# hagabbar/GenNet

Hardware: AMD Instinct MI355X
Metric: waveforms/sec (CNN+GAN step, 2048-sample BBH) (higher is better)
Workload: dtype f32

## Files before the change

### gennet_amd/csrc/bn.hip

```cpp
#include "common.h"

namespace gn {


__device__ __forceinline__ float bn_bwd_g(float dy, float y, uint8_t keep, int act, float p, float keep_scale) {
  if (!keep) return 0.f;
  const float yact = y / keep_scale;
  return dy * keep_scale * act_grad_from_y(yact, act, p);
}

__device__ __forceinline__ float bn_bwd_g_act(float dy, float yact, uint8_t keep, int act, float p, float keep_scale) {
  if (!keep) return 0.f;
  return dy * keep_scale * act_grad_from_y(yact, act, p);
}

__device__ __forceinline__ void lazy_dy_taps(const LazyDy& z, int C, int q, float wq[5][4]) {
#pragma unroll
  for (int j = 0; j < 5; ++j) {
    float4 w4 = make_float4(0.f, 0.f, 0.f, 0.f);
    if (j < z.k) w4 = *reinterpret_cast<const float4*>(z.w + (size_t)j * C + 4 * q);
    wq[j][0] = w4.x; wq[j][1] = w4.y; wq[j][2] = w4.z; wq[j][3] = w4.w;
  }
}
struct LazyWin {
  float win;
  int base;
  unsigned b;
};
template <bool UNI>
__device__ __forceinline__ void lazy_dy4(const LazyDy& z, unsigned b, int t, const float wq[5][4], float v[4], LazyWin& w) {
  float gv[5];
  if (UNI) {
    b = __builtin_amdgcn_readfirstlane(b);
    t = __builtin_amdgcn_readfirstlane(t);
    const int uhi = t + z.pad_left, ulo = uhi - (z.k - 1);
    if (b != w.b || ulo < w.base || uhi >= w.base + 64) {
      w.b = b;
      w.base = ulo;
      const int idx = ulo + (int)(threadIdx.x & 63);
      w.win = (idx >= 0 && idx < z.Lout) ? z.g[(size_t)b * z.Lout + idx] : 0.f;
    }
#pragma unroll
    for (int j = 0; j < 5; ++j)
      gv[j] = __int_as_float(__builtin_amdgcn_readlane(__float_as_int(w.win), max(uhi - j - w.base, 0)));
  } else {
    const float* gb = z.g + (size_t)b * z.Lout;
#pragma unroll
    for (int j = 0; j < 5; ++j) {
      const int u = t - j + z.pad_left;
      const int uc = min(max(u, 0), z.Lout - 1);
      const float g = gb[uc];
      gv[j] = (u == uc) ? g : 0.f;
    }
  }
  v[0] = v[1] = v[2] = v[3] = 0.f;
#pragma unroll
  for (int j = 0; j < 5; ++j)
#pragma unroll
    for (int e = 0; e < 4; ++e) v[e] = fmaf(gv[j], wq[j][e], v[e]);
}
__device__ __forceinline__ void lazy_dy_pos(const LazyDy& z, size_t r, unsigned* b, int* t) {
  *b = (unsigned)(r / (unsigned)z.L);
  *t = (int)(r - (size_t)*b * z.L);
}
__device__ __forceinline__ void lazy_dy_step(const LazyDy& z, int step, unsigned* b, int* t) {
  *t += step;
  while (*t >= z.L) { *t -= z.L; ++*b; }
}

template <int MODE>
__global__ __launch_bounds__(256) void colred_kernel(ColRedArgs a) {
  constexpr int NV = MODE == 0 ? 1 : 2;
  const int NQ = a.C >> 2;
  const int NQc = NQ < 256 ? NQ : 256;
  const int RL = 256 / NQc;
  const int tid = threadIdx.x, ql = tid % NQc, rl = tid / NQc;
  const int q = blockIdx.x * NQc + ql;
  double s[NV][4];
#pragma unroll
  for (int v = 0; v < NV; ++v)
#pragma unroll
    for (int e = 0; e < 4; ++e) s[v][e] = 0.0;
// ... 172 lines not shown
  else hipLaunchKernelGGL((colred_final_kernel<OUT, 32>), dim3(cdiv(n, 32)), dim3(256), 0, s, part, out, n, chunks);
}

static int colred_chunks(size_t rows, int C) {
  if (C % 4) {
    const int NCc = C < 256 ? C : 256, RL = 256 / NCc;
    const int gx = (C + NCc - 1) / NCc;
    int chunks = (1024 + gx - 1) / gx;
    const size_t max_chunks = (rows + (size_t)RL * 4 - 1) / ((size_t)RL * 4);
    if ((size_t)chunks > max_chunks) chunks = (int)max_chunks;
    return chunks < 1 ? 1 : chunks;
  }
  const int NQ = C / 4, NQc = NQ < 256 ? NQ : 256, RL = 256 / NQc;
  const int gx = (NQ + NQc - 1) / NQc;
  int chunks = (1024 + gx - 1) / gx;
  const size_t max_chunks = (rows + (size_t)RL * 4 - 1) / ((size_t)RL * 4);
  if ((size_t)chunks > max_chunks) chunks = (int)max_chunks;
  if (chunks < 1) chunks = 1;
  return chunks;
}
size_t colred_workspace_bytes(size_t rows, int C) { return (size_t)colred_chunks(rows, C) * 2 * C * sizeof(double); }

int colred_run(int mode, ColRedArgs a, void* ws, size_t ws_bytes, double* out_f64, float* out_f32, hipStream_t s) {
  if (a.C < 1) { set_error("column reduction: C %d", a.C); return GN_EINVAL; }
  if (a.C % 4 && a.lz.g) { set_error("column reduction: the on-the-fly conv gradient needs C %% 4 == 0"); return GN_EINVAL; }
  if (a.rows == 0) { set_error("column reduction: no rows"); return GN_EINVAL; }
  const int chunks = colred_chunks(a.rows, a.C);
  const int NV = mode == 0 ? 1 : 2;
  if (ws_bytes < (size_t)chunks * NV * a.C * sizeof(double)) { set_error("column reduction: workspace too small"); return GN_EWORKSPACE; }
  a.part = (double*)ws;
  a.rows_per_chunk = (int)((a.rows + chunks - 1) / chunks);
  if (a.C % 4) {
    const int NCc = a.C < 256 ? a.C : 256;
    dim3 grid((a.C + NCc - 1) / NCc, chunks);
    if (mode == 0) hipLaunchKernelGGL(colred_anyc_kernel<0>, grid, dim3(256), 0, s, a);
    else if (mode == 1) hipLaunchKernelGGL(colred_anyc_kernel<1>, grid, dim3(256), 0, s, a);
    else hipLaunchKernelGGL(colred_anyc_kernel<2>, grid, dim3(256), 0, s, a);
  } else {
    const int NQ = a.C / 4, NQc = NQ < 256 ? NQ : 256;
    dim3 grid((NQ + NQc - 1) / NQc, chunks);
    if (mode == 0) hipLaunchKernelGGL(colred_kernel<0>, grid, dim3(256), 0, s, a);
    else if (mode == 1) hipLaunchKernelGGL(colred_kernel<1>, grid, dim3(256), 0, s, a);
    else hipLaunchKernelGGL(colred_kernel<2>, grid, dim3(256), 0, s, a);
  }
  int rc = check_launch("colred");
  if (rc) return rc;
  const size_t n = (size_t)NV * a.C;
  if (out_f32) colred_final_launch((const double*)ws, out_f32, n, chunks, s);
  else colred_final_launch((const double*)ws, out_f64, n, chunks, s);
  return check_launch("colred_final");
}

int colred_finalize(const double* part, double* out_f64, size_t n, int chunks, hipStream_t s) {
  colred_final_launch(part, out_f64, n, chunks, s);
  return check_launch("colred_final");
}
int colred_finalize_f32(const double* part, float* out_f32, size_t n, int chunks, hipStream_t s) {
  colred_final_launch(part, out_f32, n, chunks, s);
  return check_launch("colred_final");
}

__global__ void colsum_anyc_kernel(const float* __restrict__ x, double* __restrict__ acc, size_t n, int C) {
  double s[4] = {0, 0, 0, 0};
  const size_t stride = (size_t)gridDim.x * blockDim.x;
  for (size_t i = (size_t)blockIdx.x * blockDim.x + threadIdx.x; i < n; i += stride) {
    const int c = (int)(i % C);
    const double v = (double)x[i];
    s[0] += c == 0 ? v : 0.0; s[1] += c == 1 ? v : 0.0; s[2] += c == 2 ? v : 0.0; s[3] += c == 3 ? v : 0.0;
  }
  __shared__ double red[4][256];
  for (int c = 0; c < 4; ++c) red[c][threadIdx.x] = s[c];
  __syncthreads();
  for (int sft = 128; sft >= 1; sft >>= 1) {
    if (threadIdx.x < sft)
      for (int c = 0; c < 4; ++c) red[c][threadIdx.x] += red[c][threadIdx.x + sft];
    __syncthreads();
  }
  if (threadIdx.x < C) atomicAdd(&acc[threadIdx.x], red[threadIdx.x][0]);
}
__global__ void f64_to_f32_small_kernel(const double* __restrict__ a, float* __restrict__ o, int n) {
  if ((int)threadIdx.x < n) o[threadIdx.x] = (float)a[threadIdx.x];
}

int bias_grad(const float* dy, float* db, size_t rows, int C, void* ws, size_t ws_bytes, hipStream_t s) {
  if (C % 4 == 0 || C > 4) {
    ColRedArgs r = {};
    r.a = dy; r.rows = rows; r.C = C;
    return colred_run(0, r, ws, ws_bytes, nullptr, db, s);
  }
  if (ws_bytes < 32) { set_error("bias_grad: workspace too small"); return GN_EWORKSPACE; }
  (void)hipMemsetAsync(ws, 0, 32, s);
  size_t g = (rows * C + 255) / 256;
  if (g > 1024) g = 1024;
  hipLaunchKernelGGL(colsum_anyc_kernel, dim3((unsigned)g), dim3(256), 0, s, dy, (double*)ws, rows * C, C);
  hipLaunchKernelGGL(f64_to_f32_small_kernel, dim3(1), dim3(64), 0, s, (const double*)ws, db, C);
  return check_launch("bias_grad");
}

size_t bias_grad_ws(size_t rows, int C) { return C % 4 == 0 || C > 4 ? colred_workspace_bytes(rows, C) : 32; }

__global__ void bn_finalize_kernel(const double* __restrict__ sums, double count, const float* __restrict__ gamma, const float* __restrict__ beta,
                                   float eps, float momentum, float* __restrict__ mm, float* __restrict__ mv, float* __restrict__ bm,
                                   float* __restrict__ bv, float zd_step, float* __restrict__ scale,
                                   float* __restrict__ shift, float* __restrict__ smean, float* __restrict__ sinv, int C, const int32_t* __restrict__ zd_step_dev) {
  const int c = blockIdx.x * blockDim.x + threadIdx.x;
  if (c >= C) return;
  if (zd_step_dev) zd_step = (float)*zd_step_dev;
  const double mean = sums[c] / count;
  double var = sums[C + c] / count - mean * mean;
  if (var < 0) var = 0;
  const float meanf = (float)mean, varf = (float)var;
  const float inv = 1.0f / sqrtf(varf + eps);
  const float sc = gamma[c] * inv;
  scale[c] = sc;
  shift[c] = beta[c] - meanf * sc;
  smean[c] = meanf;
  sinv[c] = inv;
  if (mm) {
    const float corr = (float)(count / (count - (1.0 + (double)eps)));
    const float decay = (float)(1.0 - (double)momentum);
    const float varc = varf * corr;
    if (bm) {
      const float nbm = bm[c] - (bm[c] - meanf) * decay;
      const float nbv = bv[c] - (bv[c] - varc) * decay;
      bm[c] = nbm;
      bv[c] = nbv;
      const float unb = 1.0f - powf(1.0f - decay, zd_step);
      mm[c] = mm[c] - (mm[c] - nbm / unb);
      mv[c] = mv[c] - (mv[c] - nbv / unb);
    } else {
      mm[c] = mm[c] - (mm[c] - meanf) * decay;
      mv[c] = mv[c] - (mv[c] - varc) * decay;
    }
  }
}
static int bn_finalize(const double* sums, double count, const float* gamma, const float* beta, float eps, float momentum, float* mm, float* mv,
                float* bm, float* bv, float zd_step, float* scale, float* shift, float* smean, float* sinv, int C, hipStream_t s, const int32_t* zd_step_dev = nullptr) {
  hipLaunchKernelGGL(bn_finalize_kernel, dim3(cdiv(C, 256)), dim3(256), 0, s, sums, count, gamma, beta, eps, momentum, mm, mv, bm, bv, zd_step, scale, shift,
                     smean, sinv, C, zd_step_dev);
  return check_launch("bn_finalize");
}

__global__ void bn_infer_coeffs_kernel(const float* __restrict__ gamma, const float* __restrict__ beta, const float* __restrict__ mm,
                                       const float* __restrict__ mv, float eps, float* __restrict__ scale, float* __restrict__ shift, int C) {
  const int c = blockIdx.x * blockDim.x + threadIdx.x;
  if (c >= C) return;
  const float sc = gamma[c] / sqrtf(mv[c] + eps);
  scale[c] = sc;
  shift[c] = beta[c] - mm[c] * sc;
}

__global__ void bn_apply_kernel(const float4* __restrict__ x, const float4* __restrict__ scale, const float4* __restrict__ shift,
                                const uchar4* __restrict__ mask, float4* __restrict__ y, size_t n4, int C4, int act, float p, float keep_scale) {
  const size_t stride = (size_t)gridDim.x * blockDim.x;
  for (size_t i = (size_t)blockIdx.x * blockDim.x + threadIdx.x; i < n4; i += stride) {
    const int c = (int)(i % C4);
    const float4 v = x[i], sc = scale[c], sh = shift[c];
    float4 o;
    o.x = act_apply(fmaf(v.x, sc.x, sh.x), act, p); o.y = act_apply(fmaf(v.y, sc.y, sh.y), act, p);
    o.z = act_apply(fmaf(v.z, sc.z, sh.z), act, p); o.w = act_apply(fmaf(v.w, sc.w, sh.w), act, p);
    if (mask) {
      const uchar4 m = mask[i];
      o.x = m.x ? o.x * keep_scale : 0.f; o.y = m.y ? o.y * keep_scale : 0.f;
      o.z = m.z ? o.z * keep_scale : 0.f; o.w = m.w ? o.w * keep_scale : 0.f;
    }
    y[i] = o;
  }
}
__global__ void bn_apply_anyc_kernel(const float* __restrict__ x, const float* __restrict__ scale, const float* __restrict__ shift,
                                     const uint8_t* __restrict__ mask, float* __restrict__ y, size_t n, int C, int act, float p, float keep_scale) {
  const size_t stride = (size_t)gridDim.x * blockDim.x;
  for (size_t i = (size_t)blockIdx.x * blockDim.x + threadIdx.x; i < n; i += stride) {
    const int c = (int)(i % C);
    float o = act_apply(fmaf(x[i], scale[c], shift[c]), act, p);
    if (mask) o = mask[i] ? o * keep_scale : 0.f;
    y[i] = o;
  }
}

__global__ void bn_bwd_apply_kernel(const float* __restrict__ dy, const float* __restrict__ y, const float* __restrict__ x, const uint8_t* __restrict__ mask,
                                    const float* __restrict__ gamma, const float* __restrict__ mean, const float* __restrict__ invstd,
                                    const double* __restrict__ dsums, double count, float* __restrict__ dx, size_t n, int C, int act, float p, float keep_scale,
                                    const float* __restrict__ scale, const float* __restrict__ shift) {
  const size_t stride = (size_t)gridDim.x * blockDim.x;
  for (size_t i = (size_t)blockIdx.x * blockDim.x + threadIdx.x; i < n; i += stride) {
    const int c = (int)(i % C);
    const uint8_t keep = mask ? mask[i] : (uint8_t)1;
    const float g = scale ? bn_bwd_g_act(dy[i], act_apply(fmaf(x[i], scale[c], shift[c]), act, p), keep, act, p, keep_scale)
                          : bn_bwd_g(dy[i], y[i], keep, act, p, keep_scale);
    const float inv = invstd[c];
    const float xh = (x[i] - mean[c]) * inv;
    const float mg = (float)(dsums[c] / count), mgx = (float)(dsums[C + c] / count);
    dx[i] = gamma[c] * inv * (g - mg - xh * mgx);
  }
}
__global__ __launch_bounds__(256) void bn_bwd_apply_v4_kernel(const float* __restrict__ dy, const float* __restrict__ y, const float* __restrict__ x,
                                                              const uint8_t* __restrict__ mask, const float* __restrict__ gamma, const float* __restrict__ mean,
                                                              const float* __restrict__ invstd, const double* __restrict__ dsums, double count,
                                                              const float* __restrict__ scale, const float* __restrict__ shift, float* __restrict__ dx,
                                                              size_t rows, int C, int rows_per_chunk, int act, float p, float keep_scale, LazyDy lz) {
  const int NQ = C >> 2;
  const int NQc = NQ < 256 ? NQ : 256;
  const int RL = 256 / NQc;
  const int tid = threadIdx.x, ql = tid % NQc, rl = tid / NQc;
  const int qblocks = (NQ + NQc - 1) / NQc;
  const int q = (blockIdx.x % qblocks) * NQc + ql;
  const size_t r_lo = (size_t)(blockIdx.x / qblocks) * rows_per_chunk;
  const size_t r_hi = r_lo + rows_per_chunk < rows ? r_lo + rows_per_chunk : rows;
  if (rl >= RL || q >= NQ) return;
  float gi[4], mu[4], is[4], mg[4], mgx[4], sc[4] = {0, 0, 0, 0}, sh[4] = {0, 0, 0, 0};
#pragma unroll
  for (int e = 0; e < 4; ++e) {
    const int c = 4 * q + e;
    is[e] = invstd[c]; mu[e] = mean[c]; gi[e] = gamma[c] * is[e];
    mg[e] = (float)(dsums[c] / count); mgx[e] = (float)(dsums[C + c] / count);
    if (scale) { sc[e] = scale[c]; sh[e] = shift[c]; }
  }
  float wq[5][4];
  LazyWin lw = {0.f, 0, 0xffffffffu};
  unsigned lb = 0;
  int lt = 0;
  if (lz.g) {
    lazy_dy_taps(lz, C, q, wq);
    lazy_dy_pos(lz, r_lo + rl, &lb, &lt);
  }
  constexpr int U = 2;
  const bool uni = ((NQc | NQ) & 63) == 0;
  for (size_t r = r_lo + rl; r < r_hi; r += (size_t)RL * U) {
    float4 d4[U], x4[U], y4[U];
    uchar4 m4[U];
    bool ok[U];
#pragma unroll
    for (int u = 0; u < U; ++u) {
      const size_t ru = r + (size_t)u * RL;
      ok[u] = ru < r_hi;
      const size_t o = (ok[u] ? ru : r) * C + 4 * q;
      x4[u] = *reinterpret_cast<const float4*>(x + o);
      if (!lz.g) d4[u] = *reinterpret_cast<const float4*>(dy + o);
      if (!scale) y4[u] = *reinterpret_cast<const float4*>(y + o);
      m4[u] = mask ? *reinterpret_cast<const uchar4*>(mask + o) : make_uchar4(1, 1, 1, 1);
    }
#pragma unroll
    for (int u = 0; u < U; ++u) {
      if (!ok[u]) break;
      const size_t o = (r + (size_t)u * RL) * C + 4 * q;
      const float xv[4] = {x4[u].x, x4[u].y, x4[u].z, x4[u].w};
      float dv[4];
      if (lz.g) {
        if (uni) lazy_dy4<true>(lz, lb, lt, wq, dv, lw);
        else lazy_dy4<false>(lz, lb, lt, wq, dv, lw);
        lazy_dy_step(lz, RL, &lb, &lt);
      } else {
        dv[0] = d4[u].x; dv[1] = d4[u].y; dv[2] = d4[u].z; dv[3] = d4[u].w;
      }
      float yv[4] = {0, 0, 0, 0};
      if (!scale) { yv[0] = y4[u].x; yv[1] = y4[u].y; yv[2] = y4[u].z; yv[3] = y4[u].w; }
      const uint8_t k[4] = {m4[u].x, m4[u].y, m4[u].z, m4[u].w};
      float ov[4];
#pragma unroll
      for (int e = 0; e < 4; ++e) {
        const float g = scale ? bn_bwd_g_act(dv[e], act_apply(fmaf(xv[e], sc[e], sh[e]), act, p), k[e], act, p, keep_scale)
                              : bn_bwd_g(dv[e], yv[e], k[e], act, p, keep_scale);
        const float xh = (xv[e] - mu[e]) * is[e];
        ov[e] = gi[e] * (g - mg[e] - xh * mgx[e]);
      }
      *reinterpret_cast<float4*>(dx + o) = make_float4(ov[0], ov[1], ov[2], ov[3]);
    }
  }
}
__global__ void bn_param_grads_kernel(const double* __restrict__ dsums_local, float* __restrict__ dgamma, float* __restrict__ dbeta, int C) {
  const int c = blockIdx.x * blockDim.x + threadIdx.x;
  if (c >= C) return;
  dbeta[c] = (float)dsums_local[c];
  dgamma[c] = (float)dsums_local[C + c];
}
static int bn_bwd_apply(const float* dy, const float* y, const float* x, const uint8_t* mask, const float* gamma, const float* mean, const float* invstd,
                 const double* dsums_global, double count, const double* dsums_local, float* dx, float* dgamma, float* dbeta, size_t rows, int C,
                 int act, float p, float rate, const float* scale, const float* shift, hipStream_t s, const LazyDy* lz = nullptr) {
  const size_t n = rows * C;
  if (!n) return GN_OK;
  LazyDy z = {};
  if (lz) z = *lz;
  if (z.g && (C % 4 || !scale)) { set_error("bn_bwd_apply: the on-the-fly conv gradient needs C %% 4 == 0 and scale / shift"); return GN_EINVAL; }
  if (C % 4 == 0) {
    const int NQ = C / 4, NQc = NQ < 256 ? NQ : 256, RL = 256 / NQc, qblocks = cdiv(NQ, NQc);
    size_t chunks = 8192 / qblocks;
    if (chunks < 1) chunks = 1;
    size_t rpc = (rows + chunks - 1) / chunks;
    rpc = ((rpc + RL - 1) / RL) * RL;
    if (rpc < (size_t)RL) rpc = RL;
    chunks = (rows + rpc - 1) / rpc;
    hipLaunchKernelGGL(bn_bwd_apply_v4_kernel, dim3((unsigned)(chunks * qblocks)), dim3(256), 0, s, dy, y, x, mask, gamma, mean, invstd, dsums_global, count, scale,
                       shift, dx, rows, C, (int)rpc, act, p, 1.0f / (1.0f - rate), z);
  } else {
    if (!y && !scale) { set_error("bn_bwd_apply: C %d %% 4 != 0 needs the stored layer output y or scale / shift", C); return GN_EINVAL; }
    hipLaunchKernelGGL(bn_bwd_apply_kernel, dim3(stream_grid(n)), dim3(256), 0, s, dy, y, x, mask, gamma, mean, invstd, dsums_global, count, dx, n, C, act, p,
                       1.0f / (1.0f - rate), y ? nullptr : scale, y ? nullptr : shift);
  }
  int rc = check_launch("bn_bwd_apply");
  if (rc) return rc;
  hipLaunchKernelGGL(bn_param_grads_kernel, dim3(cdiv(C, 256)), dim3(256), 0, s, dsums_local, dgamma, dbeta, C);
  return check_launch("bn_param_grads");
}

static int lazy_dy_check(const char* who, const float* g, const float* w, int L, int Lout, int k, int pad_left, size_t rows, int C, const float* scale,
                         const float* shift, LazyDy* z) {
  GN_REQUIRE(g && w && L > 0 && Lout > 0 && k >= 1 && k <= 5 && pad_left >= 0, "%s: bad conv description (1 filter, 1..5 taps, stride 1)", who);
  GN_REQUIRE(C % 4 == 0 && scale && shift, "%s: needs C %% 4 == 0 and the forward pass' scale / shift", who);
  GN_REQUIRE(rows % (size_t)L == 0 && rows / (size_t)L < 0x7fffffffull, "%s: rows %zu is not a whole number of length-%d segments", who, rows, L);
  z->g = g; z->w = w; z->L = L; z->Lout = Lout; z->k = k; z->pad_left = pad_left;
  return GN_OK;
}

}

using namespace gn;

extern "C" {

size_t gn_bn_stats_workspace(size_t rows, int C) { return colred_workspace_bytes(rows, C) + 256; }

int gn_bn_stats(const float* x, size_t rows, int C, double* sums, void* ws, size_t ws_bytes, void* stream) {
  GN_REQUIRE(x && sums && ws && rows > 0 && C > 0, "bn_stats: bad arguments");
  ColRedArgs r = {};
  r.a = x; r.rows = rows; r.C = C;
  return colred_run(1, r, ws, ws_bytes, sums, nullptr, (hipStream_t)stream);
}

int gn_bn_finalize(const double* sums, double count, const float* gamma, const float* beta, float eps, float momentum, float* moving_mean, float* moving_var,
                   float* scale, float* shift, float* save_mean, float* save_invstd, int C, void* stream) {
  GN_REQUIRE(sums && gamma && beta && scale && shift && save_mean && save_invstd && C > 0 && count > 1.0, "bn_finalize: bad arguments");
  GN_REQUIRE((moving_mean == nullptr) == (moving_var == nullptr), "bn_finalize: moving_mean/moving_var must both be given or both be NULL");
  return bn_finalize(sums, count, gamma, beta, eps, momentum, moving_mean, moving_var, nullptr, nullptr, 0.f, scale, shift, save_mean, save_invstd, C,
                     (hipStream_t)stream);
}
int gn_bn_finalize_zero_debias(const double* sums, double count, const float* gamma, const float* beta, float eps, float momentum, float* moving_mean,
                               float* moving_var, float* biased_mean, float* biased_var, int local_step, float* scale, float* shift, float* save_mean,
                               float* save_invstd, int C, void* stream) {
  GN_REQUIRE(sums && gamma && beta && scale && shift && save_mean && save_invstd && C > 0 && count > 1.0, "bn_finalize_zero_debias: bad arguments");
  GN_REQUIRE(moving_mean && moving_var && biased_mean && biased_var && local_step >= 1,
             "bn_finalize_zero_debias: needs moving_mean/var, the biased accumulators and the incremented local_step (>= 1, got %d)", local_step);
  return bn_finalize(sums, count, gamma, beta, eps, momentum, moving_mean, moving_var, biased_mean, biased_var, (float)local_step, scale, shift, save_mean,
                     save_invstd, C, (hipStream_t)stream);
}
int gn_bn_finalize_zero_debias_dyn(const double* sums, double count, const float* gamma, const float* beta, float eps, float momentum, float* moving_mean,
                                   float* moving_var, float* biased_mean, float* biased_var, const int32_t* local_step_dev, float* scale, float* shift,
                                   float* save_mean, float* save_invstd, int C, void* stream) {
  GN_REQUIRE(sums && gamma && beta && scale && shift && save_mean && save_invstd && C > 0 && count > 1.0, "bn_finalize_zero_debias_dyn: bad arguments");
  GN_REQUIRE(moving_mean && moving_var && biased_mean && biased_var && local_step_dev, "bn_finalize_zero_debias_dyn: needs moving statistics, accumulators, step");
  return bn_finalize(sums, count, gamma, beta, eps, momentum, moving_mean, moving_var, biased_mean, biased_var, 1.f, scale, shift, save_mean, save_invstd, C,
                     (hipStream_t)stream, local_step_dev);
}

int gn_bn_infer_coeffs(const float* gamma, const float* beta, const float* moving_mean, const float* moving_var, float eps, float* scale, float* shift, int C,
                       void* stream) {
  GN_REQUIRE(gamma && beta && moving_mean && moving_var && scale && shift && C > 0, "bn_infer_coeffs: bad arguments");
  hipLaunchKernelGGL(bn_infer_coeffs_kernel, dim3(cdiv(C, 256)), dim3(256), 0, (hipStream_t)stream, gamma, beta, moving_mean, moving_var, eps, scale, shift, C);
  return check_launch("bn_infer_coeffs");
}

int gn_bn_apply(const float* x, const float* scale, const float* shift, const uint8_t* mask, float* y, size_t rows, int C, int act, float p, float rate,
                void* stream) {
  GN_REQUIRE(x && scale && shift && y && C > 0, "bn_apply: bad arguments");
  GN_REQUIRE(rate >= 0.f && rate < 1.f && (mask || rate == 0.f), "bn_apply: dropout rate %f without mask", rate);
  hipStream_t s = (hipStream_t)stream;
  const float keep_scale = 1.0f / (1.0f - (mask ? rate : 0.f));
  if (C % 4) {
    const size_t n = rows * C;
    if (!n) return GN_OK;
    hipLaunchKernelGGL(bn_apply_anyc_kernel, dim3(stream_grid(n)), dim3(256), 0, s, x, scale, shift, mask, y, n, C, act, p, keep_scale);
    return check_launch("bn_apply");
  }
  const size_t n4 = rows * (C / 4);
  if (!n4) return GN_OK;
  hipLaunchKernelGGL(bn_apply_kernel, dim3(stream_grid(n4)), dim3(256), 0, s, (const float4*)x, (const float4*)scale, (const float4*)shift, (const uchar4*)mask,
                     (float4*)y, n4, C / 4, act, p, keep_scale);
  return check_launch("bn_apply");
}

int gn_bn_bwd_stats(const float* dy, const float* y, const float* x, const uint8_t* mask, const float* save_mean, const float* save_invstd, double* dsums, void* ws,
                    size_t ws_bytes, size_t rows, int C, int act, float p, float rate, const float* scale, const float* shift, void* stream) {
  GN_REQUIRE(dy && x && save_mean && save_invstd && dsums && ws && rows > 0 && C > 0, "bn_bwd_stats: bad arguments");
  GN_REQUIRE((scale == nullptr) == (shift == nullptr) && (y || scale), "bn_bwd_stats: needs the layer output y, or scale AND shift to recompute it");
  ColRedArgs r = {};
  r.a = dy; r.y = y; r.xpre = x; r.mask = mask; r.mean = save_mean; r.invstd = save_invstd; r.scale = scale; r.shift = shift;
  r.rows = rows; r.C = C; r.act = act; r.act_param = p; r.keep_scale = 1.0f / (1.0f - (mask ? rate : 0.f));
  return colred_run(2, r, ws, ws_bytes, dsums, nullptr, (hipStream_t)stream);
}
int gn_bn_bwd_apply(const float* dy, const float* y, const float* x, const uint8_t* mask, const float* gamma, const float* save_mean, const float* save_invstd,
                    const double* dsums_global, double count, const double* dsums_local, float* dx, float* dgamma, float* dbeta, size_t rows, int C, int act,
                    float p, float rate, const float* scale, const float* shift, void* stream) {
  GN_REQUIRE(dy && x && gamma && save_mean && save_invstd && dsums_global && dsums_local && dx && dgamma && dbeta && C > 0, "bn_bwd_apply: bad arguments");
  GN_REQUIRE((scale == nullptr) == (shift == nullptr) && (y || scale), "bn_bwd_apply: needs the layer output y, or scale AND shift to recompute it");
  return bn_bwd_apply(dy, y, x, mask, gamma, save_mean, save_invstd, dsums_global, count, dsums_local, dx, dgamma, dbeta, rows, C, act, p, mask ? rate : 0.f, scale,
                      shift, (hipStream_t)stream);
}

int gn_bn_bwd_stats_conv1(const float* g, const float* w, int L, int Lout, int k, int pad_left, const float* x, const uint8_t* mask, const float* save_mean,
                          const float* save_invstd, double* dsums, void* ws, size_t ws_bytes, size_t rows, int C, int act, float p, float rate,
                          const float* scale, const float* shift, void* stream) {
  GN_REQUIRE(x && save_mean && save_invstd && dsums && ws && rows > 0 && C > 0, "bn_bwd_stats_conv1: bad arguments");
  ColRedArgs r = {};
  int rc = lazy_dy_check("bn_bwd_stats_conv1", g, w, L, Lout, k, pad_left, rows, C, scale, shift, &r.lz);
  if (rc) return rc;
  r.a = nullptr; r.y = nullptr; r.xpre = x; r.mask = mask; r.mean = save_mean; r.invstd = save_invstd; r.scale = scale; r.shift = shift;
  r.rows = rows; r.C = C; r.act = act; r.act_param = p; r.keep_scale = 1.0f / (1.0f - (mask ? rate : 0.f));
  return colred_run(2, r, ws, ws_bytes, dsums, nullptr, (hipStream_t)stream);
}
int gn_bn_bwd_apply_conv1(const float* g, const float* w, int L, int Lout, int k, int pad_left, const float* x, const uint8_t* mask, const float* gamma,
                          const float* save_mean, const float* save_invstd, const double* dsums_global, double count, const double* dsums_local, float* dx,
                          float* dgamma, float* dbeta, size_t rows, int C, int act, float p, float rate, const float* scale, const float* shift, void* stream) {
  GN_REQUIRE(x && gamma && save_mean && save_invstd && dsums_global && dsums_local && dx && dgamma && dbeta && C > 0, "bn_bwd_apply_conv1: bad arguments");
  LazyDy z = {};
  int rc = lazy_dy_check("bn_bwd_apply_conv1", g, w, L, Lout, k, pad_left, rows, C, scale, shift, &z);
  if (rc) return rc;
  return bn_bwd_apply(nullptr, nullptr, x, mask, gamma, save_mean, save_invstd, dsums_global, count, dsums_local, dx, dgamma, dbeta, rows, C, act, p,
                      mask ? rate : 0.f, scale, shift, (hipStream_t)stream, &z);
}

size_t gn_bias_grad_workspace(size_t rows, int C) { return bias_grad_ws(rows, C) + 256; }

int gn_bias_grad(const float* dy, float* db, void* ws, size_t ws_bytes, size_t rows, int C, void* stream) {
  GN_REQUIRE(dy && db && ws && rows > 0 && C > 0, "bias_grad: bad arguments");
  return bias_grad(dy, db, rows, C, ws, ws_bytes, (hipStream_t)stream);
}

}
```

### gennet_amd/csrc/capi.hip

```cpp
#include <stdarg.h>
#include <algorithm>
#include <mutex>
#include <vector>
#include <stdlib.h>
#include "common.h"

namespace gn {

static thread_local char g_err[512] = "";

void set_error(const char* fmt, ...) {
  va_list ap;
  va_start(ap, fmt);
  vsnprintf(g_err, sizeof(g_err), fmt, ap);
  va_end(ap);
}

int check_launch(const char* what) {
  hipError_t e = hipGetLastError();
  if (e != hipSuccess) {
    set_error("%s: %s", what, hipGetErrorString(e));
    return GN_ELAUNCH;
  }
  return GN_OK;
// ... 393 lines not shown
  return dgrad_impl(dy, wt, dx, B, L, Cin, Cout, k, stride, pad_left, Lout, y_prev, mask_prev, act_prev, act_param_prev, mask_prev ? rate_prev : 0.f, stream);
}

static WgradArgs wgrad_args(const float* x, const float* dy, void* ws, int B, int L, int Cin, int Cout, int k, int stride, int pad_left, int Lout) {
  WgradArgs a = {};
  a.x = x; a.dy = dy; a.part = (float*)ws;
  a.B = B; a.Lin = L; a.Cin = Cin; a.Cout = Cout; a.M = Lout; a.ntaps = k; a.in_stride = stride;
  for (int j = 0; j < k && j < 8; ++j) a.off[j] = j - pad_left;
  return a;
}

size_t gn_conv1d_wgrad_workspace(int B, int L, int Cin, int Cout, int k, int stride, int Lout) {
  WgradArgs a = wgrad_args(nullptr, nullptr, nullptr, B, L, Cin, Cout, k, stride, 0, Lout);
  a.any_channels = 1;
  return std::max(wgrad_ws_need(select_wgrad(a), a), bias_grad_ws((size_t)B * Lout, Cout)) + 256;
}

static int wgrad_impl(const float* x, const float* dy, float* dw, float* db, void* ws, size_t ws_bytes, int B, int L, int Cin, int Cout, int k, int stride,
                      int pad_left, int Lout, bool any_channels, void* stream) {
  GN_REQUIRE(x && dy && dw && ws, "conv1d_wgrad: null pointer");
  GN_REQUIRE(B > 0 && L > 0 && Cin > 0 && Cout > 0 && k >= 1 && k <= 5 && stride >= 1 && Lout > 0 && pad_left >= 0, "conv1d_wgrad: bad shape");
  hipStream_t s = (hipStream_t)stream;
  WgradArgs a = wgrad_args(x, dy, ws, B, L, Cin, Cout, k, stride, pad_left, Lout);
  a.db = db;
  a.any_channels = any_channels;
  const WgradFamily f = select_wgrad(a);
  int rc = ws_check("conv1d_wgrad", std::max(wgrad_ws_need(f, a), bias_grad_ws((size_t)B * Lout, Cout)) + 256, ws_bytes);
  if (rc) return rc;
  switch (f) {
    case WGRAD_SMALL: {
      WgradSmallArgs sa = {x, dy, (float*)ws, B, L, Cin, Cout, Lout, k, stride};
      std::copy(a.off, a.off + k, sa.off);
      rc = wgrad_small_dispatch(sa, dw, ws_bytes, s);
      break;
    }
    case WGRAD_WINO: rc = wgrad_wino_run(a, dw, s); break;
    case WGRAD_WINO_S2: rc = wgrad_wino_s2_run(a, dw, s); break;
    case WGRAD_ANYC: rc = wgrad_anyc_dispatch(a, dw, ws_bytes, s); break;
    case WGRAD_BF16X3:
      rc = ws_check("conv-math", wgrad_bf16x3_workspace_bytes(B, Lout, Cin, Cout, stride), g_conv_ws_bytes);
      if (!rc) rc = wgrad_bf16x3_dispatch(a, dw, g_conv_ws, g_conv_ws_bytes, s);
      break;
    default:
      rc = wgrad_mfma_dispatch(a, dw, ws_bytes, s);
      if (!rc && a.db_done) return GN_OK;
  }
  if (rc) return rc;
  return db ? bias_grad(dy, db, (size_t)B * Lout, Cout, ws, ws_bytes, s) : GN_OK;
}

int gn_conv1d_wgrad(const float* x, const float* dy, float* dw, float* db, void* ws, size_t ws_bytes, int B, int L, int Cin, int Cout, int k, int stride,
                    int pad_left, int Lout, void* stream) {
  return wgrad_impl(x, dy, dw, db, ws, ws_bytes, B, L, Cin, Cout, k, stride, pad_left, Lout, false, stream);
}
int gn_conv1d_wgrad_any(const float* x, const float* dy, float* dw, float* db, void* ws, size_t ws_bytes, int B, int L, int Cin, int Cout, int k, int stride,
                        int pad_left, int Lout, void* stream) {
  return wgrad_impl(x, dy, dw, db, ws, ws_bytes, B, L, Cin, Cout, k, stride, pad_left, Lout, true, stream);
}

int gn_dense_fwd(const float* x, const float* w, const float* bias, float* y, int B, int in, int out, int act, float act_param, void* stream) {
  GN_REQUIRE(x && w && y && B >= 0 && in > 0 && out > 0, "dense_fwd: bad arguments");
  if (B == 0) return GN_OK;
  if (dense_any_shape(in, out))
    return dense_any_gemm(x, w, bias, y, B, out, in, (size_t)in, 1, (size_t)out, 1, act, act_param, (hipStream_t)stream);
  if (out <= 4) return dense_small_fwd(x, w, bias, y, B, in, out, act, act_param, (hipStream_t)stream);
  return conv_mfma_dispatch(fwd_args(x, w, bias, y, 1, B, in, out, 1, 1, 0, B, act, act_param), (hipStream_t)stream);
}

size_t gn_dense_bwd_workspace(int B, int in, int out) {
  if (out <= 4) return 256;
  if (dense_any_shape(in, out)) return bias_grad_ws((size_t)B, out) + 256;
  size_t w = wgrad_workspace_bytes(1, B, in, out, 1);
  size_t b = bias_grad_ws((size_t)B, out);
  return (w > b ? w : b) + (size_t)in * out * sizeof(float) + 256;
}

int gn_dense_bwd_fused(const float* x, const float* w, const float* dy, float* dx, float* dw, float* db, int B, int in, int out, const uint8_t* mask_prev,
                       int act_prev, float act_param_prev, float rate_prev, void* stream) {
  GN_REQUIRE(x && w && dy && dx && dw && B > 0 && in > 0 && out >= 1 && out <= 4, "dense_bwd_fused: bad arguments (small-output heads only)");
  GN_REQUIRE(rate_prev >= 0.f && rate_prev < 1.f, "dense_bwd_fused: bad rate");
  return dense_small_bwd(x, w, dy, dx, dw, db, B, in, out, (hipStream_t)stream, act_prev, act_param_prev, mask_prev, 1.0f / (1.0f - (mask_prev ? rate_prev : 0.f)));
}

int gn_dense_bwd(const float* x, const float* w, const float* dy, float* dx, float* dw, float* db, void* ws, size_t ws_bytes, int B, int in, int out, void* stream) {
  GN_REQUIRE(x && w && dy && dw && B > 0 && in > 0 && out > 0, "dense_bwd: bad arguments");
  hipStream_t s = (hipStream_t)stream;
  if (dense_any_shape(in, out)) {
    GN_REQUIRE(ws, "dense_bwd: null workspace");
    if (int rc = ws_check("dense_bwd", gn_dense_bwd_workspace(B, in, out), ws_bytes)) return rc;
    int rc = dx ? dense_any_gemm(dy, w, nullptr, dx, B, in, out, (size_t)out, 1, 1, (size_t)out, GN_ACT_LINEAR, 0.f, s) : GN_OK;
    if (!rc) rc = dense_any_gemm(x, dy, nullptr, dw, in, out, B, 1, (size_t)in, (size_t)out, 1, GN_ACT_LINEAR, 0.f, s);
    if (!rc && db) rc = bias_grad(dy, db, (size_t)B, out, ws, ws_bytes, s);
    return rc;
  }
  if (out <= 4) return dense_small_bwd(x, w, dy, dx, dw, db, B, in, out, s);
  GN_REQUIRE(ws, "dense_bwd: null workspace");
  if (int rc = ws_check("dense_bwd", gn_dense_bwd_workspace(B, in, out), ws_bytes)) return rc;
  const size_t wt_bytes = (size_t)in * out * sizeof(float);
  float* wt = (float*)ws;
  void* ws2 = (char*)ws + wt_bytes;
  const size_t ws2_bytes = ws_bytes - wt_bytes;
  int rc;
  if (dx) {
    rc = transpose_w(w, wt, 1, in, out, s);
    if (rc) return rc;
    rc = conv_run(fwd_args(dy, wt, nullptr, dx, 1, B, out, in, 1, 1, 0, B, GN_ACT_LINEAR, 0.f), s);
    if (rc) return rc;
  }
  WgradArgs g = wgrad_args(x, dy, ws2, 1, B, in, out, 1, 1, 0, B);
  rc = wgrad_mfma_dispatch(g, dw, ws2_bytes, s);
  if (rc) return rc;
  if (db) rc = bias_grad(dy, db, (size_t)B, out, ws2, ws2_bytes, s);
  return rc;
}

}
```

### gennet_amd/csrc/common.h

```cpp
#pragma once
#include <hip/hip_runtime.h>
#include <stdint.h>
#include <stdio.h>
#include "../../include/gennet_hip.h"

#define GN_LDS_DMA_CLOBBER() asm volatile("" ::: "v0", "v1", "v2", "v3")
#define gn_buffer_load_lds(...) do { __builtin_amdgcn_raw_ptr_buffer_load_lds(__VA_ARGS__); GN_LDS_DMA_CLOBBER(); } while (0)
#define gn_global_load_lds(...) do { __builtin_amdgcn_global_load_lds(__VA_ARGS__); GN_LDS_DMA_CLOBBER(); } while (0)

namespace gn {

void set_error(const char* fmt, ...);
int check_launch(const char* what);

struct Switches {
  bool conv_nopipe, conv_nodma, conv_nomerge, conv_nonarrow, conv_nopatch;
  bool wgrad_nopipe, bf16x3_no_merge;
  double bf16x3_min_gflop;
};
const Switches& switches();

const uint64_t* rng_base();
void prof_begin(hipStream_t s);
void prof_end(hipStream_t s, double flop, int kind, double bytes = 0.0);
// ... 39 lines not shown
  int ntaps, in_stride;
  int off[8];
  int chunks_per_split;
  double* db_part;
  float* db;
  int db_done;
  int any_channels;
};

struct WgradSmallArgs {
  const float* x;
  const float* dy;
  float* part;
  int B, Lin, Cin, Cout, M;
  int ntaps, in_stride;
  int off[8];
  int rows_per_chunk;
};

struct LazyDy {
  const float* g;
  const float* w;
  int L, Lout, k, pad_left;
};

struct ColRedArgs {
  const float* a;
  const float* y;
  const float* xpre;
  const uint8_t* mask;
  const float* mean;
  const float* invstd;
  const float* scale;
  const float* shift;
  double* part;
  size_t rows;
  int C;
  int rows_per_chunk;
  int act;
  float act_param;
  float keep_scale;
  LazyDy lz;
};

int conv_mfma_dispatch(const ConvArgs& a, hipStream_t s);
size_t wgrad_workspace_bytes(int B, int M, int Cin, int Cout, int ntaps);
int wgrad_mfma_dispatch(WgradArgs& a, float* dw, size_t ws_bytes, hipStream_t s);
int wgrad_bf16x3_dispatch(WgradArgs& a, float* dw, void* split_ws, size_t split_ws_bytes, hipStream_t s);
int conv_pipe_try(const ConvArgs& a, bool tall, hipStream_t s, bool* launched);
bool conv_pipe_merged_supported(const ConvArgs& a);
int conv_pipe_run_merged(const ConvArgs& a, hipStream_t s);
void wgrad_pipe_launch(const WgradArgs& a, dim3 grid, bool narrow, hipStream_t s);
size_t conv_bf16x3_workspace_bytes(int B, int Lin, int Cin, int Cout, int w_taps);
bool conv_bf16x3_supported(const ConvArgs& a);
int conv_bf16x3_split(const ConvArgs& a, int w_taps, void* ws, size_t ws_bytes, bool split_x, bool split_w, hipStream_t s);
int conv_bf16x3_run(const ConvArgs& a, int w_taps, void* ws, hipStream_t s);
int conv_bf16x3_merged_kind(const ConvArgs& a);
int conv_bf16x3_run_merged(const ConvArgs& a, void* ws, hipStream_t s);
size_t conv_wino_workspace_bytes(int Cin, int Cout);
bool conv_wino_supported(const ConvArgs& a);
int conv_wino_run(const ConvArgs& a, void* ws, size_t ws_bytes, hipStream_t s);
size_t conv_wino_s2_workspace_bytes(int Cin, int Cout);
int conv_wino_s2_kind(const ConvArgs& a);
int conv_wino_s2_run(const ConvArgs& a, void* ws, size_t ws_bytes, hipStream_t s);
void wgrad_split_plan(int B, int M, int Cin, int Cout, int TC, int TN, int* splits, int* chunks_per_split);
bool wgrad_wino_supported(const WgradArgs& a);
size_t wgrad_wino_workspace_bytes(int B, int M, int Cin, int Cout);
int wgrad_wino_run(WgradArgs& a, float* dw, hipStream_t s);
bool wgrad_wino_s2_supported(const WgradArgs& a);
size_t wgrad_wino_s2_workspace_bytes(int B, int M, int Cin, int Cout);
int wgrad_wino_s2_run(WgradArgs& a, float* dw, hipStream_t s);
size_t wgrad_bf16x3_workspace_bytes(int B, int M, int Cin, int Cout, int in_stride);
bool wgrad_bf16x3_supported(const WgradArgs& a);
int wgrad_bf16x3_run(const WgradArgs& a, int splits, void* ws, size_t ws_bytes, hipStream_t s);
int conv_anyc_dispatch(const ConvArgs& a, hipStream_t s);
size_t wgrad_anyc_workspace_bytes(int B, int M, int Cin, int Cout, int ntaps);
int wgrad_anyc_dispatch(WgradArgs& a, float* dw, size_t ws_bytes, hipStream_t s);
int conv_smallcin_dispatch(const ConvArgs& a, hipStream_t s);
int conv_smallcout_dispatch(const ConvArgs& a, hipStream_t s);
size_t wgrad_small_workspace_bytes(int B, int M, int Cin, int Cout, int ntaps);
int wgrad_small_dispatch(WgradSmallArgs a, float* dw, size_t ws_bytes, hipStream_t s);
int dense_small_fwd(const float* x, const float* w, const float* bias, float* y, int B, int in, int out, int act, float p, hipStream_t s);
int dense_small_bwd(const float* x, const float* w, const float* dy, float* dx, float* dw, float* db, int B, int in, int out, hipStream_t s,
                    int gact = 0, float gparam = 0.f, const uint8_t* gmask = nullptr, float gscale = 1.f);
size_t colred_workspace_bytes(size_t rows, int C);
int colred_run(int mode, ColRedArgs a, void* ws, size_t ws_bytes, double* out_f64, float* out_f32, hipStream_t s);
int colred_finalize(const double* part, double* out_f64, size_t n, int chunks, hipStream_t s);
int colred_finalize_f32(const double* part, float* out_f32, size_t n, int chunks, hipStream_t s);
size_t bias_grad_ws(size_t rows, int C);
int bias_grad(const float* dy, float* db, size_t rows, int C, void* ws, size_t ws_bytes, hipStream_t s);
int transpose_w(const float* w, float* wt, int k, int Cin, int Cout, hipStream_t s);

static inline unsigned cdiv(size_t a, size_t b) { return (unsigned)((a + b - 1) / b); }
static inline unsigned stream_grid(size_t n_items, int block = 256) {
  size_t g = (n_items + block - 1) / block;
  if (g > 256 * 8) g = 256 * 8;
  if (g < 1) g = 1;
  return (unsigned)g;
}

static inline void allow_big_lds(const void* kernel, unsigned long long* done) {
  int dev = 0;
  (void)hipGetDevice(&dev);
  const unsigned long long bit = 1ull << (dev & 63);
  if (!(*done & bit)) {
    (void)hipFuncSetAttribute(kernel, hipFuncAttributeMaxDynamicSharedMemorySize, 160 * 1024);
    *done |= bit;
  }
}

#define GN_REQUIRE(cond, ...)            \
  do {                                   \
    if (!(cond)) {                       \
      gn::set_error(__VA_ARGS__);        \
      return GN_EINVAL;                  \
    }                                    \
  } while (0)

__device__ __forceinline__ float gn_tanhf(float x) {
  const float ax = fabsf(x);
  const float e = __builtin_amdgcn_exp2f(ax * 2.8853900817779268f);
  const float big = 1.f - 2.f * __builtin_amdgcn_rcpf(e + 1.f);
  const float x2 = ax * ax;
  float q = fmaf(x2, -1382.f / 155925.f, 62.f / 2835.f);
  q = fmaf(x2, q, -17.f / 315.f);
  q = fmaf(x2, q, 2.f / 15.f);
  q = fmaf(x2, q, -1.f / 3.f);
  const float small = fmaf(ax * x2, q, ax);
  return copysignf(ax < 0.35f ? small : big, x);
}

__device__ __forceinline__ float act_apply(float x, int act, float p) {
  switch (act) {
    case GN_ACT_RELU: return fmaxf(x, 0.f);
    case GN_ACT_RELU_MAX: return fminf(fmaxf(x, 0.f), p);
    case GN_ACT_LEAKY: return x > 0.f ? x : p * x;
    case GN_ACT_TANH: return gn_tanhf(x);
    case GN_ACT_SIGMOID: return 1.f / (1.f + expf(-x));
    default: return x;
  }
}

__device__ __forceinline__ float act_grad_from_y(float y, int act, float p) {
  switch (act) {
    case GN_ACT_RELU: return y > 0.f ? 1.f : 0.f;
    case GN_ACT_RELU_MAX: return (y > 0.f && y < p) ? 1.f : 0.f;
    case GN_ACT_LEAKY: return y > 0.f ? 1.f : p;
    case GN_ACT_TANH: return 1.f - y * y;
    case GN_ACT_SIGMOID: return y * (1.f - y);
    default: return 1.f;
  }
}

struct Philox4 {
  uint32_t v[4];
};

__host__ __device__ __forceinline__ uint32_t mulhi32(uint32_t a, uint32_t b) { return (uint32_t)(((uint64_t)a * b) >> 32); }

__host__ __device__ __forceinline__ Philox4 philox4x32_10(uint64_t counter, uint64_t seed) {
  uint32_t c0 = (uint32_t)counter, c1 = (uint32_t)(counter >> 32), c2 = 0, c3 = 0;
  uint32_t k0 = (uint32_t)seed, k1 = (uint32_t)(seed >> 32);
#pragma unroll
  for (int r = 0; r < 10; ++r) {
    const uint32_t M0 = 0xD2511F53u, M1 = 0xCD9E8D57u;
    uint32_t h0 = mulhi32(M0, c0), l0 = M0 * c0;
    uint32_t h1 = mulhi32(M1, c2), l1 = M1 * c2;
// ... 17 lines not shown
```

### gennet_amd/csrc/small_conv.hip

```cpp
#include "common.h"

namespace gn {

static double small_conv_flop(int B, int M, int ntaps, int Cin, int Cout) { return 2.0 * B * (double)M * ntaps * Cin * Cout; }


constexpr int SMALLCIN_WIN = (2 * 255 + 5) * 4 + 4;

template <int CIN>
__global__ __launch_bounds__(256) void conv_smallcin_kernel(ConvArgs a, int m_tiles, int MT) {
  constexpr int MAXT = 5;
  const int NQ = a.Cout >> 2;
  const int NQc = NQ < 256 ? NQ : 256;
  const int RL = 256 / NQc;
  const int tid = threadIdx.x;
  const int q0 = tid % NQc, rl = tid / NQc;
  const int m_tile = blockIdx.x % m_tiles, b = blockIdx.x / m_tiles;
  const int m_lo = m_tile * MT, m_hi = min(a.M, m_lo + MT);
  const float* xb = a.x + (size_t)b * a.Lin * CIN;
  float* yb = a.y + (size_t)b * a.Ly * a.Cout;
  __shared__ float xw[SMALLCIN_WIN];
  int minoff = a.t.off[0], maxoff = a.t.off[0];
  for (int j = 1; j < a.t.ntaps; ++j) {
    minoff = min(minoff, a.t.off[j]);
// ... 510 lines not shown
    switch (CS) {
      case 1: hipLaunchKernelGGL(wgrad_smallcout_s1_kernel<1>, grid, dim3(256), 0, s, a); break;
      case 2: hipLaunchKernelGGL(wgrad_smallcout_s1_kernel<2>, grid, dim3(256), 0, s, a); break;
      case 3: hipLaunchKernelGGL(wgrad_smallcout_s1_kernel<3>, grid, dim3(256), 0, s, a); break;
      default: hipLaunchKernelGGL(wgrad_smallcout_s1_kernel<4>, grid, dim3(256), 0, s, a); break;
    }
    prof_end(s, small_conv_flop(a.B, a.M, a.ntaps, a.Cin, a.Cout), 16);
    int rc1 = check_launch("wgrad_smallcout_s1");
    if (rc1) return rc1;
    const size_t n1 = (size_t)a.ntaps * a.Cin * a.Cout;
    return sum_partials(a.part, dw, n1, chunks, s);
  }
#define GN_WS(CSV)                                                                                            \
  if (small_in) hipLaunchKernelGGL((wgrad_smallcin_tab_kernel<CSV>), grid, dim3(256), 0, s, a);               \
  else hipLaunchKernelGGL((wgrad_small_kernel<CSV, false>), grid, dim3(256), 0, s, a);
  prof_begin(s);
  switch (CS) {
    case 1: GN_WS(1); break;
    case 2: GN_WS(2); break;
    case 3: GN_WS(3); break;
    default: GN_WS(4); break;
  }
#undef GN_WS
  prof_end(s, small_conv_flop(a.B, a.M, a.ntaps, a.Cin, a.Cout), small_in ? 14 : 15);
  int rc = check_launch("wgrad_small");
  if (rc) return rc;
  const size_t n = (size_t)a.ntaps * a.Cin * a.Cout;
  return sum_partials(a.part, dw, n, chunks, s);
}

template <int OUT>
__global__ __launch_bounds__(1024) void dense_small_fwd_kernel(const float* __restrict__ x, const float* __restrict__ w, const float* __restrict__ bias,
                                                               float* __restrict__ y, int in, int act, float act_param) {
  const int b = blockIdx.x, tid = threadIdx.x;
  const float* xb = x + (size_t)b * in;
  float acc[OUT];
#pragma unroll
  for (int o = 0; o < OUT; ++o) acc[o] = 0.f;
  for (int i = 4 * tid; i < in; i += 4096) {
    const float4 xv = *reinterpret_cast<const float4*>(xb + i);
    if (OUT == 1) {
      const float4 wv = *reinterpret_cast<const float4*>(w + i);
      acc[0] = fmaf(xv.x, wv.x, acc[0]); acc[0] = fmaf(xv.y, wv.y, acc[0]);
      acc[0] = fmaf(xv.z, wv.z, acc[0]); acc[0] = fmaf(xv.w, wv.w, acc[0]);
    } else {
      const float xs[4] = {xv.x, xv.y, xv.z, xv.w};
#pragma unroll
      for (int e = 0; e < 4; ++e)
#pragma unroll
        for (int o = 0; o < OUT; ++o) acc[o] = fmaf(xs[e], w[(size_t)(i + e) * OUT + o], acc[o]);
    }
  }
  __shared__ float red[16][OUT];
#pragma unroll
  for (int o = 0; o < OUT; ++o) {
    float v = acc[o];
#pragma unroll
    for (int sft = 32; sft >= 1; sft >>= 1) v += __shfl_xor(v, sft, 64);
    if ((tid & 63) == 0) red[tid >> 6][o] = v;
  }
  __syncthreads();
  if (tid < OUT) {
    float v = 0.f;
    for (int k = 0; k < 16; ++k) v += red[k][tid];
    y[(size_t)b * OUT + tid] = act_apply(v + (bias ? bias[tid] : 0.f), act, act_param);
  }
}

int dense_small_fwd(const float* x, const float* w, const float* bias, float* y, int B, int in, int out, int act, float p, hipStream_t s) {
  if (out < 1 || out > 4 || in % 4) {
    set_error("dense_small_fwd: out %d (1..4) / in %d (%%4) unsupported", out, in);
    return GN_EINVAL;
  }
  if (B == 0) return GN_OK;
  switch (out) {
    case 1: hipLaunchKernelGGL(dense_small_fwd_kernel<1>, dim3(B), dim3(1024), 0, s, x, w, bias, y, in, act, p); break;
    case 2: hipLaunchKernelGGL(dense_small_fwd_kernel<2>, dim3(B), dim3(1024), 0, s, x, w, bias, y, in, act, p); break;
    case 3: hipLaunchKernelGGL(dense_small_fwd_kernel<3>, dim3(B), dim3(1024), 0, s, x, w, bias, y, in, act, p); break;
    default: hipLaunchKernelGGL(dense_small_fwd_kernel<4>, dim3(B), dim3(1024), 0, s, x, w, bias, y, in, act, p); break;
  }
  return check_launch("dense_small_fwd");
}

template <int OUT>
__global__ __launch_bounds__(256) void dense_small_bwd_kernel(const float* __restrict__ x, const float* __restrict__ w, const float* __restrict__ dy,
                                                              float* __restrict__ dx, float* __restrict__ dw, int B, int in, int gact, float gparam,
                                                              const uint8_t* __restrict__ gmask, float gscale) {
  const size_t i = ((size_t)blockIdx.x * 256 + threadIdx.x) * 4;
  if (i >= (size_t)in) return;
  float wv[4][OUT], acc[4][OUT];
#pragma unroll
  for (int e = 0; e < 4; ++e)
#pragma unroll
    for (int o = 0; o < OUT; ++o) {
      wv[e][o] = w[(i + e) * OUT + o];
      acc[e][o] = 0.f;
    }
  constexpr int U = 8;
  for (int b0 = 0; b0 < B; b0 += U) {
    float4 xq[U];
    uchar4 mq[U];
#pragma unroll
    for (int u = 0; u < U; ++u) {
      const int bb = min(b0 + u, B - 1);
      xq[u] = *reinterpret_cast<const float4*>(x + (size_t)bb * in + i);
      mq[u] = (dx && gmask) ? *reinterpret_cast<const uchar4*>(gmask + (size_t)bb * in + i) : make_uchar4(1, 1, 1, 1);
    }
#pragma unroll
    for (int u = 0; u < U; ++u) {
    const int b = b0 + u;
    if (b >= B) break;
    const float4 xv = xq[u];
    const float xs[4] = {xv.x, xv.y, xv.z, xv.w};
    float g[OUT];
#pragma unroll
    for (int o = 0; o < OUT; ++o) g[o] = dy[(size_t)b * OUT + o];
    float d[4] = {0.f, 0.f, 0.f, 0.f};
#pragma unroll
    for (int e = 0; e < 4; ++e)
#pragma unroll
      for (int o = 0; o < OUT; ++o) {
        acc[e][o] = fmaf(xs[e], g[o], acc[e][o]);
        d[e] = fmaf(g[o], wv[e][o], d[e]);
      }
    if (dx) {
      if (gact != GN_ACT_LINEAR || gmask) {
        const uint8_t k[4] = {mq[u].x, mq[u].y, mq[u].z, mq[u].w};
#pragma unroll
        for (int e = 0; e < 4; ++e) d[e] = k[e] ? d[e] * gscale * act_grad_from_y(xs[e] / gscale, gact, gparam) : 0.f;
      }
      *reinterpret_cast<float4*>(dx + (size_t)b * in + i) = make_float4(d[0], d[1], d[2], d[3]);
    }
    }
  }
#pragma unroll
  for (int e = 0; e < 4; ++e)
#pragma unroll
    for (int o = 0; o < OUT; ++o) dw[(i + e) * OUT + o] = acc[e][o];
}

__global__ void colsum_small_kernel(const float* __restrict__ dy, float* __restrict__ db, int B, int out) {
  const int o = threadIdx.x;
  if (o >= out) return;
  float s = 0.f;
  for (int b = 0; b < B; ++b) s += dy[(size_t)b * out + o];
  db[o] = s;
}

int dense_small_bwd(const float* x, const float* w, const float* dy, float* dx, float* dw, float* db, int B, int in, int out, hipStream_t s, int gact,
                    float gparam, const uint8_t* gmask, float gscale) {
  if (out < 1 || out > 4 || in % 4) {
    set_error("dense_small_bwd: out %d (1..4) / in %d (%%4) unsupported", out, in);
    return GN_EINVAL;
  }
  const unsigned grid = cdiv((size_t)in / 4, 256);
  switch (out) {
    case 1: hipLaunchKernelGGL(dense_small_bwd_kernel<1>, dim3(grid), dim3(256), 0, s, x, w, dy, dx, dw, B, in, gact, gparam, gmask, gscale); break;
    case 2: hipLaunchKernelGGL(dense_small_bwd_kernel<2>, dim3(grid), dim3(256), 0, s, x, w, dy, dx, dw, B, in, gact, gparam, gmask, gscale); break;
    case 3: hipLaunchKernelGGL(dense_small_bwd_kernel<3>, dim3(grid), dim3(256), 0, s, x, w, dy, dx, dw, B, in, gact, gparam, gmask, gscale); break;
    default: hipLaunchKernelGGL(dense_small_bwd_kernel<4>, dim3(grid), dim3(256), 0, s, x, w, dy, dx, dw, B, in, gact, gparam, gmask, gscale); break;
  }
  int rc = check_launch("dense_small_bwd");
  if (rc) return rc;
  if (db) {
    hipLaunchKernelGGL(colsum_small_kernel, dim3(1), dim3(64), 0, s, dy, db, B, out);
    rc = check_launch("colsum_small");
  }
  return rc;
}

}
```

### gennet_amd/engine.py

```python
import re

import numpy as np
import torch

from . import ops

_DEVICE = None


def device():
    global _DEVICE
    if _DEVICE is None:
        import os
        if not torch.cuda.is_available():
            from ._lib import GennetHipError
            raise GennetHipError('gennet_amd needs an AMD GPU (torch.cuda.is_available() is False); there is no CPU execution path')
        idx = int(os.environ.get('LOCAL_RANK', '0')) % max(torch.cuda.device_count(), 1)
        torch.cuda.set_device(idx)
        _DEVICE = torch.device('cuda', idx)
        ops.set_conv_math(device=_DEVICE)
    return _DEVICE


def to_device(a, dtype=torch.float32):
# ... 156 lines not shown
        i = len(self.providers)
        if i >= self.SLOTS:
            raise RuntimeError('StepGraph: more than %d step-varying scalars' % self.SLOTS)
        self.providers.append((i, fmt, provider))
        return ops.DevScalar(self.dev.data_ptr() + 8 * i)

    def capture(self, fn):
        global _CAPTURE
        if _CAPTURE is not None:
            raise RuntimeError('StepGraph.capture: already capturing')
        rng = device_rng()
        self.rng_start = rng.offset

        def keep(buf):
            if not any(b is buf for b in self.scratch):
                self.scratch.append(buf)

        def rng_base():
            base = device_rng().offset - self.rng_start
            device_rng().offset += self.rng_taken
            return base
        base = self.slot('Q', rng_base)
        if ops.conv_math_workspace() is not None:
            keep(ops.conv_math_workspace())
        self.graph = torch.cuda.CUDAGraph()
        _CAPTURE = self
        ops.set_rng_base(base.ptr)
        ops._ws_on_use = keep
        prof = ops.prof_enabled()
        if prof:
            ops.prof_enable(False)
        try:
            with torch.cuda.graph(self.graph):
                self.outputs = fn()
        finally:
            ops.set_rng_base(None)
            ops._ws_on_use = None
            _CAPTURE = None
            if prof:
                ops.prof_enable(True)
            self.rng_taken = rng.offset - self.rng_start
            rng.offset = self.rng_start
        return self.outputs

    def wait_inputs_consumed(self):
        if self._copied_once:
            self.copied.synchronize()

    def replay(self):
        for i, fmt, provider in self.providers:
            self._struct.pack_into('<' + fmt, self.hostbuf, 8 * i, provider())
        self.dev.copy_(self.host, non_blocking=True)
        self.copied.record()
        self._copied_once = True
        self.graph.replay()
        return self.outputs


def set_device_seed(seed):
    global _RNG
    _RNG = PhiloxStream(seed)


def device_rng():
    return _RNG


class RunContext(object):
    def __init__(self, training, dp=None, dropout_masks=None, train_params=None, site=None, row_map=None):
        self.training = training
        self.row_map = row_map
        self.site = site
        self.capture = None
        self.dp = dp
        self.dropout_masks = dropout_masks or {}
        self.train_ids = None if train_params is None else set(id(p) for p in train_params)
        self.tape = {}
        self.epi = {}
        self.pre_applied = set()
        self.skip = set()
        self.bn_sums = {}
        self.reg = None
        self.reg_y = {}

    def wants_grad(self, layer):
        if self.train_ids is None:
            return False
        return any(id(p) in self.train_ids for p in layer.trainable_params())


class SymTensor(object):
    def __init__(self, shape, layer=None, inbound=(), name=None):
        self.shape = tuple(shape)
        self.layer = layer
        self.inbound = tuple(inbound)
        self.name = name


_NAME_COUNTS = {}


def to_snake_case(name):
    intermediate = re.sub('(.)([A-Z][a-z0-9]+)', r'\1_\2', name)
    insecure = re.sub('([a-z])([A-Z])', r'\1_\2', intermediate).lower()
    return 'private' + insecure if insecure[0] == '_' else insecure


def _unique_name(base):
    _NAME_COUNTS[base] = _NAME_COUNTS.get(base, 0) + 1
    return '%s_%d' % (base, _NAME_COUNTS[base])


def Input(shape=None, name=None, batch_shape=None, dtype=None):
    if shape is None and batch_shape is not None:
        shape = tuple(batch_shape[1:])
    return SymTensor(shape, name=name or _unique_name('input'))


class Layer(object):

    def __init__(self, input_shape=None, name=None, trainable=True, **kwargs):
        if name is None:
            name = _unique_name(to_snake_case(self.__class__.__name__))
        self.name = name
        self.trainable = trainable
        self.built = False
        self.input_shape_arg = tuple(input_shape) if input_shape is not None else None
        self.params = []
        self.buffers = []

    def add_weight(self, name, value, trainable=True, regularizer=None):
        p = Param('%s/%s' % (self.name, name), value, trainable, regularizer)
        (self.params if trainable else self.buffers).append(p)
        return p

    def trainable_params(self):
        return self.params

    @property
    def trainable_weights(self):
        return list(self.params) if self.trainable else []

    @property
    def non_trainable_weights(self):
        return list(self.buffers) + ([] if self.trainable else list(self.params))

    @property
    def weights(self):
        return list(self.params) + list(self.buffers)

    def get_weights(self):
        return [p.numpy() for p in self.weights]

    def set_weights(self, ws):
        assert len(ws) == len(self.weights), '%s expects %d arrays' % (self.name, len(self.weights))
        for p, w in zip(self.weights, ws):
            p.assign(w)

    def count_params(self):
        return sum(p.size for p in self.weights)

    def build(self, input_shape):
        self.built = True

    def compute_output_shape(self, input_shape):
        return input_shape

    def get_config(self):
        from . import keras_io
        return keras_io.layer_config(self)

    def _is_user_layer(self):
        return callable(getattr(type(self), 'call', None)) and type(self).forward is Layer.forward

    def _ensure_built(self, input_shape):
        if not self.built:
            self.build((None,) + tuple(input_shape) if self._is_user_layer() else tuple(input_shape))
            self.built = True

    def _shape_after(self, input_shape):
        if self._is_user_layer():
            out = tuple(self.compute_output_shape((None,) + tuple(input_shape)))[1:]
            self._lower(tuple(input_shape), out)
            return out
        return tuple(self.compute_output_shape(tuple(input_shape)))

    def _lower(self, input_shape, out_shape):
        if getattr(self, '_lowered', None) is None or self._lowered_for != input_shape:
            from .keras import backend as K
            self._lowered = K.lower_layer_call(self, input_shape)
            self._lowered_for = input_shape
            if tuple(out_shape) != (input_shape[0], 2, 1):
                raise ValueError('%s.compute_output_shape gives %r; its call produces %r' % (type(self).__name__, (None,) + tuple(out_shape), (None, input_shape[0], 2, 1)))
        return self._lowered

    def __call__(self, x):
        if isinstance(x, (list, tuple)):
            if not self.is_merge:
                raise ValueError('%s (%s) takes a single tensor, not a list of %d: only the merge layers (Add, Subtract, Multiply, Average, Maximum, '
                                 'Minimum, Concatenate) join tensors' % (self.name, type(self).__name__, len(x)))
            if len(x) < 2:
                raise ValueError('A merge layer should be called on a list of at least 2 inputs (%s got %d)' % (self.name, len(x)))
            shapes = [tuple(t.shape) for t in x]
            if not self.built:
                self.build(shapes)
                self.built = True
            return SymTensor(tuple(self.compute_output_shape(shapes)), self, tuple(x))
        if self.is_merge:
            raise ValueError('A merge layer should be called on a list of at least 2 inputs (%s got a single tensor)' % self.name)
        self._ensure_built(x.shape)
        return SymTensor(self._shape_after(x.shape), self, (x,))

    is_merge = False
    fusable_act = False
    fusable_drop = False
    act_spec = None
    activity_regularizer = None
    drop_rate = None

    def writes_dy(self, node):
        return False

    def forward(self, ctx, node, x):
        if not self._is_user_layer():
            raise NotImplementedError
        low = self._lower(tuple(x.shape[1:]), tuple(node.out_shape))
        b0, b1 = low.betas()
        return ops.affine_stack_fwd(x.contiguous(), low.a0, b0, low.a1, b1)

    def backward(self, ctx, node, dy, need_dx, need_dw):
        if not self._is_user_layer():
            raise NotImplementedError
        return ops.affine_stack_bwd(dy.contiguous(), self._lowered.a0, self._lowered.a1)


class Node(object):
    __slots__ = ('layer', 'inbound', 'fused_act', 'fused_drop', 'absorbed', 'index', 'out_shape', 'owners', 'fuse_prev', 'infer_bn', 'fold_up', 'lazy_bn')

    def __init__(self, layer, inbound, out_shape, owners=()):
        self.layer = layer
        self.owners = tuple(owners)
        self.inbound = list(inbound)
        self.fused_act = None
        self.fused_drop = None
        self.absorbed = False
        self.index = -1
        self.out_shape = out_shape
        self.fuse_prev = -1
        self.fold_up = None
        self.infer_bn = None
        self.lazy_bn = -1


def _f32(x):
    return float(np.float32(x))


class Optimizer(object):
    RULE = None
    SLOTS = ()
    SAVES_ITERATIONS = True
    CONFIG = ()

    def __init__(self, lr, decay=0.0, clipnorm=None, clipvalue=None, **kwargs):
        if kwargs:
            raise TypeError('Unexpected keyword argument passed to optimizer: %s' % sorted(kwargs)[0])
        self.lr, self.decay = _f32(lr), _f32(decay)
        self.clipnorm, self.clipvalue = clipnorm, clipvalue
        self.iterations = 0
        self.state = None

    def _n_slots(self):
        return len(self.SLOTS)

    def _hyper(self):
        return 0.0, 0.0, 0.0, False

    def _lr_eff(self, it):
        return self.lr / (1.0 + self.decay * it) if self.decay > 0 else self.lr

    def _scalar(self, it):
        return self._lr_eff(it)

    def _layout(self):
        return list(range(self._n_slots()))

    def get_config(self):
        cfg = {'lr': self.lr}
        cfg.update((k, getattr(self, k)) for k in self.CONFIG)
        if self.clipnorm is not None:
            cfg['clipnorm'] = self.clipnorm
        if self.clipvalue is not None:
            cfg['clipvalue'] = self.clipvalue
        return cfg

    def bind(self, params):
        self.state = []
        for grp, a, b in segments(params):
            self.state.append((grp, a, b, [torch.zeros(b - a, dtype=torch.float32, device=device()) for _ in range(self._n_slots())]))
        self._partials = self._factor = None
        if self.clipnorm is not None and self.clipnorm > 0:
            self._part_slices, off = [], 0
            for _, a, b, _ in self.state:
                k = ops.optim_sumsq_slots(b - a)
                self._part_slices.append((off, k)); off += k
            self._partials = torch.zeros(off, dtype=torch.float64, device=device())
            self._factor = torch.ones(1, dtype=torch.float32, device=device())

    def _next_scalar(self):
        it = self.iterations
        self.iterations = it + 1
        return self._scalar(it)

    def _clip_scale(self):
        if self._partials is None:
            return None
        for (grp, a, b, _), (o, k) in zip(self.state, self._part_slices):
            ops.optim_sumsq(grp.grad[a:b], self._partials[o:o + k])
        ops.optim_clip_factor(self._partials, self.clipnorm, self._factor)
        return self._factor

    def _update(self, p, g, st, lr, clip):
        h0, h1, eps, nesterov = self._hyper()
        ops.optim_step(self.RULE, p, g, st, lr, h0, h1, eps, nesterov, clip, self.clipvalue if self.clipvalue and self.clipvalue > 0 else 0.0)

    def step(self):
        cap = capturing()
        lr = self._next_scalar() if cap is None else cap.slot('f', self._next_scalar)
        clip = self._clip_scale()
        for grp, a, b, st in self.state:
            self._update(grp.data[a:b], grp.grad[a:b], st, lr, clip)

    def _views(self, p):
        for grp, a, b, st in self.state:
# ... 225 lines not shown
                raise ValueError('graph reaches an Input that is not listed in inputs=')
            inb = [visit(s) for s in t.inbound]
            idx = self._append(t.layer, inb, t.shape)
            index[id(t)] = idx
            return idx

        self.output_ids = [visit(t) for t in outs]
        self.built = True

    def _append(self, layer, inbound, out_shape, owners=()):
        if isinstance(layer, Model):
            assert len(layer.input_shapes) == 1 and len(layer.output_ids) == 1 and len(inbound) == 1, 'nested models must be 1-in / 1-out'
            remap = {}
            for n in layer.nodes:
                inb = [inbound[0] if i < 0 else remap[i] for i in n.inbound]
                remap[n.index] = self._append(n.layer, inb, n.out_shape, tuple(owners) + (layer,) + n.owners)
            return remap[layer.output_ids[0]]
        node = Node(layer, inbound, out_shape, owners)
        node.index = len(self.nodes)
        self.nodes.append(node)
        self._planned = False
        return node.index

    @property
    def layers(self):
        seen, out = set(), []
        for n in self.nodes:
            if id(n.layer) not in seen:
                seen.add(id(n.layer))
                out.append(n.layer)
        return out

    @property
    def output_shape(self):
        shapes = [(None,) + tuple(self.nodes[i].out_shape) for i in self.output_ids]
        return shapes[0] if len(shapes) == 1 else shapes

    def compute_output_shape(self, input_shape):
        return self.nodes[self.output_ids[0]].out_shape

    def trainable_params(self):
        out = []
        for l in self.layers:
            out.extend(l.trainable_params())
        return out

    @property
    def trainable_weights(self):
        if not self.trainable:
            return []
        out = []
        for l in self.layers:
            out.extend(l.trainable_weights)
        return out

    @property
    def non_trainable_weights(self):
        out = []
        for l in self.layers:
            out.extend(l.non_trainable_weights if self.trainable else l.weights)
        return out

    @property
    def weights(self):
        out = []
        for l in self.layers:
            out.extend(l.weights)
        return out

    def get_weights(self):
        return [w for l in self.layers for w in l.get_weights()]

    def set_weights(self, ws):
        ws = list(ws)
        for l in self.layers:
            n = len(l.weights)
            l.set_weights(ws[:n])
            ws = ws[n:]
        assert not ws, 'too many weight arrays'

    def _plan(self):
        for n in self.nodes:
            n.fused_act, n.fused_drop, n.absorbed, n.fuse_prev, n.fold_up, n.infer_bn, n.lazy_bn = None, None, False, -1, None, None, -1
        consumers = {n.index: [] for n in self.nodes}
        for n in self.nodes:
            for i in n.inbound:
                if i >= 0:
                    consumers[i].append(n.index)
        outs = set(self.output_ids)

        def sole_consumer(i):
            if i in outs or len(consumers[i]) != 1:
                return None
            return self.nodes[consumers[i][0]]

        def areg(node):
            return node.layer.activity_regularizer is not None

        for n in self.nodes:
            if n.absorbed or areg(n):
                continue
            tail = n
            own_act = getattr(n.layer, 'activation', None)
            if n.layer.fusable_act and (own_act is None or own_act[0] == 'linear'):
                c = sole_consumer(tail.index)
                if c is not None and c.layer.act_spec is not None:
                    n.fused_act = c.layer.act_spec
                    c.absorbed = True
                    tail = c
            if n.layer.fusable_drop:
                c = sole_consumer(tail.index)
                if c is not None and c.layer.drop_rate is not None:
                    n.fused_drop = (c.layer.drop_rate, c.layer)
                    c.absorbed = True
        for n in self.nodes:
            if n.absorbed or not getattr(n.layer, 'is_upsample2', False) or len(n.inbound) != 1 or n.inbound[0] < 0:
                continue
            c = sole_consumer(n.index)
            if c is not None and not c.absorbed and not areg(c) and hasattr(c.layer, 'can_fold_upsample') and c.layer.can_fold_upsample():
                c.fold_up = n
                n.absorbed = True
        for n in self.nodes:
            if n.absorbed or areg(n) or not getattr(n.layer, 'can_fold_bn', False) or n.fused_act is not None or n.fused_drop is not None:
                continue
            c = sole_consumer(n.index)
            if c is not None and getattr(c.layer, 'is_batchnorm', False):
                n.infer_bn = c
        for n in self.nodes:
            if n.absorbed or len(n.inbound) != 1 or not getattr(n.layer, 'can_absorb_prev_act_bwd', False):
                continue
            cur, ok = n.inbound[0], True
            while cur >= 0 and (self.nodes[cur].absorbed or getattr(self.nodes[cur].layer, 'shape_only', False)):
                if len(consumers[cur]) != 1 or cur in outs:
                    ok = False
                    break
                cur = self.nodes[cur].inbound[0]
            if (ok and cur >= 0 and len(consumers[cur]) == 1 and cur not in outs and getattr(self.nodes[cur].layer, 'offers_act_bwd', False)
                    and not areg(self.nodes[cur])):
                n.fuse_prev = cur
        for n in self.nodes:
            if n.absorbed or len(n.inbound) != 1 or n.fold_up is not None or not hasattr(n.layer, 'can_defer_dgrad'):
                continue
            cur = n.inbound[0]
            while cur >= 0 and self.nodes[cur].absorbed and len(consumers[cur]) == 1 and cur not in outs:
                cur = self.nodes[cur].inbound[0]
            if cur < 0 or len(consumers[cur]) != 1 or cur in outs or not getattr(self.nodes[cur].layer, 'is_batchnorm', False) or self.nodes[cur].absorbed:
                continue
            shp = self.nodes[cur].out_shape
            if len(shp) == 2 and n.layer.can_defer_dgrad(shp[1]):
                n.lazy_bn = cur
        self._planned = True

    def _forward(self, inputs, ctx):
        if not self._planned:
            self._plan()
        vals = {}
        for k, x in enumerate(inputs):
            vals[-1 - k] = x
        for n in self.nodes:
            xs = [vals[i] for i in n.inbound]
            if n.absorbed:
                vals[n.index] = xs[0]
                continue
            vals[n.index] = n.layer.forward(ctx, n, xs[0] if len(xs) == 1 else xs)
            if ctx.reg is not None and n.layer.activity_regularizer is not None:
                y, r = vals[n.index].contiguous(), n.layer.activity_regularizer
                ops.reg_pass(y, None, r.l1, r.l2, ctx.reg[n.index])
                if ctx.training:
                    ctx.reg_y[n.index] = y
            if ctx.capture is not None:
                ctx.capture[n.layer.name] = vals[n.index]
        return [vals[i] for i in self.output_ids]

    def _backward(self, out_grads, ctx):
        grads, held = {}, {}

        def key(t):
            return t.untyped_storage().data_ptr() if isinstance(t, torch.Tensor) else id(t)

        def put(i, t):
            g = grads.get(i)
            if g is None:
                grads[i] = t
                held[key(t)] = held.get(key(t), 0) + 1
            elif held[key(g)] > 1:
                held[key(g)] -= 1
                grads[i] = g = ops.merge_fwd('add', [g.contiguous(), t.contiguous().view(g.shape)])
                held[key(g)] = held.get(key(g), 0) + 1
            else:
                ops.axpy(g, t, 1.0)

        def take(i):
            g = grads.pop(i, None)
            if g is not None:
                held[key(g)] -= 1
                if not held[key(g)]:
                    del held[key(g)]
            return g

        for i, g in zip(self.output_ids, out_grads):
            put(i, g)
        for n in reversed(self.nodes):
            dy = take(n.index)
            if dy is None:
                continue
            if n.index in ctx.reg_y:
                y, r = ctx.reg_y.pop(n.index), n.layer.activity_regularizer
                dy = ops.reg_grad(y, dy.contiguous().view(y.shape), r.l1, r.l2, inplace=key(dy) not in held)
            if n.absorbed:
                dxs = [dy]
            else:
                wanted = [i >= 0 for i in n.inbound]
                need_dx = any(wanted)
                need_dw = ctx.wants_grad(n.layer)
                if not need_dx and not need_dw:
                    continue
                if key(dy) in held and n.layer.writes_dy(n):
                    dy = ops.scale(dy.contiguous(), 1.0)
                if n.layer.is_merge:
                    dxs = n.layer.backward(ctx, n, dy, wanted, need_dw)
                else:
                    prev = ctx.epi.get(n.fuse_prev) if (n.fuse_prev >= 0 and need_dx) else None
                    dxs = [n.layer.backward(ctx, n, dy, need_dx, need_dw, prev) if prev is not None else n.layer.backward(ctx, n, dy, need_dx, need_dw)]
            for i, dx in zip(n.inbound, dxs):
                if i >= 0 and dx is not None:
                    put(i, dx)


    def compile(self, loss=None, optimizer=None, metrics=None, loss_weights=None, data_parallel=None, weighted_metrics=None, sample_weight_mode=None,
                **kwargs):
        if sample_weight_mode is not None:
            raise NotImplementedError('sample_weight_mode=%r: only per-sample weights (None), one weight per row' % (sample_weight_mode,))
        self.loss = loss
# ... 462 lines not shown
```

### gennet_amd/layers.py

```python
import collections

import numpy as np
import torch

from . import ops, regularizers
from .engine import Layer, Model, capturing, device, device_rng, glorot_uniform

import os as _os
_NO_DROPGEN = bool(_os.environ.get('GN_NO_DROPGEN'))
_NO_LAZYGRAD = bool(_os.environ.get('GN_NO_LAZYGRAD'))
_NO_UPFOLD = bool(_os.environ.get('GN_NO_UPFOLD'))
_NO_CONVSTATS = bool(_os.environ.get('GN_NO_CONVSTATS'))

_ACT_NAMES = {'relu': ('relu', 0.0), 'tanh': ('tanh', 0.0), 'sigmoid': ('sigmoid', 0.0), 'linear': ('linear', 0.0), None: ('linear', 0.0)}
_SOFTMAX = ('softmax', 0.0)
_LINEAR = ('linear', 0.0)


def _act_spec(activation, what):
    name = getattr(activation, '__name__', activation) if callable(activation) else activation
    if name == 'softmax':
        return _SOFTMAX
    if name not in _ACT_NAMES:
        raise NotImplementedError('%s(activation=%r): one of relu, tanh, sigmoid, linear, softmax' % (what, activation))
    return _ACT_NAMES[name]


def _activation_name(name):
    def fn(x, *a, **k):
        raise NotImplementedError('gennet_amd.keras.activations.%s is a name for activation=%r; applied to a tensor it has no HIP lowering: use the '
                                  'layer (Activation(%r)%s)' % (name, name, name, ', Softmax(axis)' if name == 'softmax' else ''))
    fn.__name__ = fn.__qualname__ = name
    return fn


ACTIVATIONS = dict((n, _activation_name(n)) for n in ('softmax', 'relu', 'tanh', 'sigmoid', 'linear'))


def _kernel_act(a):
    return _LINEAR if a is _SOFTMAX else a


def _is_softmax(layer):
    return getattr(layer, 'activation', None) is _SOFTMAX


def _channel_softmax(layer, y):
    P = layer.units if hasattr(layer, 'units') else layer.filters
    return ops.softmax_fwd(y, (y.numel() // P, P, 1), inplace=True)


def _check_init(kernel_initializer):
    if kernel_initializer not in (None, 'glorot_uniform'):
        raise NotImplementedError('kernel_initializer %r (only glorot_uniform is used on the hot path)' % (kernel_initializer,))


def _take_regularizers(layer, kernel, bias, activity):
    layer.kernel_regularizer, layer.bias_regularizer = regularizers.get(kernel), regularizers.get(bias)
    layer.activity_regularizer = regularizers.get(activity)


def _conv_fwd(node, ctx, x, w, b, stride, pl, Lout, act, out_shape_for_mask, any_channels=False, drop_ok=True):
    if node.fused_drop is not None:
        assert act is not _SOFTMAX, 'a fused Dropout on a softmax layer'
        assert not any_channels, 'a fused Dropout on a channel pair of the any-channel kernels (plan the model after building it)'
        if not drop_ok:
            raise NotImplementedError('Dropout directly after a Conv1D with <= 4 filters')
        if ctx.training and node.fused_drop[0] > 0.0:
            rate, drop_layer = node.fused_drop
            mask = drop_layer.make_mask(ctx, out_shape_for_mask)
            return ops.conv1d_fwd_dropout(x, w, b, mask, stride, pl, Lout, act[0], act[1], rate), mask, rate
    act = _kernel_act(act)
    return ops.conv1d_fwd(x, w, b, stride, pl, Lout, act[0], act[1], any_channels=any_channels), None, 0.0


def _conv_bwd_epilogue(dy, y, act, mask, rate, ctx=None, node=None):
    if act is _SOFTMAX:
        assert mask is None and node.index not in ctx.pre_applied
        P = node.layer.units if hasattr(node.layer, 'units') else node.layer.filters
        return ops.softmax_bwd(dy, y, (dy.numel() // P, P, 1), inplace=True)
    if ctx is not None and node.index in ctx.pre_applied:
        return dy
    if mask is not None:
        return ops.act_dropout_bwd(dy, y, mask, act[0], act[1], rate, inplace=True)
    if act[0] != 'linear':
        return ops.act_bwd(dy, y, act[0], act[1], inplace=True)
    return dy


def _epilogue_writes_dy(layer, node):
    a = node.fused_act or layer.activation
    return a[0] != 'linear' or node.fused_drop is not None


def _kconv_fwd(x, w, b, stride, pl, Lout, launch=ops.conv1d_fwd):
    if w.shape[0] > 5:
        x, w, pl = ops.conv1d_tapfold_x(x, w.shape[0], pl), ops.conv1d_tapfold_w(w), 0
    return launch(x, w, b, stride, pl, Lout), x, w


def _kconv_dgrad(dy, w, k, L, stride, pl, prev=None, any_channels=False, folded=False):
    if k <= 5:
        return ops.conv1d_dgrad(dy, ops.conv1d_transpose_w(w), L, stride, pl, prev, any_channels=any_channels)
    assert prev is None
    w2 = w if folded else ops.conv1d_tapfold_w(w)
    return ops.conv1d_tapunfold_dx(ops.conv1d_dgrad(dy, ops.conv1d_transpose_w(w2), L + pl, stride, 0, None, any_channels=any_channels), L, k, pl)


def _kconv_wgrad(x, dy, k, stride, pl, dw=None, db=None, want_db=True, any_channels=False, folded=False):
    if k <= 5:
        return ops.conv1d_wgrad(x, dy, k, stride, pl, dw, db, want_db, any_channels)
    x2 = x if folded else ops.conv1d_tapfold_x(x, k, pl)
    dw2, db = ops.conv1d_wgrad(x2, dy, ops.tap_groups(k)[1], stride, 0, None, db, want_db, any_channels)
    return ops.conv1d_tapunfold_dw(dw2, k, dw), db


def _launched_pair(k, Cin, Cout, up_folded=False, stride=1):
    return Cin * ops.tap_groups(k)[0] if k > 5 else Cin, 2 * Cout if up_folded and stride == 1 else Cout


class _ConvRun(object):
    __slots__ = ('L', 'Cin', 'k', 'stride', 'pl', 'Lout', 'tap_folded', 'up_folded', 'Cin_run', 'Cout_run', 'fwd_any', 'any_channels', 'phase')

    def __init__(self, layer, Cin, up_folded, L=None):
        self.L, self.Cin, self.up_folded, self.tap_folded, self.phase = L, Cin, up_folded, layer.k > 5, None
        self.k, self.stride = (3, 1) if up_folded else (layer.k, layer.stride)
        self.Cin_run, self.Cout_run = _launched_pair(layer.k, Cin, layer.filters, up_folded, layer.stride)
        self.fwd_any = ops.conv_needs_any(self.Cin_run, self.Cout_run)
        self.any_channels = self.fwd_any or ops.conv_needs_any(self.Cout_run, self.Cin_run)
        if L is not None and layer.phased:
            assert not up_folded
            d = layer.dilation
            Lout, pl = ops.conv_geometry(L, layer.k, layer.stride, layer.padding, d)
            pr = (layer.k - 1) * d - pl if layer.padding == 'same' else 0
            M = max(-(-(L + pl + pr) // d), layer.k)
            self.phase, self.L, self.pl, self.Lout = (d, pl, L, Lout), M, 0, (M - layer.k) // layer.stride + 1
            return
        self.Lout, self.pl = (None, None) if L is None else (L, 1) if up_folded else ops.conv_geometry(L, layer.k, layer.stride, layer.padding)


def _transpose_pair_ok(k, filters, Cin):
    a, b = _launched_pair(k, filters, Cin)
    return (a % 4 == 0 and b % 4 == 0) or (a <= 4 and b % 4 == 0) or (b <= 4 and a % 4 == 0)


_ConvTape = collections.namedtuple('_ConvTape', 'x y act mask rate w run pl in_shape', defaults=(None, None, None, None))


class Dense(Layer):
    fusable_act = True

    @property
    def offers_act_bwd(self):
        return not _is_softmax(self)

    @property
    def can_absorb_prev_act_bwd(self):
        k = getattr(self, 'kernel', None)
        return self.units <= 4 and (k is None or k.shape[0] % 4 == 0)

    def __init__(self, units, activation=None, kernel_initializer='glorot_uniform', use_bias=True, kernel_regularizer=None, bias_regularizer=None,
                 activity_regularizer=None, **kw):
        Layer.__init__(self, **kw)
        _check_init(kernel_initializer)
        _take_regularizers(self, kernel_regularizer, bias_regularizer, activity_regularizer)
        if not use_bias:
            raise NotImplementedError('Dense(use_bias=False)')
        self.units = int(units)
        self.activation = _act_spec(activation, 'Dense')

    def build(self, input_shape):
        assert len(input_shape) == 1, 'Dense expects (batch, features); Flatten first'
        self.kernel = self.add_weight('kernel', glorot_uniform((input_shape[0], self.units)), regularizer=self.kernel_regularizer)
        self.bias = self.add_weight('bias', np.zeros(self.units, np.float32), regularizer=self.bias_regularizer)

    def compute_output_shape(self, input_shape):
        return (self.units,)

    def forward(self, ctx, node, x):
        a = node.fused_act or self.activation
        ka = _kernel_act(a)
        y = ops.dense_fwd(x, self.kernel.data, self.bias.data, ka[0], ka[1])
        if a is _SOFTMAX:
            y = _channel_softmax(self, y)
        ctx.tape[node.index] = (x, y, a)
        if ctx.training and ka[0] != 'linear':
            ctx.epi[node.index] = (y, a[0], a[1], None, 0.0)
        return y

    def writes_dy(self, node):
        return _epilogue_writes_dy(self, node)

    def backward(self, ctx, node, dy, need_dx, need_dw, prev=None):
        x, y, a = ctx.tape.pop(node.index)
        dy = _conv_bwd_epilogue(dy.contiguous(), y, a, None, 0.0, ctx, node)
        if prev is not None:
            ctx.pre_applied.add(node.fuse_prev)
        if need_dw:
            dx, _, _ = ops.dense_bwd(x, self.kernel.data, dy, need_dx, self.kernel.grad, self.bias.grad, prev=prev)
            return dx
        dx, _, _ = ops.dense_bwd(x, self.kernel.data, dy, True, prev=prev)
        return dx


class Conv1D(Layer):
    fusable_act = True

    @property
    def phased(self):
        return self.dilation > 1 or self.padding == 'causal'

    @property
    def offers_act_bwd(self):
        return not self.phased and not _is_softmax(self)

    @property
    def can_absorb_prev_act_bwd(self):
        return not self.phased

    @property
    def fusable_drop(self):
        if self.phased:
            return False
        if _is_softmax(self):
            return False
        k = getattr(self, 'kernel', None)
        if k is None:
            return True
        if self.filters <= 4:
            return False
        return not any(_ConvRun(self, k.shape[1], up).any_channels for up in ((False, True) if self.can_fold_upsample() else (False,)))

    def __init__(self, filters, kernel_size, strides=1, padding='valid', activation=None, kernel_initializer='glorot_uniform', use_bias=True,
                 dilation_rate=1, kernel_regularizer=None, bias_regularizer=None, activity_regularizer=None, **kw):
        Layer.__init__(self, **kw)
        _check_init(kernel_initializer)
        _take_regularizers(self, kernel_regularizer, bias_regularizer, activity_regularizer)
        if not use_bias:
            raise NotImplementedError('Conv1D(use_bias=False)')
        self.filters = int(filters)
        self.k = int(kernel_size[0] if isinstance(kernel_size, (tuple, list)) else kernel_size)
        self.stride = int(strides[0] if isinstance(strides, (tuple, list)) else strides)
        if isinstance(dilation_rate, (tuple, list)):
            if len(dilation_rate) != 1:
                raise ValueError('Conv1D(dilation_rate=%r): an integer or a tuple / list of 1 integer' % (dilation_rate,))
            dilation_rate = dilation_rate[0]
        self.dilation = int(dilation_rate)
        if self.dilation < 1:
            raise ValueError('Conv1D(dilation_rate=%r): must be >= 1' % (dilation_rate,))
        if self.dilation > 1 and self.stride > 1:
            raise ValueError('Conv1D(strides=%d, dilation_rate=%d): strides > 1 and dilation_rate > 1 exclude each other (as in Keras)'
                             % (self.stride, self.dilation))
        if padding not in ('same', 'valid', 'causal'):
            raise NotImplementedError('padding %r' % (padding,))
        self.padding = padding
        self.activation = _act_spec(activation, 'Conv1D')

    def build(self, input_shape):
        L, Cin = input_shape
        if self.stride < 1 or (Cin > 4 and self.stride > 2):
            raise NotImplementedError('Conv1D(strides=%d) on %d input channels: the matrix-core kernels implement strides 1 and 2 '
                                      '(any stride >= 1 runs for <= 4 input channels)' % (self.stride, Cin))
        if not 1 <= self.k <= 40:
            raise NotImplementedError('Conv1D(kernel_size=%d): 1..40 taps (bbhMahoGANy.py:228 names 5 and 10)' % self.k)
        if self.phased:
            Lout = ops.conv_geometry(L, self.k, self.stride, self.padding, self.dilation)[0]
            if Lout < 1:
                raise ValueError('Conv1D(kernel_size=%d, dilation_rate=%d, padding=%r) on an input of shape %r: the output would have %d rows'
                                 % (self.k, self.dilation, self.padding, tuple(input_shape), Lout))
        if self.stride > 2 and _ConvRun(self, Cin, False).fwd_any:
            raise NotImplementedError('Conv1D(%d filters, strides=%d) on %d input channels: strides above 2 run on the small-Cin kernels only, which '
                                      'need a multiple of 4 filters; the any-channel kernels implement strides 1 and 2'
                                      % (self.filters, self.stride, Cin))
        self.kernel = self.add_weight('kernel', glorot_uniform((self.k, Cin, self.filters)), regularizer=self.kernel_regularizer)
        self.bias = self.add_weight('bias', np.zeros(self.filters, np.float32), regularizer=self.bias_regularizer)

    def compute_output_shape(self, input_shape):
        return (ops.conv_geometry(input_shape[0], self.k, self.stride, self.padding, self.dilation)[0], self.filters)

    @property
    def can_fold_bn(self):
        return self.activation[0] == 'linear' and self.filters % 4 == 0 and self.filters > 4 and not self.phased

    def can_defer_dgrad(self, Cin):
        return (self.filters == 1 and self.stride == 1 and self.k <= 5 and Cin % 4 == 0 and not self.phased and not _is_softmax(self)
                and not _NO_LAZYGRAD)

    def can_fold_upsample(self):
        return self.k == 5 and self.padding == 'same' and self.stride in (1, 2) and not self.phased and not _NO_UPFOLD

    def _launch(self, run, x, w, b, launch):
        if run.up_folded:
            w, b = ops.conv1d_up2_fold(w, b, self.stride)
        return _kconv_fwd(x, w, b, run.stride, run.pl, run.Lout, launch)

    def forward(self, ctx, node, x):
        a = node.fused_act or self.activation
        B = x.shape[0]
        run = _ConvRun(self, x.shape[2], node.fold_up is not None, x.shape[1])
        if run.phase is not None:
            assert node.fused_drop is None and node.infer_bn is None and node.fold_up is None, 'a planner fusion on a dilated or causal Conv1D'
            d, pl, _, Lout = run.phase
            xs = ops.dilate_split(x, d, pl, run.L)
            (ys, _, _), xs, w = self._launch(run, xs, self.kernel.data, self.bias.data, lambda *conv: _conv_fwd(
                node, ctx, *conv, a, None, run.any_channels))
            y = ops.dilate_merge(ys, B, d, 0, Lout) if d > 1 else ys
            if a is _SOFTMAX:
                y = _channel_softmax(self, y)
            ctx.tape[node.index] = _ConvTape(xs, y, a, None, 0.0, w, run)
            return y
        bn_node = None if run.any_channels else node.infer_bn
        if not ctx.training and bn_node is not None and run.Cin > 4:
            bn = bn_node.layer
            scale, shift = ops.bn_infer_coeffs(bn.gamma.data, bn.beta.data, bn.moving_mean.data, bn.moving_variance.data, bn.epsilon)
            w, b = ops.conv_fold_bn(self.kernel.data, self.bias.data, scale, shift)
            act = bn_node.fused_act or ('linear', 0.0)
            ctx.skip.add(bn_node.index)
            return self._launch(run, x, w, b, lambda *conv: ops.conv1d_fwd(*conv, act[0], act[1]))[0].view(B, -1, self.filters)
        if ctx.training and bn_node is not None and run.Cin_run > 4 and run.Cout_run == self.filters and not _NO_CONVSTATS:
            (y, sums), x, w = self._launch(run, x, self.kernel.data, self.bias.data, ops.conv1d_fwd_stats)
            ctx.bn_sums[bn_node.index] = sums
            ctx.tape[node.index] = _ConvTape(x, y, a, None, 0.0, w, run)
            return y
        (y, mask, rate), x, w = self._launch(run, x, self.kernel.data, self.bias.data, lambda *conv: _conv_fwd(
            node, ctx, *conv, a, (B, run.Lout, run.Cout_run), run.any_channels, self.filters > 4))
        if a is _SOFTMAX:
            y = _channel_softmax(self, y)
        ctx.tape[node.index] = _ConvTape(x, y, a, mask, rate, w, run)
        y = y.view(B, -1, self.filters)
        if ctx.training and (_kernel_act(a)[0] != 'linear' or mask is not None):
            ctx.epi[node.index] = (y, a[0], a[1], None if mask is None else mask.view(y.shape), rate)
        return y

    def writes_dy(self, node):
        return _epilogue_writes_dy(self, node)

    def backward(self, ctx, node, dy, need_dx, need_dw, prev=None):
        t = ctx.tape.pop(node.index)
        run = t.run
        dy = _conv_bwd_epilogue(dy.contiguous().view(t.y.shape), t.y, t.act, t.mask, t.rate, ctx, node)
        if run.phase is not None:
            d, pl, L, _ = run.phase
            dys = ops.dilate_split(dy, d, 0, run.Lout) if d > 1 else dy
            if need_dw:
                _kconv_wgrad(t.x, dys, run.k, run.stride, 0, self.kernel.grad, self.bias.grad, any_channels=run.any_channels, folded=True)
            if not need_dx:
                return None
            dxs = _kconv_dgrad(dys, t.w, run.k, run.L, run.stride, 0, None, run.any_channels, folded=True)
            return ops.dilate_merge(dxs, dy.shape[0], d, pl, L)
        if need_dw:
            if run.up_folded:
                dwf, dbf = _kconv_wgrad(t.x, dy, run.k, run.stride, run.pl, any_channels=run.any_channels)
                ops.conv1d_up2_unfold_grad(dwf, dbf, self.filters, self.stride, self.kernel.grad, self.bias.grad)
            else:
                _kconv_wgrad(t.x, dy, run.k, run.stride, run.pl, self.kernel.grad, self.bias.grad, any_channels=run.any_channels, folded=True)
        if not need_dx:
            return None
        if prev is not None and not run.tap_folded and ops.can_fuse_dgrad(run.Cin_run, run.Cout_run):
            ctx.pre_applied.add(node.fuse_prev)
        else:
            prev = None
        if node.lazy_bn >= 0:
            return ops.ConvGrad1(dy, self.kernel.data, run.L, run.pl)
        return _kconv_dgrad(dy, t.w, run.k, run.L, run.stride, run.pl, prev, run.any_channels, folded=True)


class Conv2D(Layer):
    fusable_act = True
    can_absorb_prev_act_bwd = True

    @property
    def fusable_drop(self):
        return not _is_softmax(self) and self.filters > 2

    @property
    def offers_act_bwd(self):
        return not _is_softmax(self)

    def __init__(self, filters, kernel_size, strides=(1, 1), padding='valid', activation=None, kernel_initializer='glorot_uniform', use_bias=True,
                 kernel_regularizer=None, bias_regularizer=None, activity_regularizer=None, **kw):
        Layer.__init__(self, **kw)
        _check_init(kernel_initializer)
        _take_regularizers(self, kernel_regularizer, bias_regularizer, activity_regularizer)
        self.filters = int(filters)
        self.kh, self.kw = (kernel_size, kernel_size) if isinstance(kernel_size, int) else tuple(kernel_size)
        self.sh, self.sw = (strides, strides) if isinstance(strides, int) else tuple(strides)
        self.padding = padding
        self.activation = _act_spec(activation, 'Conv2D')
        if self.kw != 5 or self.sw != 1 or padding != 'same' or not use_bias:
            raise NotImplementedError('Conv2D is implemented for the hot-path case only: kernel (kh,5), strides (sh,1), padding "same", width-2 input')

    def build(self, input_shape):
        H, W, Cin = input_shape
        if W != 2:
            raise NotImplementedError('Conv2D is implemented for width-2 images (got width %d)' % W)
        if ops.conv_layer_needs_any(2 * Cin, 2 * self.filters):
            raise NotImplementedError('Conv2D(%d filters) on %d input channels: the width-2 layer runs as a %d -> %d channel Conv1D, and the conv '
                                      'kernels it uses need both counts multiples of 4, or one of them <= 4 and the other a multiple of 4'
                                      % (self.filters, Cin, 2 * Cin, 2 * self.filters))
        self.kernel = self.add_weight('kernel', glorot_uniform((self.kh, self.kw, Cin, self.filters)), regularizer=self.kernel_regularizer)
        self.bias = self.add_weight('bias', np.zeros(self.filters, np.float32), regularizer=self.bias_regularizer)

    def compute_output_shape(self, input_shape):
        return (ops.conv_geometry(input_shape[0], self.kh, self.sh, 'same')[0], 2, self.filters)

    def forward(self, ctx, node, x):
        a = node.fused_act or self.activation
        B, H, W, Cin = x.shape
        Lout, pl = ops.conv_geometry(H, self.kh, self.sh, 'same')
        wf, bf = ops.conv2d_w2_fold(self.kernel.data, self.bias.data)
        xf = x.reshape(B, H, 2 * Cin)
        y, mask, rate = _conv_fwd(node, ctx, xf, wf, bf, self.sh, pl, Lout, a, (B, Lout, 2, self.filters))
        if a is _SOFTMAX:
            y = _channel_softmax(self, y)
        ctx.tape[node.index] = _ConvTape(xf, y, a, mask, rate, wf, pl=pl, in_shape=x.shape)
        if ctx.training and (_kernel_act(a)[0] != 'linear' or mask is not None):
            ctx.epi[node.index] = (y, a[0], a[1], mask, rate)
        return y.reshape(B, Lout, 2, self.filters)

    def writes_dy(self, node):
        return _epilogue_writes_dy(self, node)

    def backward(self, ctx, node, dy, need_dx, need_dw, prev=None):
        t = ctx.tape.pop(node.index)
        Cin = t.in_shape[3]
        dy = _conv_bwd_epilogue(dy.contiguous().reshape(t.y.shape), t.y, t.act, t.mask, t.rate, ctx, node)
        if need_dw:
            dwf, dbf = ops.conv1d_wgrad(t.x, dy, self.kh, self.sh, t.pl)
            ops.conv2d_w2_unfold_grad(dwf, dbf, Cin, self.filters, self.kernel.grad, self.bias.grad)
        if need_dx:
            if prev is not None and ops.can_fuse_dgrad(2 * Cin, 2 * self.filters):
                ctx.pre_applied.add(node.fuse_prev)
            else:
                prev = None
            return ops.conv1d_dgrad(dy, ops.conv1d_transpose_w(t.w), t.x.shape[1], self.sh, t.pl, prev).reshape(t.in_shape)
        return None


def _pair(v, what):
    t = (v, v) if isinstance(v, int) else tuple(int(u) for u in v)
    if len(t) != 2:
        raise ValueError('Conv2DTranspose: %s %r is not a pair' % (what, v))
    return t


class Conv2DTranspose(Layer):
    fusable_act = True

    @property
    def fusable_drop(self):
        return not _is_softmax(self)

    def __init__(self, filters, kernel_size, strides=(1, 1), padding='valid', output_padding=None, data_format=None, dilation_rate=(1, 1),
                 activation=None, use_bias=True, kernel_initializer='glorot_uniform', kernel_regularizer=None, bias_regularizer=None,
                 activity_regularizer=None, **kw):
        Layer.__init__(self, **kw)
        _check_init(kernel_initializer)
        _take_regularizers(self, kernel_regularizer, bias_regularizer, activity_regularizer)
        self.filters = int(filters)
        kh, self.k = _pair(kernel_size, 'kernel_size')
        sh, self.stride = _pair(strides, 'strides')
        supported = ('Conv2DTranspose is implemented for kernel (1, kw) with 1 <= kw <= 40, strides (1, 1) or (1, 2), padding "valid" or "same", '
                     'dilation (1, 1), no output_padding, use_bias=True, channels_last')
        if kh != 1 or sh != 1 or self.stride not in (1, 2) or not 1 <= self.k <= 40:
            raise NotImplementedError('%s (got kernel_size %r, strides %r)' % (supported, kernel_size, strides))
        if _pair(dilation_rate, 'dilation_rate') != (1, 1) or output_padding is not None or not use_bias:
            raise NotImplementedError('%s (got dilation_rate %r, output_padding %r, use_bias %r)' % (supported, dilation_rate, output_padding, use_bias))
        if data_format not in (None, 'channels_last'):
            raise NotImplementedError('%s (got data_format %r)' % (supported, data_format))
        if padding not in ('same', 'valid'):
            raise NotImplementedError('%s (got padding %r)' % (supported, padding))
        if self.k < self.stride:
            raise NotImplementedError('Conv2DTranspose(kernel (1, %d), strides (1, %d)): every stride phase needs a tap (kw >= s)' % (self.k, self.stride))
        self.padding = padding
        self.activation = _act_spec(activation, 'Conv2DTranspose')

    def build(self, input_shape):
        if len(input_shape) != 3:
            raise ValueError('Conv2DTranspose expects (batch, H, W, channels) inputs, got %r' % (tuple(input_shape),))
        if not _transpose_pair_ok(self.k, self.filters, input_shape[2]):
            raise NotImplementedError('Conv2DTranspose(%d filters, kernel (1, %d)) on %d input channels: the conv kernels need both channel counts '
                                      'multiples of 4, or one of them <= 4 and the other a multiple of 4' % (self.filters, self.k, input_shape[2]))
        self.kernel = self.add_weight('kernel', glorot_uniform((1, self.k, self.filters, input_shape[2])), regularizer=self.kernel_regularizer)
        self.bias = self.add_weight('bias', np.zeros(self.filters, np.float32), regularizer=self.bias_regularizer)

    def out_length(self, W):
        return W * self.stride + max(self.k - self.stride, 0) if self.padding == 'valid' else W * self.stride

    def compute_output_shape(self, input_shape):
        return (input_shape[0], self.out_length(input_shape[1]), self.filters)

    def forward(self, ctx, node, x):
        a = node.fused_act or self.activation
        B, H, W, Cin = x.shape
        Wout = self.out_length(W)
        pl = ops.conv_geometry(Wout, self.k, self.stride, self.padding)[1]
        x3 = x.contiguous().view(B * H, W, Cin)
        wadj = self.kernel.data.view(self.k, self.filters, Cin)
        y = _kconv_dgrad(x3, wadj, self.k, Wout, self.stride, pl)
        mask, rate = None, 0.0
        soft, a = a is _SOFTMAX, _kernel_act(a)
        if ctx.training and node.fused_drop is not None and node.fused_drop[0] > 0.0:
            rate, drop_layer = node.fused_drop
            if ctx.dropout_masks.get(drop_layer.name) is None and ctx.row_map is None:
                mask = torch.empty(y.shape, dtype=torch.uint8, device=y.device)
                ops.bias_act_dropout(y, self.bias.data, a[0], a[1], mask, rate, gen=device_rng().take(y.numel()))
            else:
                mask = drop_layer.make_mask(ctx, (B, H, Wout, self.filters)).view(y.shape)
                ops.bias_act_dropout(y, self.bias.data, a[0], a[1], mask, rate)
        else:
            ops.bias_act_dropout(y, self.bias.data, a[0], a[1])
        if soft:
            y, a = _channel_softmax(self, y), _SOFTMAX
        ctx.tape[node.index] = _ConvTape(x3, y, a, mask, rate, wadj, pl=pl, in_shape=x.shape)
        y = y.view(B, H, Wout, self.filters)
        if ctx.training and (_kernel_act(a)[0] != 'linear' or mask is not None):
            ctx.epi[node.index] = (y, a[0], a[1], None if mask is None else mask.view(y.shape), rate)
        return y

    def writes_dy(self, node):
        return _epilogue_writes_dy(self, node)

    def backward(self, ctx, node, dy, need_dx, need_dw, prev=None):
        t = ctx.tape.pop(node.index)
        dy = _conv_bwd_epilogue(dy.contiguous().view(t.y.shape), t.y, t.act, t.mask, t.rate, ctx, node)
        if need_dw:
            ops.bias_grad(dy.view(-1, self.filters), self.bias.grad)
            _kconv_wgrad(dy, t.x, self.k, self.stride, t.pl, self.kernel.grad.view(t.w.shape), want_db=False)
        if not need_dx:
            return None
        return _kconv_fwd(dy, t.w, None, self.stride, t.pl, t.x.shape[1])[0].view(t.in_shape)


BN_MOVING_AVERAGE = 'tf_zero_debias'


class BatchNormalization(Layer):
    def __init__(self, axis=-1, momentum=0.99, epsilon=1e-3, moving_average=None, beta_regularizer=None, gamma_regularizer=None, **kw):
        Layer.__init__(self, **kw)
        self.beta_regularizer, self.gamma_regularizer = regularizers.get(beta_regularizer), regularizers.get(gamma_regularizer)
        if isinstance(axis, bool) or not isinstance(axis, (int, np.integer)):
            raise NotImplementedError('BatchNormalization(axis=%r): one integer axis' % (axis,))
        self.axis = int(axis)
        self.view = None
        self.momentum, self.epsilon = float(momentum), float(epsilon)
        self.moving_average = moving_average or BN_MOVING_AVERAGE
        if self.moving_average not in ('tf_zero_debias', 'ema'):
            raise ValueError("BatchNormalization(moving_average=%r): 'tf_zero_debias' or 'ema'" % (moving_average,))
        self.zero_debias = {}

    def zero_debias_state(self, site):
        st = self.zero_debias.get(site)
        if st is None:
            C = self.gamma.shape[0]
            st = [torch.zeros(C, dtype=torch.float32, device=device()), torch.zeros(C, dtype=torch.float32, device=device()), 0]
            self.zero_debias[site] = st
        return st

    def build(self, input_shape):
        n = len(input_shape) + 1
        if not (1 <= self.axis <= n - 1 or -(n - 1) <= self.axis <= -1):
            raise ValueError('BatchNormalization(axis=%d) on inputs of shape %r: the axis must be one of 1..%d or -1..-%d'
                             % (self.axis, (None,) + tuple(input_shape), n - 1, n - 1))
        k = (self.axis if self.axis > 0 else self.axis + n) - 1
        C = int(input_shape[k])
        self.view = (int(np.prod(input_shape[:k], dtype=np.int64)), C, int(np.prod(input_shape[k + 1:], dtype=np.int64)))
        self._last_axis = k == len(input_shape) - 1
        self.gamma = self.add_weight('gamma', np.ones(C, np.float32), regularizer=self.gamma_regularizer)
        self.beta = self.add_weight('beta', np.zeros(C, np.float32), regularizer=self.beta_regularizer)
        self.moving_mean = self.add_weight('moving_mean', np.zeros(C, np.float32), trainable=False)
        self.moving_variance = self.add_weight('moving_variance', np.ones(C, np.float32), trainable=False)

    @property
    def is_batchnorm(self):
        return self._last_axis if self.view is not None else self.axis == -1

    fusable_act = fusable_drop = is_batchnorm

    def _train_coeffs(self, ctx, sums, count):
        if ctx.dp is not None:
            ctx.dp.all_reduce_sum(sums)
            count *= ctx.dp.world_size
        zd = None
        if self.moving_average == 'tf_zero_debias':
            st = self.zero_debias_state(ctx.site)
            cap = capturing()
            if cap is None:
                st[2] += 1
                zd = (st[0], st[1], st[2])
            else:

                def next_step(st=st):
                    st[2] += 1
                    return st[2]
                zd = (st[0], st[1], cap.slot('i', next_step))
        return ops.bn_finalize(sums, count, self.gamma.data, self.beta.data, self.epsilon, self.momentum,
                               self.moving_mean.data, self.moving_variance.data, zd) + (count,)

    def _param_grads(self, need_dw):
        if need_dw:
            return self.gamma.grad, self.beta.grad
        return torch.empty_like(self.gamma.data), torch.empty_like(self.beta.data)

    def forward(self, ctx, node, x):
        if not self.is_batchnorm:
            return self._forward_axis(ctx, node, x)
        if node.index in ctx.skip:
            return x
        C = x.shape[-1]
        x2 = x.reshape(-1, C)
        act = node.fused_act or ('linear', 0.0)
        if not ctx.training:
            scale, shift = ops.bn_infer_coeffs(self.gamma.data, self.beta.data, self.moving_mean.data, self.moving_variance.data, self.epsilon)
            return ops.bn_apply(x2, scale, shift, None, act[0], act[1]).reshape(x.shape)
        sums = ctx.bn_sums.pop(node.index, None)
        if sums is None:
            sums = ops.bn_stats(x2)
        scale, shift, smean, sinv, count = self._train_coeffs(ctx, sums, x2.shape[0])
        mask, rate = None, 0.0
        if node.fused_drop is not None and node.fused_drop[0] > 0.0:
            rate, drop_layer = node.fused_drop
            if ctx.dropout_masks.get(drop_layer.name) is None and C % 4 == 0 and not _NO_DROPGEN and (ctx.row_map is None or len(ctx.row_map[0]) == 1):
                if ctx.row_map is None:
                    seed, off = device_rng().take(x2.numel())
                else:
                    (g0, nrows), grows = ctx.row_map[0][0], ctx.row_map[1]
                    seed, offs = device_rng().take_rows(x2.numel() // nrows, [(g0, nrows)], grows)
                    off = offs[0]
                y, mask = ops.bn_apply_dropgen(x2, scale, shift, act[0], act[1], rate, seed, off)
                ctx.tape[node.index] = (x2, mask, smean, sinv, count, act, rate, scale, shift)
                return y.reshape(x.shape)
            mask = drop_layer.make_mask(ctx, x2.shape)
        y = ops.bn_apply(x2, scale, shift, mask, act[0], act[1], rate)
        ctx.tape[node.index] = (x2, mask, smean, sinv, count, act, rate, scale, shift)
        return y.reshape(x.shape)

    def backward(self, ctx, node, dy, need_dx, need_dw):
        if not self.is_batchnorm:
            return self._backward_axis(ctx, node, dy, need_dw)
        x2, mask, smean, sinv, count, act, rate, scale, shift = ctx.tape.pop(node.index)
        y = None
        lazy = isinstance(dy, ops.ConvGrad1)
        if lazy:
            local = ops.bn_bwd_stats_conv1(dy, x2, mask, smean, sinv, act[0], act[1], rate, scale, shift)
        else:
            dy2 = dy.contiguous().reshape(x2.shape)
            local = ops.bn_bwd_stats(dy2, y, x2, mask, smean, sinv, act[0], act[1], rate, scale, shift)
        glob = local
        if ctx.dp is not None:
            glob = local.clone()
            ctx.dp.all_reduce_sum(glob)
        dgamma, dbeta = self._param_grads(need_dw)
        if lazy:
            dx = ops.bn_bwd_apply_conv1(dy, x2, mask, self.gamma.data, smean, sinv, glob, count, local, dgamma, dbeta, act[0], act[1], rate, scale, shift)
        else:
            dx = ops.bn_bwd_apply(dy2, y, x2, mask, self.gamma.data, smean, sinv, glob, count, local, dgamma, dbeta, act[0], act[1], rate, scale, shift)
        return dx.reshape(dy.shape)

    def _forward_axis(self, ctx, node, x):
        P, inner = self.view[1], self.view[2]
        xv = x.contiguous().reshape((-1, P) if inner == 1 else (-1, P, inner))
        apply_ = ops.bn_apply if inner == 1 else ops.bn_axis_apply
        if not ctx.training:
            scale, shift = ops.bn_infer_coeffs(self.gamma.data, self.beta.data, self.moving_mean.data, self.moving_variance.data, self.epsilon)
            return apply_(xv, scale, shift).reshape(x.shape)
        sums = ops.bn_stats(xv) if inner == 1 else ops.bn_axis_stats(xv)
        scale, shift, smean, sinv, count = self._train_coeffs(ctx, sums, xv.shape[0] * inner)
        ctx.tape[node.index] = (xv, smean, sinv, count, scale, shift)
        return apply_(xv, scale, shift).reshape(x.shape)

    def _backward_axis(self, ctx, node, dy, need_dw):
        xv, smean, sinv, count, scale, shift = ctx.tape.pop(node.index)
        dyv = dy.contiguous().reshape(xv.shape)
        if xv.dim() == 2:
            local = ops.bn_bwd_stats(dyv, None, xv, None, smean, sinv, scale=scale, shift=shift)
        else:
            local = ops.bn_axis_bwd_stats(dyv, xv, smean, sinv)
        glob = local
        if ctx.dp is not None:
            glob = local.clone()
            ctx.dp.all_reduce_sum(glob)
        dgamma, dbeta = self._param_grads(need_dw)
        if xv.dim() == 2:
            dx = ops.bn_bwd_apply(dyv, None, xv, None, self.gamma.data, smean, sinv, glob, count, local, dgamma, dbeta, scale=scale, shift=shift)
        else:
            dx = ops.bn_axis_bwd_apply(dyv, xv, self.gamma.data, smean, sinv, glob, count, local, dgamma, dbeta)
        return dx.reshape(dy.shape)


def _softmax_view(layer, axis, input_shape):
    n = len(input_shape) + 1
    what = '%s (%s)' % (layer.name, type(layer).__name__)
    if n == 1:
        raise ValueError('%s: Cannot apply softmax to a tensor that is 1D' % what)
    if axis == 0 or axis == -n:
        raise ValueError('%s: softmax over axis %d is the batch axis: it would normalise across the samples of a batch, and under data parallelism '
                         'across ranks; choose one of 1..%d or -1..-%d' % (what, axis, n - 1, n - 1))
    if not (1 <= axis <= n - 1 or -(n - 1) <= axis <= -1):
        raise ValueError('%s: softmax axis %d on inputs of shape %r: the axis must be one of 1..%d or -1..-%d'
                         % (what, axis, (None,) + tuple(input_shape), n - 1, n - 1))
    k = (axis if axis > 0 else axis + n) - 1
    return (int(np.prod(input_shape[:k], dtype=np.int64)), int(input_shape[k]), int(np.prod(input_shape[k + 1:], dtype=np.int64)))


class Softmax(Layer):

    def __init__(self, axis=-1, **kw):
        Layer.__init__(self, **kw)
        if isinstance(axis, bool) or not isinstance(axis, (int, np.integer)):
            raise ValueError('%s (Softmax): axis=%r is not one integer' % (self.name, axis))
        self.axis = int(axis)
        self.view = None

    def build(self, input_shape):
        self.view = _softmax_view(self, self.axis, input_shape)

    def compute_output_shape(self, input_shape):
        _softmax_view(self, self.axis, input_shape)
        return tuple(input_shape)

    def forward(self, ctx, node, x):
        per, P, inner = self.view
        view = (x.shape[0] * per, P, inner)
        y = ops.softmax_fwd(x.contiguous(), view)
        ctx.tape[node.index] = (y, view)
        return y

    def backward(self, ctx, node, dy, need_dx, need_dw):
        y, view = ctx.tape.pop(node.index)
        return ops.softmax_bwd(dy.contiguous(), y, view)


class Activation(Layer):

    def __init__(self, activation, **kw):
        Layer.__init__(self, **kw)
        spec = _act_spec(activation, 'Activation')
        self.softmax = spec is _SOFTMAX
        self.act_spec = None if self.softmax else spec
# ... 593 lines not shown
```

### gennet_amd/ops.py

```python
import ctypes
import functools

import torch

from . import _lib

ACT = _lib.enum_members('GN_ACT_')
ACT[None] = ACT['linear']

_ws = {}


def _stream():
    return torch.cuda.current_stream().cuda_stream


def _p(t):
    return None if t is None else t.data_ptr()


def _chk(*ts):
    for t in ts:
        if t is None:
            continue
# ... 108 lines not shown
def conv1d_fwd_dropout(x, w, b, mask, stride, pad_left, Lout, act, act_param, rate):
    _chk(x, w, b, mask)
    B, L, Cin = x.shape
    k, _, Cout = w.shape
    y = torch.empty((B, Lout, Cout), dtype=torch.float32, device=x.device)
    assert mask.numel() == y.numel()
    _lib.call('gn_conv1d_fwd_dropout', _p(x), _p(w), _p(b), _p(mask), _p(y), B, L, Cin, Cout, k, stride, pad_left, Lout, ACT[act], float(act_param),
              float(rate), _stream())
    return y


def act_dropout_bwd(dy, y, mask, act, act_param, rate, inplace=False):
    _chk(dy, y, mask)
    dx = dy if inplace else torch.empty_like(dy)
    _lib.call('gn_act_dropout_bwd', _p(dy), _p(y), _p(mask), _p(dx), dy.numel(), ACT[act], float(act_param), float(rate), _stream())
    return dx


def conv1d_transpose_w(w):
    _chk(w)
    k, Cin, Cout = w.shape
    wt = torch.empty((k, Cout, Cin), dtype=torch.float32, device=w.device)
    _lib.call('gn_conv1d_transpose_w', _p(w), _p(wt), k, Cin, Cout, _stream())
    return wt


def conv1d_dgrad(dy, wt, L, stride, pad_left, prev=None, any_channels=False):
    _chk(dy, wt)
    B, Lout, Cout = dy.shape
    k, _, Cin = wt.shape
    if any_channels and prev is not None:
        raise ValueError('conv1d_dgrad(any_channels=True) has no fused producer gradient')
    dx = torch.empty((B, L, Cin), dtype=torch.float32, device=dy.device)
    if prev is None:
        _lib.call('gn_conv1d_dgrad_any' if any_channels else 'gn_conv1d_dgrad', _p(dy), _p(wt), _p(dx), B, L, Cin, Cout, k, stride, pad_left, Lout, _stream())
    else:
        y_prev, act, param, mask, rate = prev
        _chk(y_prev, mask)
        assert y_prev.numel() == dx.numel()
        _lib.call('gn_conv1d_dgrad_fused', _p(dy), _p(wt), _p(dx), B, L, Cin, Cout, k, stride, pad_left, Lout, _p(y_prev), _p(mask), ACT[act], float(param),
                  float(rate), _stream())
    return dx


def can_fuse_dgrad(Cin, Cout):
    return Cin > 4 and Cout > 4 and not conv_needs_any(Cin, Cout)


def conv1d_wgrad(x, dy, k, stride, pad_left, dw=None, db=None, want_db=True, any_channels=False):
    _chk(x, dy, dw, db)
    B, L, Cin = x.shape
    _, Lout, Cout = dy.shape
    if dw is None:
        dw = torch.empty((k, Cin, Cout), dtype=torch.float32, device=x.device)
    if db is None and want_db:
        db = torch.empty((Cout,), dtype=torch.float32, device=x.device)
    nb = _lib.size('gn_conv1d_wgrad_workspace', B, L, Cin, Cout, k, stride, Lout)
    ws = workspace(nb, x.device)
    _lib.call('gn_conv1d_wgrad_any' if any_channels else 'gn_conv1d_wgrad', _p(x), _p(dy), _p(dw), _p(db), _p(ws), ws.numel(), B, L, Cin, Cout, k, stride, pad_left, Lout, _stream())
    return dw, db


def bias_act_dropout(y, b, act='linear', act_param=0.0, mask=None, rate=0.0, gen=None):
    _chk(y, b, mask)
    C = y.shape[-1]
    if mask is not None:
        assert mask.numel() == y.numel()
    seed, off = gen if gen is not None else (0, 0)
    _lib.call('gn_bias_act_dropout', _p(y), _p(b), _p(mask), y.numel() // C, C, ACT[act], float(act_param), float(rate), 1 if gen is not None else 0,
              int(seed), int(off), _stream())
    return y


def bias_grad(dy2d, db=None):
    _chk(dy2d, db)
    rows, C = dy2d.shape
    if db is None:
        db = torch.empty((C,), dtype=torch.float32, device=dy2d.device)
    ws = workspace(_lib.size('gn_bias_grad_workspace', rows, C), dy2d.device)
    _lib.call('gn_bias_grad', _p(dy2d), _p(db), _p(ws), ws.numel(), rows, C, _stream())
    return db


def conv2d_w2_fold(w, b):
    _chk(w, b)
    kh, kw, Cin, Cout = w.shape
    assert kw == 5
    wf = torch.empty((kh, 2 * Cin, 2 * Cout), dtype=torch.float32, device=w.device)
    bf = torch.empty((2 * Cout,), dtype=torch.float32, device=w.device)
    _lib.call('gn_conv2d_w2_fold', _p(w), _p(b), _p(wf), _p(bf), kh, Cin, Cout, _stream())
    return wf, bf


def conv2d_w2_unfold_grad(dwf, dbf, Cin, Cout, dw=None, db=None):
    _chk(dwf, dbf, dw, db)
    kh = dwf.shape[0]
    if dw is None:
        dw = torch.empty((kh, 5, Cin, Cout), dtype=torch.float32, device=dwf.device)
    if db is None:
        db = torch.empty((Cout,), dtype=torch.float32, device=dwf.device)
    _lib.call('gn_conv2d_w2_unfold_grad', _p(dwf), _p(dbf), _p(dw), _p(db), kh, Cin, Cout, _stream())
    return dw, db


def maxpool_h2_fwd(x):
    _chk(x)
    B, H = x.shape[0], x.shape[1]
    R = x.numel() // max(B * H, 1)
    y = torch.empty((B, H // 2) + tuple(x.shape[2:]), dtype=torch.float32, device=x.device)
    _lib.call('gn_maxpool_h2_fwd', _p(x), _p(y), B, H, R, _stream())
    return y


def maxpool_h2_bwd(dy, x):
    _chk(dy, x)
    B, H = x.shape[0], x.shape[1]
    R = x.numel() // max(B * H, 1)
    dx = torch.empty_like(x)
    _lib.call('gn_maxpool_h2_bwd', _p(dy), _p(x), _p(dx), B, H, R, _stream())
    return dx


POOL_MODES = _lib.enum_members('GN_POOL_')


def _pool_args(x_shape, pool, strides, padding):
    B, H, W, C = (int(v) for v in x_shape)
    (Ho, pt), (Wo, pl) = pool_geometry(H, pool[0], strides[0], padding), pool_geometry(W, pool[1], strides[1], padding)
    return B, H, W, C, int(pool[0]), int(pool[1]), int(strides[0]), int(strides[1]), pt, pl, Ho, Wo


def pool2d_fwd(mode, x, pool, strides, padding, out=None):
    _chk(x, out)
    B, H, W, C, ph, pw, sh, sw, pt, pl, Ho, Wo = _pool_args(x.shape, pool, strides, padding)
    y = torch.empty((B, Ho, Wo, C), dtype=torch.float32, device=x.device) if out is None else out
    assert tuple(y.shape) == (B, Ho, Wo, C)
    _lib.call('gn_pool2d_fwd', POOL_MODES[mode], _p(x), _p(y), B, H, W, C, ph, pw, sh, sw, pt, pl, Ho, Wo, _stream())
    return y


def pool2d_bwd(mode, dy, x, x_shape, pool, strides, padding, out=None):
    _chk(dy, x, out)
    B, H, W, C, ph, pw, sh, sw, pt, pl, Ho, Wo = _pool_args(x_shape, pool, strides, padding)
    assert tuple(dy.shape) == (B, Ho, Wo, C) and (x is None or tuple(x.shape) == (B, H, W, C))
    dx = torch.empty((B, H, W, C), dtype=torch.float32, device=dy.device) if out is None else out
    _lib.call('gn_pool2d_bwd', POOL_MODES[mode], _p(dy), _p(x), _p(dx), B, H, W, C, ph, pw, sh, sw, pt, pl, Ho, Wo, _stream())
    return dx


def _global_pool_ws(B, P, C, device):
    return workspace(_lib.size('gn_global_pool_workspace', B, P, C), device)


def global_pool_fwd(mode, x, out=None):
    _chk(x, out)
    B, P, C = (int(v) for v in x.shape)
    y = torch.empty((B, C), dtype=torch.float32, device=x.device) if out is None else out
    ws = _global_pool_ws(B, P, C, x.device)
    _lib.call('gn_global_pool_fwd', POOL_MODES[mode], _p(x), _p(y), _p(ws), ws.numel(), B, P, C, _stream())
    return y


def global_pool_bwd(mode, dy, x, y, x_shape, out=None):
    _chk(dy, x, y, out)
    B, P, C = (int(v) for v in x_shape)
    dx = torch.empty((B, P, C), dtype=torch.float32, device=dy.device) if out is None else out
    ws = _global_pool_ws(B, P, C, dy.device)
    _lib.call('gn_global_pool_bwd', POOL_MODES[mode], _p(dy), _p(x), _p(y), _p(dx), _p(ws), ws.numel(), B, P, C, _stream())
    return dx


@functools.lru_cache(maxsize=None)
def tap_groups(k):
    G, h = ctypes.c_int(), ctypes.c_int()
    _lib.call('gn_conv1d_tap_groups', k, ctypes.byref(G), ctypes.byref(h))
    return G.value, h.value


def conv1d_tapfold_x(x, k, pl):
    _chk(x)
    B, L, Cin = x.shape
    x2 = torch.empty((B, L + pl, tap_groups(k)[0] * Cin), dtype=torch.float32, device=x.device)
    _lib.call('gn_conv1d_tapfold_x', _p(x), _p(x2), B, L, Cin, k, pl, _stream())
    return x2


def conv1d_tapunfold_dx(dx2, L, k, pl):
    _chk(dx2)
    B, L2, C2 = dx2.shape
    G = tap_groups(k)[0]
    assert L2 == L + pl and C2 % G == 0
    dx = torch.empty((B, L, C2 // G), dtype=torch.float32, device=dx2.device)
    _lib.call('gn_conv1d_tapunfold_dx', _p(dx2), _p(dx), B, L, C2 // G, k, pl, _stream())
    return dx


def conv1d_tapfold_w(w):
    _chk(w)
    k, Cin, Cout = w.shape
    G, h = tap_groups(k)
    w2 = torch.empty((h, G * Cin, Cout), dtype=torch.float32, device=w.device)
    _lib.call('gn_conv1d_tapfold_w', _p(w), _p(w2), k, Cin, Cout, _stream())
    return w2


def conv1d_tapunfold_dw(dw2, k, dw=None):
    _chk(dw2, dw)
    h, C2, Cout = dw2.shape
    G, hh = tap_groups(k)
    assert h == hh and C2 % G == 0
    if dw is None:
        dw = torch.empty((k, C2 // G, Cout), dtype=torch.float32, device=dw2.device)
    _lib.call('gn_conv1d_tapunfold_dw', _p(dw2), _p(dw), k, C2 // G, Cout, _stream())
    return dw


def conv1d_up2_fold(w, b, stride):
    _chk(w, b)
    k, Cin, Cout = w.shape
    assert k == 5 and stride in (1, 2)
    Cf = Cout * (2 if stride == 1 else 1)
    wf = torch.empty((3, Cin, Cf), dtype=torch.float32, device=w.device)
    bf = torch.empty((Cf,), dtype=torch.float32, device=w.device)
    _lib.call('gn_conv1d_up2_fold', _p(w), _p(b), _p(wf), _p(bf), Cin, Cout, stride, _stream())
    return wf, bf


def conv1d_up2_unfold_grad(dwf, dbf, Cout, stride, dw=None, db=None):
    _chk(dwf, dbf, dw, db)
    Cin = dwf.shape[1]
    assert dwf.shape[0] == 3 and dwf.shape[2] == Cout * (2 if stride == 1 else 1)
    if dw is None:
        dw = torch.empty((5, Cin, Cout), dtype=torch.float32, device=dwf.device)
    if db is None:
        db = torch.empty((Cout,), dtype=torch.float32, device=dwf.device)
    _lib.call('gn_conv1d_up2_unfold_grad', _p(dwf), _p(dbf), _p(dw), _p(db), Cin, Cout, stride, _stream())
    return dw, db


def dense_fwd(x, w, b, act='linear', act_param=0.0):
    _chk(x, w, b)
    B, n_in = x.shape
    n_out = w.shape[1]
    y = torch.empty((B, n_out), dtype=torch.float32, device=x.device)
    _lib.call('gn_dense_fwd', _p(x), _p(w), _p(b), _p(y), B, n_in, n_out, ACT[act], float(act_param), _stream())
    return y


def dense_bwd(x, w, dy, need_dx=True, dw=None, db=None, prev=None):
    _chk(x, w, dy, dw, db)
    B, n_in = x.shape
    n_out = w.shape[1]
    dx = torch.empty_like(x) if need_dx else None
    if prev is not None:
        _, act, param, mask, rate = prev
        assert need_dx and n_out <= 4
        if dw is None:
            dw = torch.empty_like(w)
        if db is None:
            db = torch.empty((n_out,), dtype=torch.float32, device=x.device)
        _lib.call('gn_dense_bwd_fused', _p(x), _p(w), _p(dy), _p(dx), _p(dw), _p(db), B, n_in, n_out, _p(mask), ACT[act], float(param), float(rate), _stream())
        return dx, dw, db
    if dw is None:
        dw = torch.empty_like(w)
    if db is None:
        db = torch.empty((n_out,), dtype=torch.float32, device=x.device)
    nb = _lib.size('gn_dense_bwd_workspace', B, n_in, n_out)
    ws = workspace(nb, x.device)
    _lib.call('gn_dense_bwd', _p(x), _p(w), _p(dy), _p(dx), _p(dw), _p(db), _p(ws), ws.numel(), B, n_in, n_out, _stream())
    return dx, dw, db


def act_fwd(x, act, act_param=0.0):
    _chk(x)
    y = torch.empty_like(x)
    _lib.call('gn_act_fwd', _p(x), _p(y), x.numel(), ACT[act], float(act_param), _stream())
    return y


def act_bwd(dy, y, act, act_param=0.0, inplace=False):
    _chk(dy, y)
    dx = dy if inplace else torch.empty_like(dy)
    _lib.call('gn_act_bwd', _p(dy), _p(y), _p(dx), dy.numel(), ACT[act], float(act_param), _stream())
    return dx


def _softmax_view(t, view):
    outer, P, inner = (int(v) for v in view)
    if outer < 1 or P < 1 or inner < 1 or outer * P * inner != t.numel():
        raise ValueError('softmax: the (outer, P, inner) view %r does not cover a tensor of %d elements' % ((outer, P, inner), t.numel()))
    if P * inner >= 1 << 31:
        raise ValueError('softmax: P * inner = %d * %d does not fit the int parameters of the kernels (< 2^31)' % (P, inner))
    return outer, P, inner


def softmax_fwd(x, view, out=None, inplace=False):
    _chk(x, out)
    outer, P, inner = _softmax_view(x, view)
    y = x if inplace else torch.empty_like(x) if out is None else out
    _lib.call('gn_softmax_fwd', _p(x), _p(y), outer, P, inner, _stream())
    return y


def softmax_bwd(dy, y, view, out=None, inplace=False):
    _chk(dy, y, out)
    outer, P, inner = _softmax_view(dy, view)
    assert y.numel() == dy.numel()
    dx = dy if inplace else torch.empty_like(dy) if out is None else out
    _lib.call('gn_softmax_bwd', _p(dy), _p(y), _p(dx), outer, P, inner, _stream())
    return dx


def bmm(a, b, trans_a=False, trans_b=False, out=None, valu=False):
    _chk(a, b, out)
    if a.dim() != 3 or b.dim() != 3 or a.dtype != torch.float32 or b.dtype != torch.float32 or a.shape[0] != b.shape[0]:
        raise ValueError('bmm: float32 tensors (batch, ., .) of one batch size are expected, got %r and %r' % (tuple(a.shape), tuple(b.shape)))
    batch = a.shape[0]
    K, M = (a.shape[1], a.shape[2]) if trans_a else (a.shape[2], a.shape[1])
    Kb, N = (b.shape[2], b.shape[1]) if trans_b else (b.shape[1], b.shape[2])
    if K != Kb:
        raise ValueError('bmm: the contracted extents differ, %d and %d (a %r%s, b %r%s)'
                         % (K, Kb, tuple(a.shape), '^T' if trans_a else '', tuple(b.shape), '^T' if trans_b else ''))
    c = torch.empty((batch, M, N), dtype=torch.float32, device=a.device) if out is None else out
    assert c.numel() == batch * M * N
    a_m, a_k = (1, M) if trans_a else (K, 1)
    b_k, b_n = (1, K) if trans_b else (N, 1)
    _lib.call('gn_bmm_valu' if valu else 'gn_bmm', _p(a), _p(b), _p(c), batch, M, N, K, M * K, a_m, a_k, K * N, b_k, b_n, _stream())
    return c


def _l2norm_view(t, view):
    outer, P, inner = (int(v) for v in view)
    if outer < 0 or P < 1 or inner < 1 or outer * P * inner != t.numel():
        raise ValueError('l2norm: the (outer, P, inner) view %r does not cover a tensor of %d elements' % ((outer, P, inner), t.numel()))
    return outer, P, inner


def l2norm_fwd(x, view):
    _chk(x)
    outer, P, inner = _l2norm_view(x, view)
    y = torch.empty_like(x)
    inv = torch.empty((outer, inner), dtype=torch.float32, device=x.device)
    _lib.call('gn_l2norm_fwd', _p(x), _p(y), _p(inv), outer, P, inner, _stream())
    return y, inv


def l2norm_bwd(dy, y, inv, view, out=None):
    _chk(dy, y, inv, out)
    outer, P, inner = _l2norm_view(dy, view)
# ... 594 lines not shown
    xs = torch.empty((B * d, M, C), dtype=torch.float32, device=x.device) if out is None else out
    assert tuple(xs.shape) == (B * d, M, C)
    _lib.call('gn_dilate_split', _p(x), _p(xs), B, L, C, d, off, M, _stream())
    return xs


def dilate_merge(xs, B, d, off, L, out=None):
    _chk(xs, out)
    Bd, M, C = (int(v) for v in xs.shape)
    B, d, off, L = int(B), int(d), int(off), int(L)
    if B < 1 or d < 1 or L < 1 or Bd != B * d:
        raise ValueError('dilate_merge: %d phase sequences are not B = %d times d = %d (L = %d)' % (Bd, B, d, L))
    x = torch.empty((B, L, C), dtype=torch.float32, device=xs.device) if out is None else out
    assert tuple(x.shape) == (B, L, C)
    _lib.call('gn_dilate_merge', _p(xs), _p(x), B, L, C, d, off, M, _stream())
    return x


def bn_stats(x2d):
    _chk(x2d)
    rows, Cc = x2d.shape
    sums = torch.empty((2 * Cc,), dtype=torch.float64, device=x2d.device)
    nb = _lib.size('gn_bn_stats_workspace', rows, Cc)
    ws = workspace(nb, x2d.device)
    _lib.call('gn_bn_stats', _p(x2d), rows, Cc, _p(sums), _p(ws), ws.numel(), _stream())
    return sums


def bn_finalize(sums, count, gamma, beta, eps, momentum, moving_mean, moving_var, zero_debias=None):
    Cc = gamma.numel()
    dev = gamma.device
    scale, shift, smean, sinv = (torch.empty((Cc,), dtype=torch.float32, device=dev) for _ in range(4))
    if zero_debias is not None:
        bm, bv, step = zero_debias
        if isinstance(step, DevScalar):
            _lib.call('gn_bn_finalize_zero_debias_dyn', _p(sums), float(count), _p(gamma), _p(beta), float(eps), float(momentum), _p(moving_mean), _p(moving_var),
                      _p(bm), _p(bv), step.ptr, _p(scale), _p(shift), _p(smean), _p(sinv), Cc, _stream())
        else:
            _lib.call('gn_bn_finalize_zero_debias', _p(sums), float(count), _p(gamma), _p(beta), float(eps), float(momentum), _p(moving_mean), _p(moving_var),
                      _p(bm), _p(bv), int(step), _p(scale), _p(shift), _p(smean), _p(sinv), Cc, _stream())
    else:
        _lib.call('gn_bn_finalize', _p(sums), float(count), _p(gamma), _p(beta), float(eps), float(momentum), _p(moving_mean), _p(moving_var),
                  _p(scale), _p(shift), _p(smean), _p(sinv), Cc, _stream())
    return scale, shift, smean, sinv


def bn_infer_coeffs(gamma, beta, moving_mean, moving_var, eps):
    Cc = gamma.numel()
    scale, shift = (torch.empty((Cc,), dtype=torch.float32, device=gamma.device) for _ in range(2))
    _lib.call('gn_bn_infer_coeffs', _p(gamma), _p(beta), _p(moving_mean), _p(moving_var), float(eps), _p(scale), _p(shift), Cc, _stream())
    return scale, shift


def bn_apply(x2d, scale, shift, mask=None, act='linear', act_param=0.0, rate=0.0):
    _chk(x2d, mask)
    rows, Cc = x2d.shape
    y = torch.empty_like(x2d)
    _lib.call('gn_bn_apply', _p(x2d), _p(scale), _p(shift), _p(mask), _p(y), rows, Cc, ACT[act], float(act_param), float(rate), _stream())
    return y


def bn_apply_dropgen(x2d, scale, shift, act, act_param, rate, seed, offset):
    _chk(x2d)
    rows, Cc = x2d.shape
    y = torch.empty_like(x2d)
    mask = torch.empty((rows, Cc), dtype=torch.uint8, device=x2d.device)
    _lib.call('gn_bn_apply_dropgen', _p(x2d), _p(scale), _p(shift), _p(mask), _p(y), rows, Cc, ACT[act], float(act_param), float(rate), int(seed), int(offset),
              _stream())
    return y, mask


def bn_bwd_stats(dy2d, y2d, x2d, mask, smean, sinv, act='linear', act_param=0.0, rate=0.0, scale=None, shift=None):
    _chk(dy2d, y2d, x2d, mask)
    rows, Cc = x2d.shape
    dsums = torch.empty((2 * Cc,), dtype=torch.float64, device=x2d.device)
    nb = _lib.size('gn_bn_stats_workspace', rows, Cc)
    ws = workspace(nb, x2d.device)
    _lib.call('gn_bn_bwd_stats', _p(dy2d), _p(y2d), _p(x2d), _p(mask), _p(smean), _p(sinv), _p(dsums), _p(ws), ws.numel(), rows, Cc,
              ACT[act], float(act_param), float(rate), _p(scale), _p(shift), _stream())
    return dsums


def bn_bwd_apply(dy2d, y2d, x2d, mask, gamma, smean, sinv, dsums_global, count, dsums_local, dgamma, dbeta, act='linear', act_param=0.0, rate=0.0,
                 scale=None, shift=None):
    rows, Cc = x2d.shape
    dx = torch.empty_like(x2d)
    _lib.call('gn_bn_bwd_apply', _p(dy2d), _p(y2d), _p(x2d), _p(mask), _p(gamma), _p(smean), _p(sinv), _p(dsums_global), float(count),
              _p(dsums_local), _p(dx), _p(dgamma), _p(dbeta), rows, Cc, ACT[act], float(act_param), float(rate), _p(scale), _p(shift), _stream())
    return dx


def _axis_ws(x3d):
    outer, P, inner = x3d.shape
    return workspace(_lib.size('gn_bn_axis_stats_workspace', outer, P, inner), x3d.device)


def bn_axis_stats(x3d):
    _chk(x3d)
    outer, P, inner = x3d.shape
    sums = torch.empty((2 * P,), dtype=torch.float64, device=x3d.device)
    ws = _axis_ws(x3d)
    _lib.call('gn_bn_axis_stats', _p(x3d), outer, P, inner, _p(sums), _p(ws), ws.numel(), _stream())
    return sums


def bn_axis_apply(x3d, scale, shift):
    _chk(x3d)
    outer, P, inner = x3d.shape
    y = torch.empty_like(x3d)
    _lib.call('gn_bn_axis_apply', _p(x3d), _p(scale), _p(shift), _p(y), outer, P, inner, _stream())
    return y


def bn_axis_bwd_stats(dy3d, x3d, smean, sinv):
    _chk(dy3d, x3d)
    outer, P, inner = x3d.shape
    dsums = torch.empty((2 * P,), dtype=torch.float64, device=x3d.device)
    ws = _axis_ws(x3d)
    _lib.call('gn_bn_axis_bwd_stats', _p(dy3d), _p(x3d), _p(smean), _p(sinv), _p(dsums), _p(ws), ws.numel(), outer, P, inner, _stream())
    return dsums


def bn_axis_bwd_apply(dy3d, x3d, gamma, smean, sinv, dsums_global, count, dsums_local, dgamma, dbeta):
    _chk(dy3d, x3d)
    outer, P, inner = x3d.shape
    dx = torch.empty_like(x3d)
    ws = _axis_ws(x3d)
    _lib.call('gn_bn_axis_bwd_apply', _p(dy3d), _p(x3d), _p(gamma), _p(smean), _p(sinv), _p(dsums_global), float(count), _p(dsums_local), _p(dx),
              _p(dgamma), _p(dbeta), _p(ws), ws.numel(), outer, P, inner, _stream())
    return dx


class ConvGrad1(object):

    def __init__(self, g, w, L, pad_left):
        _chk(g, w)
        self.g, self.w, self.L, self.pad_left = g, w, int(L), int(pad_left)
        self.B, self.Lout = int(g.shape[0]), int(g.shape[1])
        self.k, self.C = int(w.shape[0]), int(w.shape[1])
        self.shape = (self.B, self.L, self.C)


def bn_bwd_stats_conv1(cg, x2d, mask, smean, sinv, act, act_param, rate, scale, shift):
    _chk(x2d, mask)
    rows, Cc = x2d.shape
    assert rows == cg.B * cg.L and Cc == cg.C
    dsums = torch.empty((2 * Cc,), dtype=torch.float64, device=x2d.device)
    ws = workspace(_lib.size('gn_bn_stats_workspace', rows, Cc), x2d.device)
    _lib.call('gn_bn_bwd_stats_conv1', _p(cg.g), _p(cg.w), cg.L, cg.Lout, cg.k, cg.pad_left, _p(x2d), _p(mask), _p(smean), _p(sinv), _p(dsums), _p(ws),
              ws.numel(), rows, Cc, ACT[act], float(act_param), float(rate), _p(scale), _p(shift), _stream())
    return dsums


def bn_bwd_apply_conv1(cg, x2d, mask, gamma, smean, sinv, dsums_global, count, dsums_local, dgamma, dbeta, act, act_param, rate, scale, shift):
    rows, Cc = x2d.shape
    dx = torch.empty_like(x2d)
    _lib.call('gn_bn_bwd_apply_conv1', _p(cg.g), _p(cg.w), cg.L, cg.Lout, cg.k, cg.pad_left, _p(x2d), _p(mask), _p(gamma), _p(smean), _p(sinv),
              _p(dsums_global), float(count), _p(dsums_local), _p(dx), _p(dgamma), _p(dbeta), rows, Cc, ACT[act], float(act_param), float(rate),
              _p(scale), _p(shift), _stream())
    return dx


def loss(kind, p, y, Bglobal=None):
    _chk(p, y)
    B = p.shape[0]
    dp = torch.empty_like(p)
    out = torch.empty((2,), dtype=torch.float32, device=p.device)
    fn = {'binary_crossentropy': 'gn_bce_loss', 'mean_squared_error': 'gn_mse_loss'}[kind]
    _lib.call(fn, _p(p), _p(y), _p(dp), _p(out), B, int(Bglobal or B), _stream())
    return dp, out


LOSS_KINDS = _lib.enum_members('GN_LOSS_')
del LOSS_KINDS['kinds']
LOSS_ALIASES = {'mse': 'mean_squared_error', 'mae': 'mean_absolute_error', 'mape': 'mean_absolute_percentage_error',
                'msle': 'mean_squared_logarithmic_error', 'kld': 'kullback_leibler_divergence', 'cosine': 'cosine_proximity'}
LOSS_PASS_MIN_ELEMENTS = 131072


def loss_pass(kind, p, y, denom=None, grad=True, dp=None):
    _chk(p, y, dp)
    rows, cols = p.shape
    if grad and dp is None:
        dp = torch.empty_like(p)
    out = torch.empty((2,), dtype=torch.float32, device=p.device)
    ws = workspace(_lib.size('gn_loss_pass_workspace', rows, cols), p.device)
    _lib.call('gn_loss_pass', LOSS_KINDS.get(kind, kind), _p(p), _p(y), _p(dp) if grad else None, _p(out), rows, cols, float(rows if denom is None else denom),
              _p(ws), ws.numel(), _stream())
    return (dp if grad else None), out


def weight_count(w, count=None):
    _chk(w, count)
    if count is None:
        count = torch.empty((1,), dtype=torch.float64, device=w.device)
    ws = workspace(_lib.size('gn_weight_count_workspace', w.numel()), w.device)
    _lib.call('gn_weight_count', _p(w), w.numel(), _p(count), _p(ws), ws.numel(), _stream())
    return count


def loss_pass_weighted(kind, p, y, w, count, grad=True, dp=None):
    _chk(p, y, w, count, dp)
    rows, cols = p.shape
    if w.numel() != rows or w.dtype != torch.float32:
        raise ValueError('loss_pass_weighted: %d float32 weights expected, got %s %s' % (rows, tuple(w.shape), w.dtype))
    if count.numel() != 1 or count.dtype != torch.float64:
        raise ValueError('loss_pass_weighted: count is one float64 value on the device')
    if grad and dp is None:
        dp = torch.empty_like(p)
    out = torch.empty((3,), dtype=torch.float32, device=p.device)
    ws = workspace(_lib.size('gn_loss_pass_weighted_workspace', rows, cols), p.device)
    _lib.call('gn_loss_pass_weighted', LOSS_KINDS.get(kind, kind), _p(p), _p(y), _p(w), _p(count), _p(dp) if grad else None, _p(out), rows, cols,
              _p(ws), ws.numel(), _stream())
    return (dp if grad else None), out


def adam_step(p, g, m, v, lr_t, b1, b2, eps):
    _chk(p, g, m, v)
    if isinstance(lr_t, DevScalar):
        _lib.call('gn_adam_step_dyn', _p(p), _p(g), _p(m), _p(v), p.numel(), lr_t.ptr, float(b1), float(b2), float(eps), _stream())
    else:
        _lib.call('gn_adam_step', _p(p), _p(g), _p(m), _p(v), p.numel(), float(lr_t), float(b1), float(b2), float(eps), _stream())


OPT_RULES = _lib.enum_members('GN_OPT_')


def optim_step(rule, p, g, states, lr, h0=0.0, h1=0.0, eps=0.0, nesterov=False, clip_scale=None, clipvalue=0.0):
    _chk(p, g, *states)
    st = [_p(s) for s in states] + [None] * (3 - len(states))
    dyn = isinstance(lr, DevScalar)
    _lib.call('gn_optim_step', OPT_RULES[rule], _p(p), _p(g), st[0], st[1], st[2], p.numel(), 0.0 if dyn else float(lr), lr.ptr if dyn else None,
              float(h0), float(h1), float(eps), 1 if nesterov else 0, None if clip_scale is None else _p(clip_scale), float(clipvalue), _stream())


def optim_sumsq_slots(n):
    return _lib.size('gn_optim_sumsq_slots', int(n))


# ... 68 lines not shown
```

### include/gennet_hip.h

```cpp
#ifndef GENNET_HIP_H
#define GENNET_HIP_H

#include <stddef.h>
#include <stdint.h>

#ifdef __cplusplus
extern "C" {
#endif

#define GN_OK 0
#define GN_EINVAL (-1)
#define GN_ELAUNCH (-2)
#define GN_EWORKSPACE (-3)

enum gn_act { GN_ACT_LINEAR = 0, GN_ACT_RELU = 1, GN_ACT_RELU_MAX = 2, GN_ACT_LEAKY = 3, GN_ACT_TANH = 4, GN_ACT_SIGMOID = 5 };

const char* gn_last_error(void);
int gn_version(void);

int gn_conv1d_fwd(const float* x, const float* w, const float* bias, float* y,
                  int B, int L, int Cin, int Cout, int k, int stride, int pad_left, int Lout,
                  int act, float act_param, void* stream);

size_t gn_conv1d_bf16x3_workspace(int B, int L, int Cin, int Cout, int k);
int gn_conv1d_fwd_bf16x3(const float* x, const float* w, const float* bias, float* y, void* ws, size_t ws_bytes,
                         int B, int L, int Cin, int Cout, int k, int stride, int pad_left, int Lout,
                         int act, float act_param, int resplit, void* stream);
size_t gn_conv1d_wino_workspace(int Cin, int Cout);
int gn_conv1d_fwd_wino(const float* x, const float* w, const float* bias, float* y, void* ws, size_t ws_bytes,
                       int B, int L, int Cin, int Cout, int k, int stride, int pad_left, int Lout,
                       int act, float act_param, void* stream);
int gn_set_conv_math(int mode, void* workspace, size_t workspace_bytes);

int gn_conv1d_fwd_dropout(const float* x, const float* w, const float* bias, const uint8_t* mask, float* y,
                          int B, int L, int Cin, int Cout, int k, int stride, int pad_left, int Lout,
                          int act, float act_param, float rate, void* stream);
size_t gn_conv1d_fwd_stats_workspace(int B, int Lout, int Cout);
int gn_conv1d_fwd_stats(const float* x, const float* w, const float* bias, float* y, double* sums, void* ws, size_t ws_bytes,
                        int B, int L, int Cin, int Cout, int k, int stride, int pad_left, int Lout, void* stream);

int gn_conv1d_transpose_w(const float* w, float* wt, int k, int Cin, int Cout, void* stream);

int gn_conv1d_dgrad(const float* dy, const float* wt, float* dx,
                    int B, int L, int Cin, int Cout, int k, int stride, int pad_left, int Lout, void* stream);

int gn_conv1d_dgrad_fused(const float* dy, const float* wt, float* dx,
                          int B, int L, int Cin, int Cout, int k, int stride, int pad_left, int Lout,
                          const float* y_prev, const uint8_t* mask_prev, int act_prev, float act_param_prev, float rate_prev, void* stream);

size_t gn_conv1d_wgrad_workspace(int B, int L, int Cin, int Cout, int k, int stride, int Lout);
int gn_conv1d_wgrad(const float* x, const float* dy, float* dw, float* db, void* ws, size_t ws_bytes,
                    int B, int L, int Cin, int Cout, int k, int stride, int pad_left, int Lout, void* stream);

int gn_conv1d_needs_any(int Cin, int Cout);
int gn_conv1d_fwd_any(const float* x, const float* w, const float* bias, float* y,
                      int B, int L, int Cin, int Cout, int k, int stride, int pad_left, int Lout,
                      int act, float act_param, void* stream);
int gn_conv1d_dgrad_any(const float* dy, const float* wt, float* dx,
                        int B, int L, int Cin, int Cout, int k, int stride, int pad_left, int Lout, void* stream);
int gn_conv1d_wgrad_any(const float* x, const float* dy, float* dw, float* db, void* ws, size_t ws_bytes,
                        int B, int L, int Cin, int Cout, int k, int stride, int pad_left, int Lout, void* stream);

int gn_conv2d_w2_fold(const float* w, const float* bias, float* wf, float* biasf, int kh, int Cin, int Cout, void* stream);
int gn_conv2d_w2_unfold_grad(const float* dwf, const float* dbf, float* dw, float* db, int kh, int Cin, int Cout, void* stream);
int gn_conv1d_tap_groups(int k, int* groups, int* taps);
int gn_conv1d_tapfold_x(const float* x, float* x2, int B, int L, int Cin, int k, int pad_left, void* stream);
int gn_conv1d_tapunfold_dx(const float* dx2, float* dx, int B, int L, int Cin, int k, int pad_left, void* stream);
int gn_conv1d_tapfold_w(const float* w, float* w2, int k, int Cin, int Cout, void* stream);
int gn_conv1d_tapunfold_dw(const float* dw2, float* dw, int k, int Cin, int Cout, void* stream);

int gn_conv1d_up2_fold(const float* w, const float* bias, float* wf, float* biasf, int Cin, int Cout, int stride, void* stream);
int gn_conv1d_up2_unfold_grad(const float* dwf, const float* dbf, float* dw, float* db, int Cin, int Cout, int stride, void* stream);

int gn_dense_fwd(const float* x, const float* w, const float* bias, float* y, int B, int in, int out,
                 int act, float act_param, void* stream);
size_t gn_dense_bwd_workspace(int B, int in, int out);
int gn_dense_bwd(const float* x, const float* w, const float* dy, float* dx, float* dw, float* db,
                 void* ws, size_t ws_bytes, int B, int in, int out, void* stream);

int gn_dense_bwd_fused(const float* x, const float* w, const float* dy, float* dx, float* dw, float* db, int B, int in, int out,
                       const uint8_t* mask_prev, int act_prev, float act_param_prev, float rate_prev, void* stream);

int gn_act_fwd(const float* x, float* y, size_t n, int act, float act_param, void* stream);
int gn_act_bwd(const float* dy, const float* y, float* dx, size_t n, int act, float act_param, void* stream);
int gn_act_dropout_bwd(const float* dy, const float* y, const uint8_t* mask, float* dx, size_t n, int act, float act_param, float rate, void* stream);
int gn_bn_apply_dropgen(const float* x, const float* scale, const float* shift, uint8_t* mask_out, float* y, size_t rows, int C,
                        int act, float act_param, float rate, uint64_t seed, uint64_t offset, void* stream);
int gn_bias_act_dropout(float* y, const float* bias, uint8_t* mask, size_t rows, int C, int act, float act_param, float rate, int gen,
                        uint64_t seed, uint64_t offset, void* stream);
size_t gn_bias_grad_workspace(size_t rows, int C);
int gn_bias_grad(const float* dy, float* db, void* ws, size_t ws_bytes, size_t rows, int C, void* stream);
int gn_conv_fold_bn(const float* w, const float* bias, const float* scale, const float* shift, float* w_out, float* bias_out,
                    size_t rows, int Cout, void* stream);
int gn_prelu_fwd(const float* x, const float* alpha, float* y, int B, size_t F, void* stream);
int gn_prelu_bwd(const float* dy, const float* x, const float* alpha, float* dx, float* dalpha, int B, size_t F, void* stream);
int gn_dropout_mask(uint8_t* mask, size_t n, float rate, uint64_t seed, uint64_t offset, void* stream);
int gn_dropout_apply(const float* x, const uint8_t* mask, float* y, size_t n, float rate, void* stream);
int gn_upsample2_fwd(const float* x, float* y, int B, int L, int C, void* stream);
int gn_upsample2_bwd(const float* dy, float* dx, int B, int L, int C, void* stream);
int gn_maxpool_h2_fwd(const float* x, float* y, int B, int H, int R, void* stream);
int gn_maxpool_h2_bwd(const float* dy, const float* x, float* dx, int B, int H, int R, void* stream);
enum gn_pool { GN_POOL_MAX = 0, GN_POOL_AVG = 1 };
int gn_pool2d_fwd(int mode, const float* x, float* y, int B, int H, int W, int C, int ph, int pw, int sh, int sw,
                  int pad_top, int pad_left, int Ho, int Wo, void* stream);
int gn_pool2d_bwd(int mode, const float* dy, const float* x, float* dx, int B, int H, int W, int C, int ph, int pw, int sh, int sw,
                  int pad_top, int pad_left, int Ho, int Wo, void* stream);
size_t gn_global_pool_workspace(int B, int P, int C);
int gn_global_pool_fwd(int mode, const float* x, float* y, void* ws, size_t ws_bytes, int B, int P, int C, void* stream);
int gn_global_pool_bwd(int mode, const float* dy, const float* x, const float* y, float* dx, void* ws, size_t ws_bytes, int B, int P, int C,
                       void* stream);
int gn_subtract_stack_fwd(const float* x, const float* event, float* img, int B, int n, void* stream);
int gn_subtract_stack_bwd(const float* dimg, float* dx, int B, int n, void* stream);
int gn_affine_stack_fwd(const float* x, const float* b0, const float* b1, float a0, float a1, float* img, int B, int n, void* stream);
int gn_affine_stack_bwd(const float* dimg, float a0, float a1, float* dx, int B, int n, void* stream);
int gn_assemble_d_batch(const float* real, const float* noise, const float* fake, const float* event, float* sX, int B, int n, void* stream);
int gn_fill_uniform(float* out, size_t n, float lo, float hi, uint64_t seed, uint64_t offset, void* stream);
int gn_fill_normal(float* out, size_t n, float mean, float std, uint64_t seed, uint64_t offset, void* stream);
int gn_gaussian_noise_fwd(const float* x, float* y, size_t n, float stddev, uint64_t seed, uint64_t offset, void* stream);
int gn_gaussian_dropout_apply(const float* x, float* y, size_t n, float sd, uint64_t seed, uint64_t offset, void* stream);
int gn_alpha_dropout_fwd(const float* x, float* y, size_t n, float rate, float a, float b, float alpha_p, uint64_t seed, uint64_t offset, void* stream);
int gn_alpha_dropout_bwd(const float* dy, float* dx, size_t n, float rate, float a, uint64_t seed, uint64_t offset, void* stream);
int gn_gather_rows(const float* src, const int64_t* idx, float* out, int rows, int width, void* stream);
int gn_axpy(float* y, const float* x, float a, size_t n, void* stream);

#define GN_MERGE_MAX_INPUTS 8
enum gn_merge { GN_MERGE_ADD = 0, GN_MERGE_SUB = 1, GN_MERGE_MUL = 2, GN_MERGE_AVG = 3, GN_MERGE_MAX = 4, GN_MERGE_MIN = 5 };
int gn_merge_fwd(int mode, const float* const* xs_host, int n_inputs, float* y, size_t n, void* stream);
int gn_merge_bwd(int mode, const float* dy, const float* const* xs_host, int n_inputs, int which, float* dx, size_t n, void* stream);
int gn_scale(const float* x, float a, float* y, size_t n, void* stream);
int gn_concat_fwd(const float* const* xs_host, const int* widths_host, int n_inputs, float* y, size_t outer, void* stream);
int gn_concat_bwd(const float* dy, float* const* dxs_host, const int* widths_host, int n_inputs, size_t outer, void* stream);

int gn_dilate_split(const float* x, float* xs, int B, int L, int C, int d, int off, int M, void* stream);
int gn_dilate_merge(const float* xs, float* x, int B, int L, int C, int d, int off, int M, void* stream);

size_t gn_bn_stats_workspace(size_t rows, int C);
int gn_bn_stats(const float* x, size_t rows, int C, double* sums, void* ws, size_t ws_bytes, void* stream);
int gn_bn_finalize(const double* sums, double count, const float* gamma, const float* beta, float eps, float momentum,
                   float* moving_mean, float* moving_var, float* scale, float* shift,
                   float* save_mean, float* save_invstd, int C, void* stream);
int gn_bn_finalize_zero_debias(const double* sums, double count, const float* gamma, const float* beta, float eps, float momentum,
                               float* moving_mean, float* moving_var, float* biased_mean, float* biased_var, int local_step,
                               float* scale, float* shift, float* save_mean, float* save_invstd, int C, void* stream);
int gn_bn_infer_coeffs(const float* gamma, const float* beta, const float* moving_mean, const float* moving_var,
                       float eps, float* scale, float* shift, int C, void* stream);
int gn_bn_apply(const float* x, const float* scale, const float* shift, const uint8_t* mask, float* y,
                size_t rows, int C, int act, float act_param, float rate, void* stream);
int gn_bn_bwd_stats(const float* dy, const float* y, const float* x, const uint8_t* mask,
                    const float* save_mean, const float* save_invstd, double* dsums, void* ws, size_t ws_bytes,
                    size_t rows, int C, int act, float act_param, float rate, const float* scale, const float* shift, void* stream);
int gn_bn_bwd_apply(const float* dy, const float* y, const float* x, const uint8_t* mask,
                    const float* gamma, const float* save_mean, const float* save_invstd,
                    const double* dsums_global, double count, const double* dsums_local, float* dx, float* dgamma, float* dbeta,
                    size_t rows, int C, int act, float act_param, float rate, const float* scale, const float* shift, void* stream);

int gn_bn_bwd_stats_conv1(const float* g, const float* w, int L, int Lout, int k, int pad_left, const float* x, const uint8_t* mask,
                          const float* save_mean, const float* save_invstd, double* dsums, void* ws, size_t ws_bytes, size_t rows, int C,
                          int act, float act_param, float rate, const float* scale, const float* shift, void* stream);
int gn_bn_bwd_apply_conv1(const float* g, const float* w, int L, int Lout, int k, int pad_left, const float* x, const uint8_t* mask,
                          const float* gamma, const float* save_mean, const float* save_invstd, const double* dsums_global, double count,
                          const double* dsums_local, float* dx, float* dgamma, float* dbeta, size_t rows, int C, int act, float act_param,
                          float rate, const float* scale, const float* shift, void* stream);

size_t gn_bn_axis_stats_workspace(size_t outer, int P, int inner);
int gn_bn_axis_stats(const float* x, size_t outer, int P, int inner, double* sums, void* ws, size_t ws_bytes, void* stream);
int gn_bn_axis_apply(const float* x, const float* scale, const float* shift, float* y, size_t outer, int P, int inner, void* stream);
int gn_bn_axis_bwd_stats(const float* dy, const float* x, const float* save_mean, const float* save_invstd, double* dsums, void* ws,
                         size_t ws_bytes, size_t outer, int P, int inner, void* stream);
int gn_bn_axis_bwd_apply(const float* dy, const float* x, const float* gamma, const float* save_mean, const float* save_invstd,
                         const double* dsums_global, double count, const double* dsums_local, float* dx, float* dgamma, float* dbeta,
                         void* ws, size_t ws_bytes, size_t outer, int P, int inner, void* stream);

int gn_softmax_fwd(const float* x, float* y, size_t outer, int P, int inner, void* stream);
int gn_softmax_bwd(const float* dy, const float* y, float* dx, size_t outer, int P, int inner, void* stream);

int gn_bmm(const float* a, const float* b, float* c, int batch, int M, int N, int K, long long a_batch, long long a_m, long long a_k,
           long long b_batch, long long b_k, long long b_n, void* stream);
int gn_bmm_valu(const float* a, const float* b, float* c, int batch, int M, int N, int K, long long a_batch, long long a_m, long long a_k,
                long long b_batch, long long b_k, long long b_n, void* stream);

int gn_l2norm_fwd(const float* x, float* y, float* inv, size_t outer, int P, int inner, void* stream);
int gn_l2norm_bwd(const float* dy, const float* y, const float* inv, float* dx, size_t outer, int P, int inner, void* stream);

enum gn_lstm_act { GN_LSTM_TANH = 0, GN_LSTM_SIGMOID = 1, GN_LSTM_RELU = 2, GN_LSTM_LINEAR = 3, GN_LSTM_HARD_SIGMOID = 4 };
size_t gn_lstm_fwd_workspace(int u);
size_t gn_lstm_bwd_workspace(int u);
int gn_lstm_fwd(const float* zx, const float* U, const float* bias, const float* h0, const float* c0, float* h, float* gates, float* c, float* hprev,
                void* ws, size_t ws_bytes, int B, int T, int u, int act, int ract, int reverse, int training, void* stream);
int gn_lstm_bwd(const float* dy, const float* gates, const float* c, const float* c0, const float* U, float* dz, float* dh0, float* dc0, void* ws,
                size_t ws_bytes, int B, int T, int u, int act, int ract, int reverse, int dy_seq, void* stream);

int gn_lstm_pair_fwd(const float* const* zx, const float* const* U, const float* const* bias, float* const* h, float* const* gates, float* const* c,
                     float* const* hprev, void* ws, size_t ws_bytes, int B, int T, int u, int ld, int act, int ract, int reverse0, int seq, int training,
                     void* stream);
int gn_lstm_pair_bwd(const float* const* dy, const float* const* gates, const float* const* c, const float* const* U, float* const* dz, void* ws,
                     size_t ws_bytes, int B, int T, int u, int ld, int act, int ract, int reverse0, int dy_seq, void* stream);

size_t gn_gru_fwd_workspace(int u);
size_t gn_gru_bwd_workspace(int u);
int gn_gru_fwd(const float* zx, const float* U, const float* bias, const float* rbias, const float* h0, float* h, float* gates, float* hprev, float* aux,
               void* ws, size_t ws_bytes, int B, int T, int u, int act, int ract, int reset_after, int reverse, int training, void* stream);
int gn_gru_bwd(const float* dy, const float* gates, const float* hprev, const float* aux, const float* U, float* dz, float* dzr, float* dh0, void* ws,
               size_t ws_bytes, int B, int T, int u, int act, int ract, int reset_after, int reverse, int dy_seq, void* stream);

int gn_gru_pair_fwd(const float* const* zx, const float* const* U, const float* const* bias, const float* const* rbias, float* const* h, float* const* gates,
                    float* const* hprev, float* const* aux, void* ws, size_t ws_bytes, int B, int T, int u, int ld, int act, int ract, int reset_after,
                    int reverse0, int seq, int training, void* stream);
int gn_gru_pair_bwd(const float* const* dy, const float* const* gates, const float* const* hprev, const float* const* aux, const float* const* U,
                    float* const* dz, float* const* dzr, void* ws, size_t ws_bytes, int B, int T, int u, int ld, int act, int ract, int reset_after,
                    int reverse0, int dy_seq, void* stream);

size_t gn_rnn_fwd_workspace(int u);
size_t gn_rnn_bwd_workspace(int u);
int gn_rnn_fwd(const float* zx, const float* U, const float* bias, const float* h0, float* h, float* hs, float* hprev, void* ws, size_t ws_bytes, int B,
               int T, int u, int act, int reverse, int training, void* stream);
int gn_rnn_bwd(const float* dy, const float* hs, const float* U, float* dz, float* dh0, void* ws, size_t ws_bytes, int B, int T, int u, int act,
               int reverse, int dy_seq, void* stream);

int gn_rnn_pair_fwd(const float* const* zx, const float* const* U, const float* const* bias, float* const* h, float* const* hs, float* const* hprev,
                    void* ws, size_t ws_bytes, int B, int T, int u, int ld, int act, int reverse0, int seq, int training, void* stream);
int gn_rnn_pair_bwd(const float* const* dy, const float* const* hs, const float* const* U, float* const* dz, void* ws, size_t ws_bytes, int B, int T,
                    int u, int ld, int act, int reverse0, int dy_seq, void* stream);

size_t gn_dwconv1d_wgrad_workspace(int B, int Lout, int C, int k, int dm);
int gn_dwconv1d_fwd(const float* x, const float* w, float* y, int B, int L, int C, int k, int dm, int stride, int dilation, int pad_left, int Lout,
                    void* stream);
int gn_dwconv1d_dgrad(const float* dy, const float* w, float* dx, int B, int L, int C, int k, int dm, int stride, int dilation, int pad_left, int Lout,
                      void* stream);
int gn_dwconv1d_wgrad(const float* x, const float* dy, float* dw, void* ws, size_t ws_bytes, int B, int L, int C, int k, int dm, int stride, int dilation,
                      int pad_left, int Lout, void* stream);

int gn_bce_loss(const float* p, const float* y, float* dp, float* out, int B, int Bglobal, void* stream);
int gn_mse_loss(const float* p, const float* y, float* dp, float* out, int B, int Bglobal, void* stream);

enum gn_loss {
  GN_LOSS_BINARY_CROSSENTROPY = 0, GN_LOSS_MEAN_SQUARED_ERROR = 1, GN_LOSS_MEAN_ABSOLUTE_ERROR = 2, GN_LOSS_MEAN_ABSOLUTE_PERCENTAGE_ERROR = 3,
  GN_LOSS_MEAN_SQUARED_LOGARITHMIC_ERROR = 4, GN_LOSS_HINGE = 5, GN_LOSS_SQUARED_HINGE = 6, GN_LOSS_LOGCOSH = 7, GN_LOSS_POISSON = 8,
  GN_LOSS_KULLBACK_LEIBLER_DIVERGENCE = 9, GN_LOSS_CATEGORICAL_CROSSENTROPY = 10, GN_LOSS_COSINE_PROXIMITY = 11,
  GN_LOSS_CATEGORICAL_ACCURACY = 12, GN_LOSS_KINDS = 13
};
size_t gn_loss_pass_workspace(long long rows, int cols);
int gn_loss_pass(int kind, const float* p, const float* y, float* dp, float* out, long long rows, int cols, double denom,
                 void* ws, size_t ws_bytes, void* stream);

size_t gn_weight_count_workspace(long long rows);
int gn_weight_count(const float* w, long long rows, double* count, void* ws, size_t ws_bytes, void* stream);
// ... 65 lines not shown
```

Measured before the change: 1945.

## Fuse downstream bias-gradient column sums into BN backward apply and dense backward

The BN backward apply kernel and the small-output dense backward kernel can now also accumulate per-channel column sums of the dx they produce. Partial sums are written to a workspace and finalized into the previous layer's bias gradient, so the separate bias_grad pass that re-read dx is no longer needed. The Python layers route the previous conv's db through these fused paths. The cost is extra double-precision accumulation, a shared-memory reduction and a finalize launch. When the fused path runs, the chunk geometry switches to colred_chunks, which may change occupancy.

```diff
diff --git a/gennet_amd/csrc/bn.hip b/gennet_amd/csrc/bn.hip
--- a/gennet_amd/csrc/bn.hip
+++ b/gennet_amd/csrc/bn.hip
@@ -1,3 +1,5 @@
+#include <atomic>
+
 #include "common.h"
 
 namespace gn {
@@ -336,7 +338,9 @@
   if ((int)threadIdx.x < n) o[threadIdx.x] = (float)a[threadIdx.x];
 }
 
+static std::atomic<size_t> g_bias_grad_passes{0};
 int bias_grad(const float* dy, float* db, size_t rows, int C, void* ws, size_t ws_bytes, hipStream_t s) {
+  g_bias_grad_passes.fetch_add(1, std::memory_order_relaxed);
   if (C % 4 == 0 || C > 4) {
     ColRedArgs r = {};
     r.a = dy; r.rows = rows; r.C = C;
@@ -448,11 +452,13 @@
     dx[i] = gamma[c] * inv * (g - mg - xh * mgx);
   }
 }
-__global__ __launch_bounds__(256) void bn_bwd_apply_v4_kernel(const float* __restrict__ dy, const float* __restrict__ y, const float* __restrict__ x,
-                                                              const uint8_t* __restrict__ mask, const float* __restrict__ gamma, const float* __restrict__ mean,
-                                                              const float* __restrict__ invstd, const double* __restrict__ dsums, double count,
-                                                              const float* __restrict__ scale, const float* __restrict__ shift, float* __restrict__ dx,
-                                                              size_t rows, int C, int rows_per_chunk, int act, float p, float keep_scale, LazyDy lz) {
+template <bool DB>
+__device__ __forceinline__ void bn_bwd_apply_v4_rows(const float* __restrict__ dy, const float* __restrict__ y, const float* __restrict__ x,
+                                                     const uint8_t* __restrict__ mask, const float* __restrict__ gamma, const float* __restrict__ mean,
+                                                     const float* __restrict__ invstd, const double* __restrict__ dsums, double count,
+                                                     const float* __restrict__ scale, const float* __restrict__ shift, float* __restrict__ dx,
+                                                     size_t rows, int C, int rows_per_chunk, int act, float p, float keep_scale, const LazyDy& lz,
+                                                     double (&ds)[4]) {
   const int NQ = C >> 2;
   const int NQc = NQ < 256 ? NQ : 256;
   const int RL = 256 / NQc;
@@ -519,6 +525,37 @@
         ov[e] = gi[e] * (g - mg[e] - xh * mgx[e]);
       }
       *reinterpret_cast<float4*>(dx + o) = make_float4(ov[0], ov[1], ov[2], ov[3]);
+      if (DB) {
+#pragma unroll
+        for (int e = 0; e < 4; ++e) ds[e] += (double)ov[e];
+      }
+    }
+  }
+}
+template <bool DB>
+__global__ __launch_bounds__(256) void bn_bwd_apply_v4_kernel(const float* __restrict__ dy, const float* __restrict__ y, const float* __restrict__ x,
+                                                              const uint8_t* __restrict__ mask, const float* __restrict__ gamma, const float* __restrict__ mean,
+                                                              const float* __restrict__ invstd, const double* __restrict__ dsums, double count,
+                                                              const float* __restrict__ scale, const float* __restrict__ shift, float* __restrict__ dx,
+                                                              size_t rows, int C, int rows_per_chunk, int act, float p, float keep_scale, LazyDy lz,
+                                                              double* __restrict__ part) {
+  double ds[4] = {0.0, 0.0, 0.0, 0.0};
+  bn_bwd_apply_v4_rows<DB>(dy, y, x, mask, gamma, mean, invstd, dsums, count, scale, shift, dx, rows, C, rows_per_chunk, act, p, keep_scale, lz, ds);
+  if (DB) {
+    const int NQ = C >> 2, NQc = NQ < 256 ? NQ : 256, RL = 256 / NQc, qblocks = (NQ + NQc - 1) / NQc;
+    const int tid = threadIdx.x, ql = tid % NQc, rl = tid / NQc, q = (blockIdx.x % qblocks) * NQc + ql;
+    __shared__ double red[256 * 4];
+#pragma unroll
+    for (int e = 0; e < 4; ++e) red[tid * 4 + e] = ds[e];
+    __syncthreads();
+    if (rl == 0 && q < NQ) {
+      double t[4] = {red[ql * 4], red[ql * 4 + 1], red[ql * 4 + 2], red[ql * 4 + 3]};
+      for (int k = 1; k < RL; ++k)
+#pragma unroll
+        for (int e = 0; e < 4; ++e) t[e] += red[(k * NQc + ql) * 4 + e];
+      double* d = part + (size_t)(blockIdx.x / qblocks) * C + 4 * q;
+#pragma unroll
+      for (int e = 0; e < 4; ++e) d[e] = t[e];
     }
   }
 }
@@ -528,24 +565,42 @@
   dbeta[c] = (float)dsums_local[c];
   dgamma[c] = (float)dsums_local[C + c];
 }
+static void bn_bwd_apply_geom(size_t rows, int C, size_t* chunks, size_t* rpc, int* qblocks) {
+  const int NQ = C / 4, NQc = NQ < 256 ? NQ : 256, RL = 256 / NQc;
+  *qblocks = cdiv(NQ, NQc);
+  size_t ch = 8192 / *qblocks;
+  if (ch < 1) ch = 1;
+  size_t r = (rows + ch - 1) / ch;
+  r = ((r + RL - 1) / RL) * RL;
+  if (r < (size_t)RL) r = RL;
+  *rpc = r;
+  *chunks = (rows + r - 1) / r;
+}
 static int bn_bwd_apply(const float* dy, const float* y, const float* x, const uint8_t* mask, const float* gamma, const float* mean, const float* invstd,
                  const double* dsums_global, double count, const double* dsums_local, float* dx, float* dgamma, float* dbeta, size_t rows, int C,
-                 int act, float p, float rate, const float* scale, const float* shift, hipStream_t s, const LazyDy* lz = nullptr) {
+                 int act, float p, float rate, const float* scale, const float* shift, hipStream_t s, const LazyDy* lz = nullptr, float* db = nullptr,
+                 void* ws = nullptr, size_t ws_bytes = 0) {
   const size_t n = rows * C;
+  if (db && (C % 4 || !n)) { set_error("bn_bwd_apply_db: the column sums of dx need C %% 4 == 0 and rows > 0 (C %d, rows %zu)", C, rows); return GN_EINVAL; }
   if (!n) return GN_OK;
   LazyDy z = {};
   if (lz) z = *lz;
   if (z.g && (C % 4 || !scale)) { set_error("bn_bwd_apply: the on-the-fly conv gradient needs C %% 4 == 0 and scale / shift"); return GN_EINVAL; }
+  size_t chunks = 0;
   if (C % 4 == 0) {
-    const int NQ = C / 4, NQc = NQ < 256 ? NQ : 256, RL = 256 / NQc, qblocks = cdiv(NQ, NQc);
-    size_t chunks = 8192 / qblocks;
-    if (chunks < 1) chunks = 1;
-    size_t rpc = (rows + chunks - 1) / chunks;
-    rpc = ((rpc + RL - 1) / RL) * RL;
-    if (rpc < (size_t)RL) rpc = RL;
-    chunks = (rows + rpc - 1) / rpc;
-    hipLaunchKernelGGL(bn_bwd_apply_v4_kernel, dim3((unsigned)(chunks * qblocks)), dim3(256), 0, s, dy, y, x, mask, gamma, mean, invstd, dsums_global, count, scale,
-                       shift, dx, rows, C, (int)rpc, act, p, 1.0f / (1.0f - rate), z);
+    size_t rpc;
+    int qblocks;
+    bn_bwd_apply_geom(rows, C, &chunks, &rpc, &qblocks);
+    if (db) {
+      chunks = (size_t)colred_chunks(rows, C);
+      rpc = (rows + chunks - 1) / chunks;
+      if (!ws || ((uintptr_t)ws & 7) || ws_bytes < chunks * C * sizeof(double)) { set_error("bn_bwd_apply_db: workspace missing, misaligned or too small"); return GN_EWORKSPACE; }
+      hipLaunchKernelGGL(bn_bwd_apply_v4_kernel<true>, dim3((unsigned)(chunks * qblocks)), dim3(256), 0, s, dy, y, x, mask, gamma, mean, invstd, dsums_global, count,
+                         scale, shift, dx, rows, C, (int)rpc, act, p, 1.0f / (1.0f - rate), z, (double*)ws);
+    } else {
+      hipLaunchKernelGGL(bn_bwd_apply_v4_kernel<false>, dim3((unsigned)(chunks * qblocks)), dim3(256), 0, s, dy, y, x, mask, gamma, mean, invstd, dsums_global, count,
+                         scale, shift, dx, rows, C, (int)rpc, act, p, 1.0f / (1.0f - rate), z, (double*)nullptr);
+    }
   } else {
     if (!y && !scale) { set_error("bn_bwd_apply: C %d %% 4 != 0 needs the stored layer output y or scale / shift", C); return GN_EINVAL; }
     hipLaunchKernelGGL(bn_bwd_apply_kernel, dim3(stream_grid(n)), dim3(256), 0, s, dy, y, x, mask, gamma, mean, invstd, dsums_global, count, dx, n, C, act, p,
@@ -553,6 +608,10 @@
   }
   int rc = check_launch("bn_bwd_apply");
   if (rc) return rc;
+  if (db) {
+    rc = colred_finalize_f32((const double*)ws, db, (size_t)C, (int)chunks, s);
+    if (rc) return rc;
+  }
   hipLaunchKernelGGL(bn_param_grads_kernel, dim3(cdiv(C, 256)), dim3(256), 0, s, dsums_local, dgamma, dbeta, C);
   return check_launch("bn_param_grads");
 }
@@ -672,7 +731,32 @@
                       mask ? rate : 0.f, scale, shift, (hipStream_t)stream, &z);
 }
 
+size_t gn_bn_bwd_apply_db_workspace(size_t rows, int C) {
+  if (C < 4 || C % 4 || !rows) return 0;
+  return (size_t)colred_chunks(rows, C) * C * sizeof(double) + 256;
+}
+int gn_bn_bwd_apply_db(const float* dy, const float* y, const float* x, const uint8_t* mask, const float* gamma, const float* save_mean, const float* save_invstd,
+                       const double* dsums_global, double count, const double* dsums_local, float* dx, float* dgamma, float* dbeta, size_t rows, int C, int act,
+                       float p, float rate, const float* scale, const float* shift, float* db, void* ws, size_t ws_bytes, void* stream) {
+  GN_REQUIRE(dy && x && gamma && save_mean && save_invstd && dsums_global && dsums_local && dx && dgamma && dbeta && db && C > 0, "bn_bwd_apply_db: bad arguments");
+  GN_REQUIRE((scale == nullptr) == (shift == nullptr) && (y || scale), "bn_bwd_apply_db: needs the layer output y, or scale AND shift to recompute it");
+  return bn_bwd_apply(dy, y, x, mask, gamma, save_mean, save_invstd, dsums_global, count, dsums_local, dx, dgamma, dbeta, rows, C, act, p, mask ? rate : 0.f, scale,
+                      shift, (hipStream_t)stream, nullptr, db, ws, ws_bytes);
+}
+int gn_bn_bwd_apply_conv1_db(const float* g, const float* w, int L, int Lout, int k, int pad_left, const float* x, const uint8_t* mask, const float* gamma,
+                             const float* save_mean, const float* save_invstd, const double* dsums_global, double count, const double* dsums_local, float* dx,
+                             float* dgamma, float* dbeta, size_t rows, int C, int act, float p, float rate, const float* scale, const float* shift, float* db,
+                             void* ws, size_t ws_bytes, void* stream) {
+  GN_REQUIRE(x && gamma && save_mean && save_invstd && dsums_global && dsums_local && dx && dgamma && dbeta && db && C > 0, "bn_bwd_apply_conv1_db: bad arguments");
+  LazyDy z = {};
+  int rc = lazy_dy_check("bn_bwd_apply_conv1_db", g, w, L, Lout, k, pad_left, rows, C, scale, shift, &z);
+  if (rc) return rc;
+  return bn_bwd_apply(nullptr, nullptr, x, mask, gamma, save_mean, save_invstd, dsums_global, count, dsums_local, dx, dgamma, dbeta, rows, C, act, p,
+                      mask ? rate : 0.f, scale, shift, (hipStream_t)stream, &z, db, ws, ws_bytes);
+}
+
 size_t gn_bias_grad_workspace(size_t rows, int C) { return bias_grad_ws(rows, C) + 256; }
+size_t gn_bias_grad_passes(void) { return g_bias_grad_passes.load(std::memory_order_relaxed); }
 
 int gn_bias_grad(const float* dy, float* db, void* ws, size_t ws_bytes, size_t rows, int C, void* stream) {
   GN_REQUIRE(dy && db && ws && rows > 0 && C > 0, "bias_grad: bad arguments");
diff --git a/gennet_amd/csrc/capi.hip b/gennet_amd/csrc/capi.hip
--- a/gennet_amd/csrc/capi.hip
+++ b/gennet_amd/csrc/capi.hip
@@ -499,6 +499,21 @@
   return dense_small_bwd(x, w, dy, dx, dw, db, B, in, out, (hipStream_t)stream, act_prev, act_param_prev, mask_prev, 1.0f / (1.0f - (mask_prev ? rate_prev : 0.f)));
 }
 
+size_t gn_dense_bwd_fused_db_workspace(int in) { return in > 0 ? (size_t)in * sizeof(double) + 256 : 0; }
+
+int gn_dense_bwd_fused_db(const float* x, const float* w, const float* dy, float* dx, float* dw, float* db, int B, int in, int out, const uint8_t* mask_prev,
+                          int act_prev, float act_param_prev, float rate_prev, float* db_prev, int C_prev, void* ws, size_t ws_bytes, void* stream) {
+  GN_REQUIRE(x && w && dy && dx && dw && db_prev && B > 0 && in > 0 && out >= 1 && out <= 4, "dense_bwd_fused_db: bad arguments (small-output heads only)");
+  GN_REQUIRE(rate_prev >= 0.f && rate_prev < 1.f, "dense_bwd_fused_db: bad rate");
+  GN_REQUIRE(C_prev > 0 && C_prev % 4 == 0 && in % C_prev == 0, "dense_bwd_fused_db: C_prev %d must be a multiple of 4 that divides in %d", C_prev, in);
+  GN_REQUIRE(ws && ((uintptr_t)ws & 7) == 0, "dense_bwd_fused_db: workspace missing or not 8-byte aligned");
+  if (int rc = ws_check("dense_bwd_fused_db", (size_t)in * sizeof(double), ws_bytes)) return rc;
+  hipStream_t s = (hipStream_t)stream;
+  int rc = dense_small_bwd(x, w, dy, dx, dw, db, B, in, out, s, act_prev, act_param_prev, mask_prev, 1.0f / (1.0f - (mask_prev ? rate_prev : 0.f)), (double*)ws);
+  if (rc) return rc;
+  return colred_finalize_f32((const double*)ws, db_prev, (size_t)C_prev, in / C_prev, s);
+}
+
 int gn_dense_bwd(const float* x, const float* w, const float* dy, float* dx, float* dw, float* db, void* ws, size_t ws_bytes, int B, int in, int out, void* stream) {
   GN_REQUIRE(x && w && dy && dw && B > 0 && in > 0 && out > 0, "dense_bwd: bad arguments");
   hipStream_t s = (hipStream_t)stream;
diff --git a/gennet_amd/csrc/common.h b/gennet_amd/csrc/common.h
--- a/gennet_amd/csrc/common.h
+++ b/gennet_amd/csrc/common.h
@@ -145,7 +145,7 @@
 int wgrad_small_dispatch(WgradSmallArgs a, float* dw, size_t ws_bytes, hipStream_t s);
 int dense_small_fwd(const float* x, const float* w, const float* bias, float* y, int B, int in, int out, int act, float p, hipStream_t s);
 int dense_small_bwd(const float* x, const float* w, const float* dy, float* dx, float* dw, float* db, int B, int in, int out, hipStream_t s,
-                    int gact = 0, float gparam = 0.f, const uint8_t* gmask = nullptr, float gscale = 1.f);
+                    int gact = 0, float gparam = 0.f, const uint8_t* gmask = nullptr, float gscale = 1.f, double* part = nullptr);
 size_t colred_workspace_bytes(size_t rows, int C);
 int colred_run(int mode, ColRedArgs a, void* ws, size_t ws_bytes, double* out_f64, float* out_f32, hipStream_t s);
 int colred_finalize(const double* part, double* out_f64, size_t n, int chunks, hipStream_t s);
diff --git a/gennet_amd/csrc/small_conv.hip b/gennet_amd/csrc/small_conv.hip
--- a/gennet_amd/csrc/small_conv.hip
+++ b/gennet_amd/csrc/small_conv.hip
@@ -616,13 +616,14 @@
   return check_launch("dense_small_fwd");
 }
 
-template <int OUT>
+template <int OUT, bool DB>
 __global__ __launch_bounds__(256) void dense_small_bwd_kernel(const float* __restrict__ x, const float* __restrict__ w, const float* __restrict__ dy,
                                                               float* __restrict__ dx, float* __restrict__ dw, int B, int in, int gact, float gparam,
-                                                              const uint8_t* __restrict__ gmask, float gscale) {
+                                                              const uint8_t* __restrict__ gmask, float gscale, double* __restrict__ part) {
   const size_t i = ((size_t)blockIdx.x * 256 + threadIdx.x) * 4;
   if (i >= (size_t)in) return;
   float wv[4][OUT], acc[4][OUT];
+  double ds[4] = {0.0, 0.0, 0.0, 0.0};
 #pragma unroll
   for (int e = 0; e < 4; ++e)
 #pragma unroll
@@ -664,6 +665,10 @@
         for (int e = 0; e < 4; ++e) d[e] = k[e] ? d[e] * gscale * act_grad_from_y(xs[e] / gscale, gact, gparam) : 0.f;
       }
       *reinterpret_cast<float4*>(dx + (size_t)b * in + i) = make_float4(d[0], d[1], d[2], d[3]);
+      if (DB) {
+#pragma unroll
+        for (int e = 0; e < 4; ++e) ds[e] += (double)d[e];
+      }
     }
     }
   }
@@ -671,6 +676,10 @@
   for (int e = 0; e < 4; ++e)
 #pragma unroll
     for (int o = 0; o < OUT; ++o) dw[(i + e) * OUT + o] = acc[e][o];
+  if (DB) {
+#pragma unroll
+    for (int e = 0; e < 4; ++e) part[i + e] = ds[e];
+  }
 }
 
 __global__ void colsum_small_kernel(const float* __restrict__ dy, float* __restrict__ db, int B, int out) {
@@ -681,19 +690,26 @@
   db[o] = s;
 }
 
+template <bool DB>
+static void dense_small_bwd_launch(const float* x, const float* w, const float* dy, float* dx, float* dw, int B, int in, int out, hipStream_t s, int gact,
+                                   float gparam, const uint8_t* gmask, float gscale, double* part) {
+  const unsigned grid = cdiv((size_t)in / 4, 256);
+  switch (out) {
+    case 1: hipLaunchKernelGGL((dense_small_bwd_kernel<1, DB>), dim3(grid), dim3(256), 0, s, x, w, dy, dx, dw, B, in, gact, gparam, gmask, gscale, part); break;
+    case 2: hipLaunchKernelGGL((dense_small_bwd_kernel<2, DB>), dim3(grid), dim3(256), 0, s, x, w, dy, dx, dw, B, in, gact, gparam, gmask, gscale, part); break;
+    case 3: hipLaunchKernelGGL((dense_small_bwd_kernel<3, DB>), dim3(grid), dim3(256), 0, s, x, w, dy, dx, dw, B, in, gact, gparam, gmask, gscale, part); break;
+    default: hipLaunchKernelGGL((dense_small_bwd_kernel<4, DB>), dim3(grid), dim3(256), 0, s, x, w, dy, dx, dw, B, in, gact, gparam, gmask, gscale, part); break;
+  }
+}
 int dense_small_bwd(const float* x, const float* w, const float* dy, float* dx, float* dw, float* db, int B, int in, int out, hipStream_t s, int gact,
-                    float gparam, const uint8_t* gmask, float gscale) {
+                    float gparam, const uint8_t* gmask, float gscale, double* part) {
   if (out < 1 || out > 4 || in % 4) {
     set_error("dense_small_bwd: out %d (1..4) / in %d (%%4) unsupported", out, in);
     return GN_EINVAL;
   }
-  const unsigned grid = cdiv((size_t)in / 4, 256);
-  switch (out) {
-    case 1: hipLaunchKernelGGL(dense_small_bwd_kernel<1>, dim3(grid), dim3(256), 0, s, x, w, dy, dx, dw, B, in, gact, gparam, gmask, gscale); break;
-    case 2: hipLaunchKernelGGL(dense_small_bwd_kernel<2>, dim3(grid), dim3(256), 0, s, x, w, dy, dx, dw, B, in, gact, gparam, gmask, gscale); break;
-    case 3: hipLaunchKernelGGL(dense_small_bwd_kernel<3>, dim3(grid), dim3(256), 0, s, x, w, dy, dx, dw, B, in, gact, gparam, gmask, gscale); break;
-    default: hipLaunchKernelGGL(dense_small_bwd_kernel<4>, dim3(grid), dim3(256), 0, s, x, w, dy, dx, dw, B, in, gact, gparam, gmask, gscale); break;
-  }
+  if (part && !dx) { set_error("dense_small_bwd: the sums of dx need dx"); return GN_EINVAL; }
+  if (part) dense_small_bwd_launch<true>(x, w, dy, dx, dw, B, in, out, s, gact, gparam, gmask, gscale, part);
+  else dense_small_bwd_launch<false>(x, w, dy, dx, dw, B, in, out, s, gact, gparam, gmask, gscale, nullptr);
   int rc = check_launch("dense_small_bwd");
   if (rc) return rc;
   if (db) {
diff --git a/gennet_amd/engine.py b/gennet_amd/engine.py
--- a/gennet_amd/engine.py
+++ b/gennet_amd/engine.py
@@ -262,6 +262,7 @@
         self.bn_sums = {}
         self.reg = None
         self.reg_y = {}
+        self.bias_sums = {}
 
     def wants_grad(self, layer):
         if self.train_ids is None:
@@ -397,6 +398,13 @@
     act_spec = None
     activity_regularizer = None
     drop_rate = None
+    sums_prev_bias = False
+
+    def takes_bias_sum(self, node, fused):
+        return False
+
+    def bias_sum_slot(self, ctx, node, fused):
+        return None
 
     def writes_dy(self, node):
         return False
@@ -415,7 +423,8 @@
 
 
 class Node(object):
-    __slots__ = ('layer', 'inbound', 'fused_act', 'fused_drop', 'absorbed', 'index', 'out_shape', 'owners', 'fuse_prev', 'infer_bn', 'fold_up', 'lazy_bn')
+    __slots__ = ('layer', 'inbound', 'fused_act', 'fused_drop', 'absorbed', 'index', 'out_shape', 'owners', 'fuse_prev', 'infer_bn', 'fold_up', 'lazy_bn',
+                 'bias_to')
 
     def __init__(self, layer, inbound, out_shape, owners=()):
         self.layer = layer
@@ -430,6 +439,7 @@
         self.fold_up = None
         self.infer_bn = None
         self.lazy_bn = -1
+        self.bias_to = None
 
 
 def _f32(x):
@@ -821,6 +831,7 @@
     def _plan(self):
         for n in self.nodes:
             n.fused_act, n.fused_drop, n.absorbed, n.fuse_prev, n.fold_up, n.infer_bn, n.lazy_bn = None, None, False, -1, None, None, -1
+            n.bias_to = None
         consumers = {n.index: [] for n in self.nodes}
         for n in self.nodes:
             for i in n.inbound:
@@ -888,6 +899,19 @@
             shp = self.nodes[cur].out_shape
             if len(shp) == 2 and n.layer.can_defer_dgrad(shp[1]):
                 n.lazy_bn = cur
+        for n in self.nodes:
+            if n.absorbed or len(n.inbound) != 1 or not n.layer.sums_prev_bias:
+                continue
+            cur = n.inbound[0] if getattr(n.layer, 'is_batchnorm', False) else n.fuse_prev
+            if cur < 0 or len(consumers[cur]) != 1 or cur in outs:
+                continue
+            own_act = getattr(self.nodes[cur].layer, 'activation', None)
+            epilogue = (self.nodes[cur].fused_act is not None and self.nodes[cur].fused_act[0] != 'linear') or self.nodes[cur].fused_drop is not None \
+                or (own_act is not None and own_act[0] != 'linear')
+            if epilogue != (cur == n.fuse_prev):
+                continue
+            if cur >= 0 and not self.nodes[cur].absorbed and not areg(self.nodes[cur]) and self.nodes[cur].layer.takes_bias_sum(self.nodes[cur], cur == n.fuse_prev):
+                n.bias_to = self.nodes[cur]
         self._planned = True
 
     def _forward(self, inputs, ctx):
diff --git a/gennet_amd/layers.py b/gennet_amd/layers.py
--- a/gennet_amd/layers.py
+++ b/gennet_amd/layers.py
@@ -11,6 +11,7 @@
 _NO_LAZYGRAD = bool(_os.environ.get('GN_NO_LAZYGRAD'))
 _NO_UPFOLD = bool(_os.environ.get('GN_NO_UPFOLD'))
 _NO_CONVSTATS = bool(_os.environ.get('GN_NO_CONVSTATS'))
+_BIAS_SUM_PASS = _os.environ.get('GENNET_BIAS_SUM') == 'pass'
 
 _ACT_NAMES = {'relu': ('relu', 0.0), 'tanh': ('tanh', 0.0), 'sigmoid': ('sigmoid', 0.0), 'linear': ('linear', 0.0), None: ('linear', 0.0)}
 _SOFTMAX = ('softmax', 0.0)
@@ -91,6 +92,20 @@
 def _epilogue_writes_dy(layer, node):
     a = node.fused_act or layer.activation
     return a[0] != 'linear' or node.fused_drop is not None
+
+
+def _bias_slot(ctx, node, fused=False):
+    p = node.bias_to
+    if p is None or _BIAS_SUM_PASS or ctx.row_map is not None or not ctx.training or not ctx.wants_grad(p.layer):
+        return None
+    slot = p.layer.bias_sum_slot(ctx, p, fused)
+    if slot is not None:
+        ctx.bias_sums[p.index] = slot
+    return slot
+
+
+def _linear_epilogue(t_act, mask):
+    return mask is None and t_act is not _SOFTMAX and _kernel_act(t_act)[0] == 'linear'
 
 
 def _kconv_fwd(x, w, b, stride, pl, Lout, launch=ops.conv1d_fwd):
@@ -159,6 +174,15 @@
         k = getattr(self, 'kernel', None)
         return self.units <= 4 and (k is None or k.shape[0] % 4 == 0)
 
+    sums_prev_bias = can_absorb_prev_act_bwd
+
+    def takes_bias_sum(self, node, fused):
+        return self.units % 4 == 0
+
+    def bias_sum_slot(self, ctx, node, fused):
+        x, y, a = ctx.tape[node.index]
+        return self.bias.grad if (fused and a is not _SOFTMAX) or _linear_epilogue(a, None) else None
+
     def __init__(self, units, activation=None, kernel_initializer='glorot_uniform', use_bias=True, kernel_regularizer=None, bias_regularizer=None,
                  activity_regularizer=None, **kw):
         Layer.__init__(self, **kw)
@@ -194,12 +218,20 @@
     def backward(self, ctx, node, dy, need_dx, need_dw, prev=None):
         x, y, a = ctx.tape.pop(node.index)
         dy = _conv_bwd_epilogue(dy.contiguous(), y, a, None, 0.0, ctx, node)
+        db_prev = None
         if prev is not None:
             ctx.pre_applied.add(node.fuse_prev)
+            slot = _bias_slot(ctx, node, fused=True)
+            if slot is not None and slot.numel() % 4 == 0 and x.shape[1] % slot.numel() == 0:
+                db_prev = (slot, slot.numel())
+            elif slot is not None:
+                del ctx.bias_sums[node.bias_to.index]
         if need_dw:
-            dx, _, _ = ops.dense_bwd(x, self.kernel.data, dy, need_dx, self.kernel.grad, self.bias.grad, prev=prev)
+            got = ctx.bias_sums.pop(node.index, None) is not None
+            dx, _, _ = ops.dense_bwd(x, self.kernel.data, dy, need_dx, self.kernel.grad, None if got else self.bias.grad, prev=prev, want_db=not got,
+                                     db_prev=db_prev)
             return dx
-        dx, _, _ = ops.dense_bwd(x, self.kernel.data, dy, True, prev=prev)
+        dx, _, _ = ops.dense_bwd(x, self.kernel.data, dy, True, prev=prev, db_prev=db_prev)
         return dx
 
 
@@ -288,6 +320,15 @@
 
     def can_fold_upsample(self):
         return self.k == 5 and self.padding == 'same' and self.stride in (1, 2) and not self.phased and not _NO_UPFOLD
+
+    def takes_bias_sum(self, node, fused):
+        return not self.phased and self.k <= 5 and self.filters % 4 == 0 and not (node.fold_up is not None and self.stride == 1)
+
+    def bias_sum_slot(self, ctx, node, fused):
+        t = ctx.tape[node.index]
+        if t.run.phase is not None or t.run.tap_folded or t.run.Cout_run != self.filters or t.act is _SOFTMAX or not (fused or _linear_epilogue(t.act, t.mask)):
+            return None
+        return self.bias.grad
 
     def _launch(self, run, x, w, b, launch):
         if run.up_folded:
@@ -348,12 +389,14 @@
                 return None
             dxs = _kconv_dgrad(dys, t.w, run.k, run.L, run.stride, 0, None, run.any_channels, folded=True)
             return ops.dilate_merge(dxs, dy.shape[0], d, pl, L)
+        got = ctx.bias_sums.pop(node.index, None) is not None
         if need_dw:
             if run.up_folded:
-                dwf, dbf = _kconv_wgrad(t.x, dy, run.k, run.stride, run.pl, any_channels=run.any_channels)
-                ops.conv1d_up2_unfold_grad(dwf, dbf, self.filters, self.stride, self.kernel.grad, self.bias.grad)
+                dwf, dbf = _kconv_wgrad(t.x, dy, run.k, run.stride, run.pl, want_db=not got, any_channels=run.any_channels)
+                ops.conv1d_up2_unfold_grad(dwf, dbf, self.filters, self.stride, self.kernel.grad, None if got else self.bias.grad, want_db=not got)
             else:
-                _kconv_wgrad(t.x, dy, run.k, run.stride, run.pl, self.kernel.grad, self.bias.grad, any_channels=run.any_channels, folded=True)
+                _kconv_wgrad(t.x, dy, run.k, run.stride, run.pl, self.kernel.grad, None if got else self.bias.grad, want_db=not got,
+                             any_channels=run.any_channels, folded=True)
         if not need_dx:
             return None
         if prev is not None and not run.tap_folded and ops.can_fuse_dgrad(run.Cin_run, run.Cout_run):
@@ -421,12 +464,25 @@
     def writes_dy(self, node):
         return _epilogue_writes_dy(self, node)
 
+    def takes_bias_sum(self, node, fused):
+        return fused and self.filters % 2 == 0
+
+    def bias_sum_slot(self, ctx, node, fused):
+        t = ctx.tape[node.index]
+        if t.act is _SOFTMAX or not (fused or _linear_epilogue(t.act, t.mask)):
+            return None
+        return torch.empty((2 * self.filters,), dtype=torch.float32, device=t.x.device)
+
     def backward(self, ctx, node, dy, need_dx, need_dw, prev=None):
         t = ctx.tape.pop(node.index)
         Cin = t.in_shape[3]
         dy = _conv_bwd_epilogue(dy.contiguous().reshape(t.y.shape), t.y, t.act, t.mask, t.rate, ctx, node)
+        dbf = ctx.bias_sums.pop(node.index, None)
         if need_dw:
-            dwf, dbf = ops.conv1d_wgrad(t.x, dy, self.kh, self.sh, t.pl)
+            if dbf is None:
+                dwf, dbf = ops.conv1d_wgrad(t.x, dy, self.kh, self.sh, t.pl)
+            else:
+                dwf, _ = ops.conv1d_wgrad(t.x, dy, self.kh, self.sh, t.pl, want_db=False)
             ops.conv2d_w2_unfold_grad(dwf, dbf, Cin, self.filters, self.kernel.grad, self.bias.grad)
         if need_dx:
             if prev is not None and ops.can_fuse_dgrad(2 * Cin, 2 * self.filters):
@@ -576,6 +632,7 @@
         return self._last_axis if self.view is not None else self.axis == -1
 
     fusable_act = fusable_drop = is_batchnorm
+    sums_prev_bias = is_batchnorm
 
     def _train_coeffs(self, ctx, sums, count):
         if ctx.dp is not None:
@@ -651,10 +708,14 @@
             glob = local.clone()
             ctx.dp.all_reduce_sum(glob)
         dgamma, dbeta = self._param_grads(need_dw)
+        db = _bias_slot(ctx, node) if x2.shape[1] % 4 == 0 else None
+        if db is not None and db.numel() != x2.shape[1]:
+            del ctx.bias_sums[node.bias_to.index]
+            db = None
         if lazy:
-            dx = ops.bn_bwd_apply_conv1(dy, x2, mask, self.gamma.data, smean, sinv, glob, count, local, dgamma, dbeta, act[0], act[1], rate, scale, shift)
+            dx = ops.bn_bwd_apply_conv1(dy, x2, mask, self.gamma.data, smean, sinv, glob, count, local, dgamma, dbeta, act[0], act[1], rate, scale, shift, db)
         else:
-            dx = ops.bn_bwd_apply(dy2, y, x2, mask, self.gamma.data, smean, sinv, glob, count, local, dgamma, dbeta, act[0], act[1], rate, scale, shift)
+            dx = ops.bn_bwd_apply(dy2, y, x2, mask, self.gamma.data, smean, sinv, glob, count, local, dgamma, dbeta, act[0], act[1], rate, scale, shift, db)
         return dx.reshape(dy.shape)
 
     def _forward_axis(self, ctx, node, x):
diff --git a/gennet_amd/ops.py b/gennet_amd/ops.py
--- a/gennet_amd/ops.py
+++ b/gennet_amd/ops.py
@@ -214,6 +214,10 @@
     return db
 
 
+def bias_grad_passes():
+    return _lib.size('gn_bias_grad_passes')
+
+
 def conv2d_w2_fold(w, b):
     _chk(w, b)
     kh, kw, Cin, Cout = w.shape
@@ -358,13 +362,13 @@
     return wf, bf
 
 
-def conv1d_up2_unfold_grad(dwf, dbf, Cout, stride, dw=None, db=None):
+def conv1d_up2_unfold_grad(dwf, dbf, Cout, stride, dw=None, db=None, want_db=True):
     _chk(dwf, dbf, dw, db)
     Cin = dwf.shape[1]
     assert dwf.shape[0] == 3 and dwf.shape[2] == Cout * (2 if stride == 1 else 1)
     if dw is None:
         dw = torch.empty((5, Cin, Cout), dtype=torch.float32, device=dwf.device)
-    if db is None:
+    if db is None and want_db:
         db = torch.empty((Cout,), dtype=torch.float32, device=dwf.device)
     _lib.call('gn_conv1d_up2_unfold_grad', _p(dwf), _p(dbf), _p(dw), _p(db), Cin, Cout, stride, _stream())
     return dw, db
@@ -379,24 +383,28 @@
     return y
 
 
-def dense_bwd(x, w, dy, need_dx=True, dw=None, db=None, prev=None):
+def dense_bwd(x, w, dy, need_dx=True, dw=None, db=None, prev=None, want_db=True, db_prev=None):
     _chk(x, w, dy, dw, db)
     B, n_in = x.shape
     n_out = w.shape[1]
     dx = torch.empty_like(x) if need_dx else None
+    if dw is None:
+        dw = torch.empty_like(w)
+    if db is None and want_db:
+        db = torch.empty((n_out,), dtype=torch.float32, device=x.device)
     if prev is not None:
         _, act, param, mask, rate = prev
         assert need_dx and n_out <= 4
-        if dw is None:
-            dw = torch.empty_like(w)
-        if db is None:
-            db = torch.empty((n_out,), dtype=torch.float32, device=x.device)
+        if db_prev is not None:
+            dbp, C_prev = db_prev
+            _chk(dbp)
+            ws = workspace(_lib.size('gn_dense_bwd_fused_db_workspace', n_in), x.device)
+            _lib.call('gn_dense_bwd_fused_db', _p(x), _p(w), _p(dy), _p(dx), _p(dw), _p(db), B, n_in, n_out, _p(mask), ACT[act], float(param), float(rate),
+                      _p(dbp), int(C_prev), _p(ws), ws.numel(), _stream())
+            return dx, dw, db
         _lib.call('gn_dense_bwd_fused', _p(x), _p(w), _p(dy), _p(dx), _p(dw), _p(db), B, n_in, n_out, _p(mask), ACT[act], float(param), float(rate), _stream())
         return dx, dw, db
-    if dw is None:
-        dw = torch.empty_like(w)
-    if db is None:
-        db = torch.empty((n_out,), dtype=torch.float32, device=x.device)
+    assert db_prev is None
     nb = _lib.size('gn_dense_bwd_workspace', B, n_in, n_out)
     ws = workspace(nb, x.device)
     _lib.call('gn_dense_bwd', _p(x), _p(w), _p(dy), _p(dx), _p(dw), _p(db), _p(ws), ws.numel(), B, n_in, n_out, _stream())
@@ -1157,9 +1165,16 @@
 
 
 def bn_bwd_apply(dy2d, y2d, x2d, mask, gamma, smean, sinv, dsums_global, count, dsums_local, dgamma, dbeta, act='linear', act_param=0.0, rate=0.0,
-                 scale=None, shift=None):
+                 scale=None, shift=None, db=None):
     rows, Cc = x2d.shape
     dx = torch.empty_like(x2d)
+    if db is not None:
+        _chk(db)
+        ws = workspace(_lib.size('gn_bn_bwd_apply_db_workspace', rows, Cc), x2d.device)
+        _lib.call('gn_bn_bwd_apply_db', _p(dy2d), _p(y2d), _p(x2d), _p(mask), _p(gamma), _p(smean), _p(sinv), _p(dsums_global), float(count),
+                  _p(dsums_local), _p(dx), _p(dgamma), _p(dbeta), rows, Cc, ACT[act], float(act_param), float(rate), _p(scale), _p(shift),
+                  _p(db), _p(ws), ws.numel(), _stream())
+        return dx
     _lib.call('gn_bn_bwd_apply', _p(dy2d), _p(y2d), _p(x2d), _p(mask), _p(gamma), _p(smean), _p(sinv), _p(dsums_global), float(count),
               _p(dsums_local), _p(dx), _p(dgamma), _p(dbeta), rows, Cc, ACT[act], float(act_param), float(rate), _p(scale), _p(shift), _stream())
     return dx
@@ -1227,9 +1242,16 @@
     return dsums
 
 
-def bn_bwd_apply_conv1(cg, x2d, mask, gamma, smean, sinv, dsums_global, count, dsums_local, dgamma, dbeta, act, act_param, rate, scale, shift):
+def bn_bwd_apply_conv1(cg, x2d, mask, gamma, smean, sinv, dsums_global, count, dsums_local, dgamma, dbeta, act, act_param, rate, scale, shift, db=None):
     rows, Cc = x2d.shape
     dx = torch.empty_like(x2d)
+    if db is not None:
+        _chk(db)
+        ws = workspace(_lib.size('gn_bn_bwd_apply_db_workspace', rows, Cc), x2d.device)
+        _lib.call('gn_bn_bwd_apply_conv1_db', _p(cg.g), _p(cg.w), cg.L, cg.Lout, cg.k, cg.pad_left, _p(x2d), _p(mask), _p(gamma), _p(smean), _p(sinv),
+                  _p(dsums_global), float(count), _p(dsums_local), _p(dx), _p(dgamma), _p(dbeta), rows, Cc, ACT[act], float(act_param), float(rate),
+                  _p(scale), _p(shift), _p(db), _p(ws), ws.numel(), _stream())
+        return dx
     _lib.call('gn_bn_bwd_apply_conv1', _p(cg.g), _p(cg.w), cg.L, cg.Lout, cg.k, cg.pad_left, _p(x2d), _p(mask), _p(gamma), _p(smean), _p(sinv),
               _p(dsums_global), float(count), _p(dsums_local), _p(dx), _p(dgamma), _p(dbeta), rows, Cc, ACT[act], float(act_param), float(rate),
               _p(scale), _p(shift), _stream())
diff --git a/include/gennet_hip.h b/include/gennet_hip.h
--- a/include/gennet_hip.h
+++ b/include/gennet_hip.h
@@ -80,6 +80,10 @@
 
 int gn_dense_bwd_fused(const float* x, const float* w, const float* dy, float* dx, float* dw, float* db, int B, int in, int out,
                        const uint8_t* mask_prev, int act_prev, float act_param_prev, float rate_prev, void* stream);
+size_t gn_dense_bwd_fused_db_workspace(int in);
+int gn_dense_bwd_fused_db(const float* x, const float* w, const float* dy, float* dx, float* dw, float* db, int B, int in, int out,
+                          const uint8_t* mask_prev, int act_prev, float act_param_prev, float rate_prev, float* db_prev, int C_prev,
+                          void* ws, size_t ws_bytes, void* stream);
 
 int gn_act_fwd(const float* x, float* y, size_t n, int act, float act_param, void* stream);
 int gn_act_bwd(const float* dy, const float* y, float* dx, size_t n, int act, float act_param, void* stream);
@@ -90,6 +94,7 @@
                         uint64_t seed, uint64_t offset, void* stream);
 size_t gn_bias_grad_workspace(size_t rows, int C);
 int gn_bias_grad(const float* dy, float* db, void* ws, size_t ws_bytes, size_t rows, int C, void* stream);
+size_t gn_bias_grad_passes(void);
 int gn_conv_fold_bn(const float* w, const float* bias, const float* scale, const float* shift, float* w_out, float* bias_out,
                     size_t rows, int Cout, void* stream);
 int gn_prelu_fwd(const float* x, const float* alpha, float* y, int B, size_t F, void* stream);
@@ -162,6 +167,17 @@
                           const double* dsums_local, float* dx, float* dgamma, float* dbeta, size_t rows, int C, int act, float act_param,
                           float rate, const float* scale, const float* shift, void* stream);
 
+size_t gn_bn_bwd_apply_db_workspace(size_t rows, int C);
+int gn_bn_bwd_apply_db(const float* dy, const float* y, const float* x, const uint8_t* mask,
+                       const float* gamma, const float* save_mean, const float* save_invstd,
+                       const double* dsums_global, double count, const double* dsums_local, float* dx, float* dgamma, float* dbeta,
+                       size_t rows, int C, int act, float act_param, float rate, const float* scale, const float* shift,
+                       float* db, void* ws, size_t ws_bytes, void* stream);
+int gn_bn_bwd_apply_conv1_db(const float* g, const float* w, int L, int Lout, int k, int pad_left, const float* x, const uint8_t* mask,
+                             const float* gamma, const float* save_mean, const float* save_invstd, const double* dsums_global, double count,
+                             const double* dsums_local, float* dx, float* dgamma, float* dbeta, size_t rows, int C, int act, float act_param,
+                             float rate, const float* scale, const float* shift, float* db, void* ws, size_t ws_bytes, void* stream);
+
 size_t gn_bn_axis_stats_workspace(size_t outer, int P, int inner);
 int gn_bn_axis_stats(const float* x, size_t outer, int P, int inner, double* sums, void* ws, size_t ws_bytes, void* stream);
 int gn_bn_axis_apply(const float* x, const float* scale, const float* shift, float* y, size_t outer, int P, int inner, void* stream);
```

Result: no change. 1964 (median of 6 runs) (+1.0%).
